# mandt-lab/vbq

Measured on AMD Instinct MI355X. Metric: quantized latents/sec (32-lambda sweep; one count per (element, lambda) pair and entropy-model build), higher is better.
Workload: dtype f32; 1 GPU; kodak24_c256 [36864 x 256] f32, 32-lambda sweep, N=10; step = two-pass entropy-model build (quantizer.py:82-150); elements_per_gpu=9437184, lambdas=32, parallelism=element-sharded x1, launch=one HIP graph replay per step

## Files before the change

### include/vbq.h

```cpp
#ifndef VBQ_H_
#define VBQ_H_

#include <stddef.h>
#include <stdint.h>

#ifdef __cplusplus
extern "C" {
#endif

#define VBQ_ABI_VERSION 5

enum {
    VBQ_OK = 0,
    VBQ_ERR_INVALID_ARGUMENT = -1,
    VBQ_ERR_UNSUPPORTED = -2,
    VBQ_ERR_LAUNCH = -3,
    VBQ_ERR_WORKSPACE = -4
};

enum {
    VBQ_LAYOUT_BC = 0,
    VBQ_LAYOUT_CB = 1,
    VBQ_LAYOUT_BC_TO_CB = 2
};

enum {
    VBQ_MODE_F32 = 0,
    VBQ_MODE_F64_SCORE = 1
};

int vbq_abi_version(void);
const char *vbq_last_error(void);


enum { VBQ_GRID_K1 = 0, VBQ_GRID_K1T = 1 };
int vbq_solve_grid(int32_t kernel, int64_t n_rows, int32_t n_ch, int32_t workgroups_per_cu, int32_t reserved_workgroups,
                   int64_t *h_grid);

int vbq_device_count(void);
int vbq_device_name(int dev, char *buf, size_t buflen);

size_t vbq_quantize_workspace_bytes(int32_t n_ch, int32_t n_lambda, int32_t N);

int vbq_check_inputs_f32(const float *d_mu, const float *d_sigma, int64_t n, uint32_t *d_bad, void *stream);

int vbq_quantize_f32(const float *d_mu, const float *d_sigma, int64_t n_rows, int32_t n_ch,
                     int32_t layout, const float *d_table_lm, const float *d_level_len,
                     const double *h_lambdas, int32_t n_lambda, int32_t N, int32_t mode,
                     uint16_t *d_out_idx, float *d_out_zhat, float *d_out_bits,
                     void *d_workspace, size_t workspace_bytes, void *stream);

int vbq_n_bit_intervals_f32(const float *d_z_cb, int64_t n_rows, int32_t n_ch, const float *d_table_lm, int32_t N,
                            float *d_left, float *d_right, void *stream);

int vbq_quantize_rows_f32(const float *d_mu, const float *d_sigma, int64_t n_rows, int32_t n_ch,
                          int32_t layout, const float *d_table_lm, const float *d_level_len,
                          const double *h_lambdas, int32_t n_lambda, int32_t N, int32_t mode,
                          uint16_t *d_out_idx, float *d_out_zhat, float *d_out_bits,
                          void *d_workspace, size_t workspace_bytes, int64_t row_begin, int64_t row_end,
                          int32_t workgroups_per_cu, int32_t reserved_workgroups, void *stream);

int vbq_level_counts_f32(const float *d_mu, const float *d_sigma, int64_t n_rows, int32_t n_ch,
                         int32_t layout, const float *d_table_lm, const float *d_level_len,
                         const double *h_lambdas, int32_t n_lambda, int32_t N, int64_t *d_level_counts,
                         void *d_workspace, size_t workspace_bytes, int32_t reserved_workgroups, void *stream);

int vbq_code_lengths_from_counts(const void *d_counts, int32_t counts_are_i32, int64_t n,
                                 const float *d_lut, int64_t lut_n, int32_t level_period,
                                 float *d_out_len, float *d_out_model, void *stream);

typedef void (*vbq_f32_loop)(char **args, const intptr_t *dimensions, const intptr_t *steps, void *data);
typedef struct vbq_host_stage {
    const void *h_counts;
    int32_t counts_are_i32;
    int32_t add_level;
    int64_t n_rows;
    int64_t K;
    float add_n_smoothing;
    int32_t status;
    vbq_f32_loop log2_loop;
    void *log2_data;
    float *h_out_model;
    float *h_out_len;
    int64_t runs;
} vbq_host_stage;
int vbq_host_neg_log2_freq_f32(const void *h_counts, int32_t counts_are_i32, int64_t n_rows, int64_t K, float add_n_smoothing,
                               int32_t add_level, vbq_f32_loop log2_loop, void *log2_data, float *h_out_model,
                               float *h_out_len);
void vbq_host_stage_run(void *stage);

int vbq_argmax_candidates_f32(const float *d_P, const float *d_len, int32_t len_per_lambda,
                              const float *d_mu, const float *d_sigma, int64_t n_elems,
                              const double *h_lambdas, int32_t n_lambda, int32_t M, int32_t mode,
                              int32_t *d_out_j, float *d_out_zhat, float *d_out_bits, void *stream);

int vbq_xi_intervals_f64(const double *d_xi, int64_t K, int32_t N, double *d_left, double *d_right, void *stream);
int vbq_xi_select_f64(const double *d_F, const double *d_endpoints, const double *d_unsquashed, int64_t K, int32_t N,
                      double lamb, double *d_z_hat, int64_t *d_num_bits, double *d_xi_hat, double *d_f_z_hat, void *stream);

int vbq_quantize_notebook_f64(const float *d_means, const float *d_stds, int64_t n,
                              const double *d_codebook_lm, const double *h_betas, int32_t n_beta,
                              int32_t N, uint16_t *d_out_idx, float *d_out_val, void *stream);

int vbq_histogram_u16(const uint16_t *d_idx, int64_t n_rows, int32_t n_ch, int32_t layout,
                      int32_t n_lambda, int32_t N, int64_t *d_counts, void *stream);

int vbq_histogram_u16_i32(const uint16_t *d_idx, int64_t n_rows, int32_t n_ch, int32_t layout,
                          int32_t n_lambda, int32_t N, int32_t *d_counts, void *stream);

int vbq_histogram_rows_u16(const uint16_t *d_idx, int64_t n_rows, int32_t n_ch, int32_t layout,
                           int32_t n_lambda, int32_t N, void *d_counts, int32_t counts_are_i32,
                           int64_t row_begin, int64_t row_end, void *stream);

int vbq_histogram_models_u16(const uint16_t *d_idx, int64_t n_rows, int32_t n_ch, int32_t n_lambda, int32_t N,
                             void *d_counts, int32_t counts_are_i32, const float *d_lut, int64_t lut_n,
                             float *d_models, void *stream);

int vbq_index_max_u16(const uint16_t *d_idx, int64_t n, uint32_t *d_max, void *stream);

int vbq_moments_f32(const float *d_x, int64_t n_rows, int32_t n_ch, int32_t layout,
                    double *d_out , void *stream);

size_t vbq_numpy_sum_sq_workspace_bytes(int64_t n);
int vbq_numpy_sum_sq_f32(const float *d_x, int64_t n, float *d_out, void *d_workspace, size_t workspace_bytes,
                         void *stream);

size_t vbq_numpy_row_sums_workspace_bytes(int64_t n_rows, int64_t n);
int vbq_numpy_row_sums_f32(const float *d_x, int64_t n_rows, int64_t n, float *d_out, void *d_workspace,
                           size_t workspace_bytes, void *stream);

int vbq_gather_f32(const uint16_t *d_idx, int64_t n_rows, int32_t n_ch, int32_t layout,
                   int32_t n_lambda, int32_t N, const float *d_tab, int32_t tab_per_lambda,
                   float *d_out, int32_t out_layout, void *stream);

int vbq_rd_sums_u16(const float *d_mu, const float *d_sigma, const uint16_t *d_idx, int64_t n_rows, int32_t n_ch,
                    int32_t layout, int32_t n_lambda, int32_t N, const float *d_tab_sorted, const float *d_rate,
                    int32_t rate_per_lambda, double *d_out, void *stream);

int vbq_transpose_f32(const float *d_in, int64_t n_rows, int64_t n_cols, float *d_out, void *stream);

int vbq_transpose_planes(const void *d_in, int64_t n_batch, int64_t n_rows, int64_t n_cols, int32_t elem_bytes,
                         void *d_out, void *stream);

enum { VBQ_SPREAD_SIGMA = 0, VBQ_SPREAD_VARIANCE = 1, VBQ_SPREAD_LOGVAR = 2 };
int vbq_prep_planes_f32(const float *d_means_bc, const float *d_spread_bc, int32_t spread_kind, int64_t n_rows,
                        int32_t n_ch, float *d_mu_cb, float *d_sigma_cb, void *stream);
int vbq_gather_latents_u16(const uint16_t *d_idx_planes, int64_t n_rows, int32_t n_ch, int32_t n_lambda, int32_t N,
                           const float *d_table_sorted, const float *d_level_len, const float *d_models,
                           float *d_out_zhat, void *d_out_raw_bits, float *d_out_num_bits, uint16_t *d_out_idx,
                           void *stream);
size_t vbq_compress_latents_workspace_bytes(int64_t n_rows, int32_t n_ch, int32_t n_lambda, int32_t N);
int vbq_compress_latents_f32(const float *d_means_bc, const float *d_spread_bc, int32_t spread_kind,
                             int64_t n_rows, int32_t n_ch, const float *d_table_lm, const float *d_table_sorted,
                             const float *d_level_len, const float *d_models, const double *h_lambdas,
                             int32_t n_lambda, int32_t N, float *d_out_zhat, void *d_out_raw_bits,
                             float *d_out_num_bits, void *d_workspace, size_t workspace_bytes, void *stream);

size_t vbq_build_entropy_models_workspace_bytes(int64_t n_rows, int32_t n_ch, int32_t n_lambda, int32_t N);
int vbq_build_entropy_models_f32(const float *d_means_bc, const float *d_spread_bc, int32_t spread_kind, int64_t n_rows,
                                 int32_t n_ch, const float *d_table_lm, const double *h_lambdas, int32_t n_lambda,
                                 int32_t N, const float *d_lut_levels, int64_t n_lut_levels, const float *d_lut_ranks,
                                 int64_t n_lut_ranks, int64_t *d_level_counts, float *d_level_len, float *d_raw_models,
                                 void *d_counts, int32_t counts_are_i32, float *d_models, void *d_workspace,
                                 size_t workspace_bytes, int32_t reserved_workgroups, void *stream);

#define VBQ_BMSHJ_PARAMS_PER_CHANNEL 43

int vbq_bmshj_cdf_pdf_f32(const float *d_params, const float *d_x, int64_t n_rows, int32_t n_ch,
                          float *d_cdf, float *d_pdf, float *d_logpdf, void *stream);

int vbq_bmshj_icdf_step_f32(const float *d_params, const float *d_xi, int64_t n_rows, int32_t n_ch,
                            float *d_left, float *d_right, float *d_mid, uint32_t *d_flags,
                            void *stream);

int vbq_bmshj_icdf_chain_f32(const float *d_params, const float *d_xi, int64_t n_rows, int32_t n_ch,
                             float *d_left, float *d_right, float *d_mid, uint32_t *d_flags, int32_t n_steps,
                             float tol, int32_t first, void *stream);

int vbq_bmshj_nll_grad_f32(const float *d_params, const float *d_x_cb, int64_t n_rows, int32_t n_ch,
                           double *d_out , void *stream);

int vbq_rans_encode_u16(const uint16_t *d_idx, int64_t n_streams, int64_t n, int32_t N, int32_t seg,
                        const uint16_t *d_freq, uint16_t *d_words, uint32_t *d_sizes, void *stream);
int vbq_rans_sizes_u16(const uint16_t *d_idx, int64_t n_streams, int64_t n, int32_t N, int32_t seg, const uint16_t *d_freq,
                       uint32_t *d_sizes, void *stream);
int vbq_rans_decode_u16(const uint16_t *d_words, const uint32_t *d_sizes, int64_t n_streams, int64_t n,
                        int32_t N, int32_t seg, const uint16_t *d_freq, uint16_t *d_idx, uint32_t *d_status,
                        void *stream);
int vbq_rans_pack_u16(const uint16_t *d_words, const uint32_t *d_sizes, int64_t n_streams, int64_t n, int32_t seg,
                      uint16_t *d_payload, int64_t *d_offsets, uint64_t *d_total, void *stream);
int vbq_rans_unpack_u16(const uint16_t *d_payload, int64_t n_words, const uint16_t *d_sizes_in, int64_t n_streams,
                        int64_t n, int32_t seg, uint16_t *d_words, uint32_t *d_sizes, int64_t *d_offsets,
                        uint32_t *d_status, void *stream);
int vbq_rans_segment_offsets_u16(const uint16_t *d_sizes, int64_t M, int32_t seg, int64_t n_words, int64_t *d_offsets,
                                 uint32_t *d_status, void *stream);
int vbq_rans_decode_values_f32(const uint16_t *d_payload, int64_t n_words, const uint16_t *d_sizes, const int64_t *d_offsets,
                               int64_t n, int32_t seg, int32_t N, const uint16_t *d_freq, const float *d_values,
                               const int64_t *d_segments, int64_t n_sel, float *d_out, uint32_t *d_status, void *stream);

int vbq_rans_il_sizes_u16(const uint16_t *d_idx, int64_t n_streams, int64_t n, int32_t N, int32_t part,
                          const uint16_t *d_freq, uint32_t *d_sizes, void *stream);
int vbq_rans_il_encode_u16(const uint16_t *d_idx, int64_t n_streams, int64_t n, int32_t N, int32_t part,
                           const uint16_t *d_freq, const uint32_t *d_sizes, const int64_t *d_offsets, uint16_t *d_payload,
                           int64_t n_words, void *stream);
int vbq_rans_il_decode_u16(const uint16_t *d_payload, int64_t n_words, const uint32_t *d_sizes, const int64_t *d_offsets,
                           int64_t n_streams, int64_t n, int32_t N, int32_t part, const uint16_t *d_freq, uint16_t *d_idx,
                           uint32_t *d_status, void *stream);

int vbq_rans_map_encode_u16(const uint16_t *d_idx, int32_t n_planes, const uint8_t *d_cls, int32_t n_classes, int64_t n_streams,
                            int64_t n, int32_t N, int32_t seg, const uint16_t *d_freq, uint16_t *d_words, uint32_t *d_sizes,
                            void *stream);
int vbq_rans_map_sizes_u16(const uint16_t *d_idx, int32_t n_planes, const uint8_t *d_cls, int32_t n_classes, int64_t n_streams,
                           int64_t n, int32_t N, int32_t seg, const uint16_t *d_freq, uint32_t *d_sizes, void *stream);
int vbq_rans_map_decode_u16(const uint16_t *d_words, const uint32_t *d_sizes, const uint8_t *d_cls, int32_t n_classes,
                            int64_t n_streams, int64_t n, int32_t N, int32_t seg, const uint16_t *d_freq, uint16_t *d_idx,
                            uint32_t *d_status, void *stream);

int vbq_pack_counts_3x21(const int32_t *d_counts, int64_t n, int64_t *d_words, int32_t n_ranks,
                         uint32_t *d_overflow, void *stream);
int vbq_unpack_counts_3x21(const int64_t *d_words, int64_t n, int32_t *d_counts, void *stream);

#define VBQ_COMM_ID_BYTES 128
// ... 75 lines not shown
```

### vbq_amd/_lib.py

```python
from __future__ import annotations

import ctypes as C
import os


_LIB = None

c_f32p = C.c_void_p
c_u16p = C.c_void_p

OK = 0
ABI_VERSION = 5
LAYOUT_BC, LAYOUT_CB, LAYOUT_BC_TO_CB = 0, 1, 2
MODE_F32, MODE_F64_SCORE = 0, 1
BMSHJ_PARAMS_PER_CHANNEL = 43
COMM_ID_BYTES = 128

SIGNATURES = {
    "vbq_abi_version": (C.c_int, []),
    "vbq_last_error": (C.c_char_p, []),
    "vbq_solve_grid": (C.c_int, [C.c_int32, C.c_int64, C.c_int32, C.c_int32, C.c_int32, C.POINTER(C.c_int64)]),
    "vbq_device_count": (C.c_int, []),
    "vbq_device_name": (C.c_int, [C.c_int, C.c_char_p, C.c_size_t]),
    "vbq_quantize_workspace_bytes": (C.c_size_t, [C.c_int32, C.c_int32, C.c_int32]),
    "vbq_check_inputs_f32": (C.c_int, [C.c_void_p, C.c_void_p, C.c_int64, C.c_void_p, C.c_void_p]),
    "vbq_quantize_f32": (C.c_int, [C.c_void_p, C.c_void_p, C.c_int64, C.c_int32, C.c_int32, C.c_void_p, C.c_void_p,
                                   C.POINTER(C.c_double), C.c_int32, C.c_int32, C.c_int32, C.c_void_p, C.c_void_p,
                                   C.c_void_p, C.c_void_p, C.c_size_t, C.c_void_p]),
    "vbq_n_bit_intervals_f32": (C.c_int, [C.c_void_p, C.c_int64, C.c_int32, C.c_void_p, C.c_int32, C.c_void_p, C.c_void_p,
                                          C.c_void_p]),
    "vbq_quantize_rows_f32": (C.c_int, [C.c_void_p, C.c_void_p, C.c_int64, C.c_int32, C.c_int32, C.c_void_p, C.c_void_p,
                                        C.POINTER(C.c_double), C.c_int32, C.c_int32, C.c_int32, C.c_void_p, C.c_void_p,
                                        C.c_void_p, C.c_void_p, C.c_size_t, C.c_int64, C.c_int64, C.c_int32, C.c_int32, C.c_void_p]),
    "vbq_level_counts_f32": (C.c_int, [C.c_void_p, C.c_void_p, C.c_int64, C.c_int32, C.c_int32, C.c_void_p, C.c_void_p,
                                       C.POINTER(C.c_double), C.c_int32, C.c_int32, C.c_void_p, C.c_void_p, C.c_size_t,
                                       C.c_int32, C.c_void_p]),
    "vbq_code_lengths_from_counts": (C.c_int, [C.c_void_p, C.c_int32, C.c_int64, C.c_void_p, C.c_int64, C.c_int32,
                                               C.c_void_p, C.c_void_p, C.c_void_p]),
    "vbq_host_neg_log2_freq_f32": (C.c_int, [C.c_void_p, C.c_int32, C.c_int64, C.c_int64, C.c_float, C.c_int32, C.c_void_p, C.c_void_p,
                                             C.c_void_p, C.c_void_p]),
    "vbq_host_stage_run": (None, [C.c_void_p]),
    "vbq_histogram_rows_u16": (C.c_int, [C.c_void_p, C.c_int64, C.c_int32, C.c_int32, C.c_int32, C.c_int32, C.c_void_p,
                                         C.c_int32, C.c_int64, C.c_int64, C.c_void_p]),
    "vbq_xi_intervals_f64": (C.c_int, [C.c_void_p, C.c_int64, C.c_int32, C.c_void_p, C.c_void_p, C.c_void_p]),
    "vbq_xi_select_f64": (C.c_int, [C.c_void_p, C.c_void_p, C.c_void_p, C.c_int64, C.c_int32, C.c_double, C.c_void_p,
                                    C.c_void_p, C.c_void_p, C.c_void_p, C.c_void_p]),
    "vbq_quantize_notebook_f64": (C.c_int, [C.c_void_p, C.c_void_p, C.c_int64, C.c_void_p, C.POINTER(C.c_double),
                                            C.c_int32, C.c_int32, C.c_void_p, C.c_void_p, C.c_void_p]),
    "vbq_histogram_u16": (C.c_int, [C.c_void_p, C.c_int64, C.c_int32, C.c_int32, C.c_int32, C.c_int32, C.c_void_p,
                                    C.c_void_p]),
    "vbq_histogram_u16_i32": (C.c_int, [C.c_void_p, C.c_int64, C.c_int32, C.c_int32, C.c_int32, C.c_int32,
                                        C.c_void_p, C.c_void_p]),
    "vbq_histogram_models_u16": (C.c_int, [C.c_void_p, C.c_int64, C.c_int32, C.c_int32, C.c_int32, C.c_void_p, C.c_int32,
                                           C.c_void_p, C.c_int64, C.c_void_p, C.c_void_p]),
    "vbq_index_max_u16": (C.c_int, [C.c_void_p, C.c_int64, C.c_void_p, C.c_void_p]),
    "vbq_moments_f32": (C.c_int, [C.c_void_p, C.c_int64, C.c_int32, C.c_int32, C.c_void_p, C.c_void_p]),
    "vbq_numpy_sum_sq_workspace_bytes": (C.c_size_t, [C.c_int64]),
    "vbq_numpy_sum_sq_f32": (C.c_int, [C.c_void_p, C.c_int64, C.c_void_p, C.c_void_p, C.c_size_t, C.c_void_p]),
    "vbq_numpy_row_sums_workspace_bytes": (C.c_size_t, [C.c_int64, C.c_int64]),
    "vbq_numpy_row_sums_f32": (C.c_int, [C.c_void_p, C.c_int64, C.c_int64, C.c_void_p, C.c_void_p, C.c_size_t, C.c_void_p]),
    "vbq_gather_f32": (C.c_int, [C.c_void_p, C.c_int64, C.c_int32, C.c_int32, C.c_int32, C.c_int32, C.c_void_p,
                                 C.c_int32, C.c_void_p, C.c_int32, C.c_void_p]),
    "vbq_rd_sums_u16": (C.c_int, [C.c_void_p, C.c_void_p, C.c_void_p, C.c_int64, C.c_int32, C.c_int32, C.c_int32, C.c_int32,
                                  C.c_void_p, C.c_void_p, C.c_int32, C.c_void_p, C.c_void_p]),
    "vbq_transpose_f32": (C.c_int, [C.c_void_p, C.c_int64, C.c_int64, C.c_void_p, C.c_void_p]),
    "vbq_transpose_planes": (C.c_int, [C.c_void_p, C.c_int64, C.c_int64, C.c_int64, C.c_int32, C.c_void_p, C.c_void_p]),
    "vbq_prep_planes_f32": (C.c_int, [C.c_void_p, C.c_void_p, C.c_int32, C.c_int64, C.c_int32, C.c_void_p, C.c_void_p, C.c_void_p]),
    "vbq_gather_latents_u16": (C.c_int, [C.c_void_p, C.c_int64, C.c_int32, C.c_int32, C.c_int32, C.c_void_p, C.c_void_p,
                                         C.c_void_p, C.c_void_p, C.c_void_p, C.c_void_p, C.c_void_p, C.c_void_p]),
    "vbq_compress_latents_workspace_bytes": (C.c_size_t, [C.c_int64, C.c_int32, C.c_int32, C.c_int32]),
    "vbq_compress_latents_f32": (C.c_int, [C.c_void_p, C.c_void_p, C.c_int32, C.c_int64, C.c_int32, C.c_void_p, C.c_void_p,
                                           C.c_void_p, C.c_void_p, C.POINTER(C.c_double), C.c_int32, C.c_int32, C.c_void_p,
                                           C.c_void_p, C.c_void_p, C.c_void_p, C.c_size_t, C.c_void_p]),
    "vbq_build_entropy_models_workspace_bytes": (C.c_size_t, [C.c_int64, C.c_int32, C.c_int32, C.c_int32]),
    "vbq_build_entropy_models_f32": (C.c_int, [C.c_void_p, C.c_void_p, C.c_int32, C.c_int64, C.c_int32, C.c_void_p,
                                               C.POINTER(C.c_double), C.c_int32, C.c_int32, C.c_void_p, C.c_int64, C.c_void_p,
                                               C.c_int64, C.c_void_p, C.c_void_p, C.c_void_p, C.c_void_p, C.c_int32, C.c_void_p,
                                               C.c_void_p, C.c_size_t, C.c_int32, C.c_void_p]),
    "vbq_argmax_candidates_f32": (C.c_int, [C.c_void_p, C.c_void_p, C.c_int32, C.c_void_p, C.c_void_p, C.c_int64,
                                            C.POINTER(C.c_double), C.c_int32, C.c_int32, C.c_int32, C.c_void_p,
                                            C.c_void_p, C.c_void_p, C.c_void_p]),
    "vbq_bmshj_cdf_pdf_f32": (C.c_int, [C.c_void_p, C.c_void_p, C.c_int64, C.c_int32, C.c_void_p, C.c_void_p,
                                        C.c_void_p, C.c_void_p]),
    "vbq_bmshj_icdf_step_f32": (C.c_int, [C.c_void_p, C.c_void_p, C.c_int64, C.c_int32, C.c_void_p, C.c_void_p,
                                          C.c_void_p, C.c_void_p, C.c_void_p]),
    "vbq_bmshj_icdf_chain_f32": (C.c_int, [C.c_void_p, C.c_void_p, C.c_int64, C.c_int32, C.c_void_p, C.c_void_p,
                                           C.c_void_p, C.c_void_p, C.c_int32, C.c_float, C.c_int32, C.c_void_p]),
    "vbq_uniform_quantize_f32": (C.c_int, [C.c_void_p, C.c_int64, C.c_float, C.c_float, C.c_float, C.c_int32, C.c_void_p,
                                           C.c_void_p, C.c_void_p, C.c_void_p]),
    "vbq_nearest_code_f64": (C.c_int, [C.c_void_p, C.c_int64, C.c_void_p, C.c_int32, C.c_void_p, C.c_void_p, C.c_void_p,
                                       C.c_void_p]),
    "vbq_analogy_ranks_workspace_bytes": (C.c_size_t, [C.c_int64, C.c_int32, C.c_int64]),
    "vbq_analogy_ranks_f32": (C.c_int, [C.c_void_p, C.c_int64, C.c_int32, C.c_void_p, C.c_int64, C.c_void_p, C.c_void_p,
                                        C.c_size_t, C.c_void_p]),
    "vbq_image_sqerr_u8": (C.c_int, [C.c_void_p, C.c_void_p, C.c_int64, C.c_int64, C.c_void_p, C.c_void_p]),
    "vbq_u8_to_f64": (C.c_int, [C.c_void_p, C.c_int64, C.c_void_p, C.c_void_p]),
    "vbq_unit_to_u8_f32": (C.c_int, [C.c_void_p, C.c_int64, C.c_void_p, C.c_void_p]),
    "vbq_ssim_scale_workspace_bytes": (C.c_size_t, [C.c_int32, C.c_int32, C.c_int32, C.c_int32, C.c_int32]),
    "vbq_ssim_scale_f64": (C.c_int, [C.c_void_p, C.c_void_p, C.c_int32, C.c_int32, C.c_int32, C.c_int32, C.c_void_p, C.c_int32,
                                     C.c_double, C.c_double, C.c_void_p, C.c_void_p, C.c_void_p, C.c_size_t, C.c_void_p]),
    "vbq_downsample2_f64": (C.c_int, [C.c_void_p, C.c_int32, C.c_int32, C.c_int32, C.c_int32, C.c_void_p, C.c_void_p]),
    "vbq_pack_counts_3x21": (C.c_int, [C.c_void_p, C.c_int64, C.c_void_p, C.c_int32, C.c_void_p, C.c_void_p]),
    "vbq_unpack_counts_3x21": (C.c_int, [C.c_void_p, C.c_int64, C.c_void_p, C.c_void_p]),
    "vbq_comm_unique_id": (C.c_int, [C.c_void_p]),
    "vbq_comm_init": (C.c_int, [C.POINTER(C.c_void_p), C.c_int32, C.c_void_p, C.c_int32]),
    "vbq_allreduce_hist": (C.c_int, [C.c_void_p, C.c_void_p, C.c_int64, C.c_int32, C.c_void_p]),
    "vbq_comm_destroy": (C.c_int, [C.c_void_p]),
    "vbq_rans_encode_u16": (C.c_int, [C.c_void_p, C.c_int64, C.c_int64, C.c_int32, C.c_int32, C.c_void_p, C.c_void_p,
                                      C.c_void_p, C.c_void_p]),
    "vbq_rans_sizes_u16": (C.c_int, [C.c_void_p, C.c_int64, C.c_int64, C.c_int32, C.c_int32, C.c_void_p, C.c_void_p,
                                     C.c_void_p]),
    "vbq_rans_decode_u16": (C.c_int, [C.c_void_p, C.c_void_p, C.c_int64, C.c_int64, C.c_int32, C.c_int32, C.c_void_p,
                                      C.c_void_p, C.c_void_p, C.c_void_p]),
    "vbq_rans_pack_u16": (C.c_int, [C.c_void_p, C.c_void_p, C.c_int64, C.c_int64, C.c_int32, C.c_void_p, C.c_void_p,
                                    C.c_void_p, C.c_void_p]),
    "vbq_rans_unpack_u16": (C.c_int, [C.c_void_p, C.c_int64, C.c_void_p, C.c_int64, C.c_int64, C.c_int32, C.c_void_p,
                                      C.c_void_p, C.c_void_p, C.c_void_p, C.c_void_p]),
    "vbq_rans_segment_offsets_u16": (C.c_int, [C.c_void_p, C.c_int64, C.c_int32, C.c_int64, C.c_void_p, C.c_void_p,
                                               C.c_void_p]),
    "vbq_rans_decode_values_f32": (C.c_int, [C.c_void_p, C.c_int64, C.c_void_p, C.c_void_p, C.c_int64, C.c_int32, C.c_int32,
                                             C.c_void_p, C.c_void_p, C.c_void_p, C.c_int64, C.c_void_p, C.c_void_p,
                                             C.c_void_p]),
    "vbq_rans_il_sizes_u16": (C.c_int, [C.c_void_p, C.c_int64, C.c_int64, C.c_int32, C.c_int32, C.c_void_p, C.c_void_p,
                                        C.c_void_p]),
    "vbq_rans_il_encode_u16": (C.c_int, [C.c_void_p, C.c_int64, C.c_int64, C.c_int32, C.c_int32, C.c_void_p, C.c_void_p,
                                         C.c_void_p, C.c_void_p, C.c_int64, C.c_void_p]),
    "vbq_rans_il_decode_u16": (C.c_int, [C.c_void_p, C.c_int64, C.c_void_p, C.c_void_p, C.c_int64, C.c_int64, C.c_int32,
                                         C.c_int32, C.c_void_p, C.c_void_p, C.c_void_p, C.c_void_p]),
    "vbq_rans_map_encode_u16": (C.c_int, [C.c_void_p, C.c_int32, C.c_void_p, C.c_int32, C.c_int64, C.c_int64, C.c_int32,
                                          C.c_int32, C.c_void_p, C.c_void_p, C.c_void_p, C.c_void_p]),
    "vbq_rans_map_sizes_u16": (C.c_int, [C.c_void_p, C.c_int32, C.c_void_p, C.c_int32, C.c_int64, C.c_int64, C.c_int32,
                                         C.c_int32, C.c_void_p, C.c_void_p, C.c_void_p]),
    "vbq_rans_map_decode_u16": (C.c_int, [C.c_void_p, C.c_void_p, C.c_void_p, C.c_int32, C.c_int64, C.c_int64, C.c_int32,
                                          C.c_int32, C.c_void_p, C.c_void_p, C.c_void_p, C.c_void_p]),
    "vbq_bmshj_nll_grad_f32":(C.c_int, [C.c_void_p, C.c_void_p, C.c_int64, C.c_int32, C.c_void_p, C.c_void_p]),
    "vbq_budget_dp_workspace_bytes": (C.c_size_t, [C.c_int64, C.c_int32, C.c_int32, C.c_int32]),
    "vbq_budget_dp_f64": (C.c_int, [C.c_void_p, C.c_int64, C.c_int32, C.c_int32, C.c_int32, C.c_void_p, C.c_void_p, C.c_void_p,
                                    C.c_void_p, C.c_size_t, C.c_void_p]),
    "vbq_budget_patience_f64": (C.c_int, [C.c_void_p, C.c_int64, C.c_int32, C.c_double, C.c_int32, C.c_void_p, C.c_void_p,
                                          C.c_void_p]),
    "vbq_records_words": (C.c_size_t, [C.c_int32, C.c_int32, C.c_int32]),
    "vbq_records_pack_u16": (C.c_int, [C.c_void_p, C.c_int64, C.c_int32, C.c_int32, C.c_int32, C.c_void_p, C.c_void_p,
                                       C.c_void_p]),
    "vbq_records_unpack_f32": (C.c_int, [C.c_void_p, C.c_int64, C.c_int32, C.c_int32, C.c_int32, C.c_void_p, C.c_int32,
                                         C.c_void_p, C.c_int64, C.c_void_p, C.c_void_p, C.c_void_p, C.c_void_p]),
    "vbq_topk_workspace_bytes": (C.c_size_t, [C.c_int64, C.c_int32, C.c_int64, C.c_int32, C.c_int32]),
    "vbq_records_topk_f32": (C.c_int, [C.c_void_p, C.c_int64, C.c_int32, C.c_int32, C.c_int32, C.c_void_p, C.c_int32,
                                       C.c_void_p, C.c_int64, C.c_int32, C.c_int32, C.c_void_p, C.c_int32, C.c_void_p,
                                       C.c_void_p, C.c_void_p, C.c_int32, C.c_void_p, C.c_size_t, C.c_void_p]),
    "vbq_topk_f32": (C.c_int, [C.c_void_p, C.c_int64, C.c_int32, C.c_void_p, C.c_int64, C.c_int32, C.c_int32, C.c_void_p,
                               C.c_int32, C.c_void_p, C.c_void_p, C.c_int32, C.c_void_p, C.c_size_t, C.c_void_p]),
    "vbq_records_bag_f32": (C.c_int, [C.c_void_p, C.c_int64, C.c_int32, C.c_int32, C.c_int32, C.c_void_p, C.c_int32,
                                      C.c_void_p, C.c_int64, C.c_void_p, C.c_int64, C.c_void_p, C.c_int32, C.c_void_p,
                                      C.c_void_p, C.c_void_p]),
    "vbq_bag_f32": (C.c_int, [C.c_void_p, C.c_int64, C.c_int32, C.c_void_p, C.c_int64, C.c_void_p, C.c_int64, C.c_void_p,
                              C.c_int32, C.c_void_p, C.c_void_p, C.c_void_p]),
    "vbq_rans_decode_window_f32": (C.c_int, [C.c_void_p, C.c_int64, C.c_void_p, C.c_void_p, C.c_int64, C.c_void_p, C.c_int32,
                                             C.c_void_p, C.c_int32, C.c_void_p, C.c_int32, C.c_int32, C.c_int32, C.c_int32,
                                             C.c_void_p, C.c_int32, C.c_void_p, C.c_int64, C.c_int64, C.c_int64, C.c_void_p,
                                             C.c_void_p, C.c_void_p]),
    "vbq_rans_encode_files_u16": (C.c_int, [C.c_void_p, C.c_int64, C.c_void_p, C.c_int32, C.c_void_p, C.c_int64, C.c_int32,
                                            C.c_int32, C.c_int32, C.c_void_p, C.c_int32, C.c_void_p, C.c_void_p, C.c_void_p,
                                            C.c_int64, C.c_void_p, C.c_void_p]),
    "vbq_rans_sizes_files_u16": (C.c_int, [C.c_void_p, C.c_int64, C.c_int64, C.c_void_p, C.c_int32, C.c_void_p, C.c_int64,
                                           C.c_int32, C.c_int32, C.c_int32, C.c_void_p, C.c_int32, C.c_void_p, C.c_void_p,
                                           C.c_void_p, C.c_void_p]),
}


class HostStageDesc(C.Structure):
    _fields_ = [("h_counts", C.c_void_p), ("counts_are_i32", C.c_int32), ("add_level", C.c_int32), ("n_rows", C.c_int64),
                ("K", C.c_int64), ("add_n_smoothing", C.c_float), ("status", C.c_int32), ("log2_loop", C.c_void_p),
                ("log2_data", C.c_void_p), ("h_out_model", C.c_void_p), ("h_out_len", C.c_void_p), ("runs", C.c_int64)]


class VBQError(RuntimeError):
    pass


def library_path() -> str:
    from . import build as _build
    return os.environ.get("VBQ_HIP_LIBRARY", _build.LIB)


def lib():
    global _LIB
    if _LIB is not None:
        return _LIB
    path = library_path()
    if not os.path.exists(path):
        raise VBQError(f"HIP extension not built: {path} is missing. Run `python -m vbq_amd.build` "
# ... 23 lines not shown
```

### vbq_amd/csrc/vbq_common.h

```cpp
#pragma once

#include <hip/hip_runtime.h>
#include <stdint.h>

#include "vbq.h"

namespace vbq {

void set_error(const char *fmt, ...);

int num_cus();
int fast_debug();
int64_t resident_slots(int per_cu, int reserved);

#define VBQ_REQUIRE(cond, code, ...)            \
    do {                                        \
        if (!(cond)) {                          \
            ::vbq::set_error(__VA_ARGS__);      \
            return (code);                      \
        }                                       \
    } while (0)

#define VBQ_CHECK_LAUNCH(what)                                                        \
    do {                                                                              \
        hipError_t e__ = hipGetLastError();                                           \
        if (e__ != hipSuccess) {                                                      \
            ::vbq::set_error("%s: %s", (what), hipGetErrorString(e__));               \
            return VBQ_ERR_LAUNCH;                                                    \
        }                                                                             \
    } while (0)

__device__ __forceinline__ void set_issue_priority(unsigned int p) {
    p = __builtin_amdgcn_readfirstlane(p) & 3u;
    if (p == 0) __builtin_amdgcn_s_setprio(0);
    else if (p == 1) __builtin_amdgcn_s_setprio(1);
    else if (p == 2) __builtin_amdgcn_s_setprio(2);
    else __builtin_amdgcn_s_setprio(3);
}
__device__ __forceinline__ unsigned int wave_slot() { return __builtin_amdgcn_s_getreg((3 << 11) | 4); }
__device__ __forceinline__ void rotate_issue_priority(unsigned int &rot) {
#ifndef VBQ_NO_ISSUE_ROTATION
    set_issue_priority(rot);
    rot += 3u;
#endif
}

constexpr int kWave = 64;
constexpr int kTileChannels = 16;
constexpr int kMaxLambdaChunk = 32;

__host__ __device__ constexpr int table_size(int N) { return (2 << N) - 1; }

__device__ __forceinline__ float neg_half_sq_err(float P, float mu, float sigma) {
    float d = __fsub_rn(P, mu);
    float t = __fdiv_rn(d, sigma);
    float q = __fmul_rn(t, t);
    return __fmul_rn(-0.5f, q);
}

#ifdef VBQ_ONLY_N10
#define VBQ_FOR_EACH_N(X) X(10)
#else
#define VBQ_FOR_EACH_N(X) X(12) X(11) X(10) X(9) X(8) X(7) X(6) X(5) X(4)
#endif

struct Lambdas32 {
    float lam[kMaxLambdaChunk];
};

template <int N>
int launch_quant_fast(const float *mu, const float *sg, int64_t n_per_ch, int64_t ch_stride, int32_t n_ch, const float *table,
                      const Lambdas32 &lam, const float *len, int32_t L, uint16_t *out_idx, float *out_zhat,
                      float *out_bits, int64_t E, int vec_ok,
                      unsigned long long *level_counts, int wg_per_cu, int reserved, hipStream_t st);

template <int N>
int launch_quant_pruned(const float *mu, const float *sg, int64_t n_per_ch, int64_t ch_stride, int32_t n_ch, const float *table,
                        const Lambdas32 &lam, const float *len, int32_t L, uint16_t *out_idx, int64_t E, int vec_ok, hipStream_t st);

int launch_level_counts_hull10(const float *mu, const float *sg, int64_t n_per_ch, int64_t ch_stride, int32_t n_ch,
                               const float *table, const double *lam, int32_t L, int vec_ok,
                               unsigned long long *level_counts, int reserved, hipStream_t st);

int launch_quant_hull_idx10(const float *mu, const float *sg, int64_t n_per_ch, int64_t ch_stride, int32_t n_ch,
                            const float *table, const double *lam, int32_t L, int vec_ok, uint16_t *out_idx, int64_t E,
                            hipStream_t st);

}
```

### vbq_amd/csrc/vbq_latents.hip

```cpp
#include <atomic>

#include <type_traits>

#include "vbq_common.h"

namespace vbq {
namespace {

constexpr int kGlRows = 32, kGlCh = 64;
template <int N>
__global__ void __launch_bounds__(256)
k_gather_latents(const uint16_t *__restrict__ idx, long B, int C, const float *__restrict__ tab_sorted,
                 const float *__restrict__ level_len, const float *__restrict__ models, float *__restrict__ out_z,
                 float *__restrict__ out_raw, int raw_as_int, float *__restrict__ out_nb, uint16_t *__restrict__ out_idx) {
    constexpr int T = table_size(N), N1 = N + 1;
    __shared__ float tz[kGlCh][kGlRows + 1], tr[kGlCh][kGlRows + 1], tn[kGlCh][kGlRows + 1];
    __shared__ uint16_t tq[kGlCh][kGlRows + 2];
    const int l = blockIdx.y;
    const long ctiles = (C + kGlCh - 1) / kGlCh;
    const long r0 = ((long)blockIdx.x / ctiles) * kGlRows;
    const int c0 = (int)((long)blockIdx.x % ctiles) * kGlCh;
    const long E = B * (long)C;
    {
        const int tx = threadIdx.x & 31, ty = threadIdx.x >> 5;
// ... 318 lines not shown
}

namespace vbq {
namespace {
__global__ void __launch_bounds__(256)
k_gather(const uint16_t *__restrict__ idx, long n_rows, int C, int layout, long E, int T,
         const float *__restrict__ tab, int per_lambda, float *__restrict__ out) {
    const int l = blockIdx.y;
    const uint16_t *src = idx + (long)l * E;
    float *dst = out + (long)l * E;
    const float *tl = tab + (per_lambda ? (long)l * C * T : 0);
    for (long e = (long)blockIdx.x * blockDim.x + threadIdx.x; e < E; e += (long)gridDim.x * blockDim.x) {
        const int c = (C == 1) ? 0 : (layout == VBQ_LAYOUT_BC ? (int)(e % C) : (int)(e / n_rows));
        dst[e] = tl[(long)c * T + min((int)src[e], T - 1)];
    }
}

__global__ void __launch_bounds__(256)
k_gather_transpose(const uint16_t *__restrict__ idx, long in_rows, long in_cols, int in_layout, long E, int C, int T,
                   const float *__restrict__ tab, int per_lambda, float *__restrict__ out) {
    __shared__ float tile[32][33];
    const int l = blockIdx.z;
    const uint16_t *src = idx + (long)l * E;
    float *dst = out + (long)l * E;
    const float *tl = tab + (per_lambda ? (long)l * C * T : 0);
    const long ctiles = (in_cols + 31) / 32;
    const long r0 = ((long)blockIdx.x / ctiles) * 32, c0 = ((long)blockIdx.x % ctiles) * 32;
    const int tx = threadIdx.x & 31, ty = threadIdx.x >> 5;
#pragma unroll
    for (int k = 0; k < 4; ++k) {
        const long r = r0 + ty + 8 * k, c = c0 + tx;
        if (r < in_rows && c < in_cols) {
            const int ch = in_layout == VBQ_LAYOUT_CB ? (int)r : (int)c;
            tile[ty + 8 * k][tx] = tl[(long)ch * T + min((int)src[r * in_cols + c], T - 1)];
        }
    }
    __syncthreads();
#pragma unroll
    for (int k = 0; k < 4; ++k) {
        const long c = c0 + ty + 8 * k, r = r0 + tx;
        if (r < in_rows && c < in_cols) dst[c * in_rows + r] = tile[tx][ty + 8 * k];
    }
}
}
}

extern "C" int vbq_gather_f32(const uint16_t *d_idx, int64_t n_rows, int32_t n_ch, int32_t layout,
                              int32_t n_lambda, int32_t N, const float *d_tab, int32_t tab_per_lambda,
                              float *d_out, int32_t out_layout, void *stream) {
    using namespace vbq;
    VBQ_REQUIRE(n_rows == 0 || (d_idx && d_tab && d_out), VBQ_ERR_INVALID_ARGUMENT, "vbq_gather_f32: null pointer argument");
    VBQ_REQUIRE(n_rows >= 0 && n_ch >= 1 && n_lambda >= 1 && n_lambda <= 65535 && N >= 0 && N <= 15,
                VBQ_ERR_INVALID_ARGUMENT, "vbq_gather_f32: bad sizes");
    VBQ_REQUIRE((layout == VBQ_LAYOUT_BC || layout == VBQ_LAYOUT_CB) &&
                    (out_layout == VBQ_LAYOUT_BC || out_layout == VBQ_LAYOUT_CB),
                VBQ_ERR_INVALID_ARGUMENT, "vbq_gather_f32: unknown layout %d -> %d", layout, out_layout);
    if (n_rows == 0) return VBQ_OK;
    const int64_t E = n_rows * (int64_t)n_ch;
    if (n_ch > 1 && layout != out_layout) {
        const int64_t in_rows = layout == VBQ_LAYOUT_CB ? n_ch : n_rows;
        const int64_t in_cols = layout == VBQ_LAYOUT_CB ? n_rows : n_ch;
        const int64_t tiles = ((in_cols + 31) / 32) * ((in_rows + 31) / 32);
        VBQ_REQUIRE(n_lambda <= 65535 && tiles <= 0x7fffffffll, VBQ_ERR_UNSUPPORTED,
                    "vbq_gather_f32: grid too large for the transposing form");
        hipLaunchKernelGGL(k_gather_transpose, dim3((unsigned)tiles, 1, (unsigned)n_lambda),
                           dim3(256), 0, reinterpret_cast<hipStream_t>(stream), d_idx, (long)in_rows, (long)in_cols,
                           (int)layout, (long)E, (int)n_ch, table_size(N), d_tab, (int)tab_per_lambda, d_out);
        VBQ_CHECK_LAUNCH("gather_transpose");
        return VBQ_OK;
    }
    int64_t gx = (E + 255) / 256;
    const int64_t cap = 4096 / n_lambda + 1;
    if (gx > cap) gx = cap;
    hipLaunchKernelGGL(k_gather, dim3((unsigned)gx, (unsigned)n_lambda), dim3(256), 0,
                       reinterpret_cast<hipStream_t>(stream), d_idx, (long)n_rows, (int)n_ch, (int)layout, (long)E,
                       table_size(N), d_tab, (int)tab_per_lambda, d_out);
    VBQ_CHECK_LAUNCH("gather");
    return VBQ_OK;
}

extern "C" size_t vbq_compress_latents_workspace_bytes(int64_t n_rows, int32_t n_ch, int32_t n_lambda, int32_t N) {
    if (n_rows < 0 || n_ch <= 0 || n_lambda <= 0 || N < 0) return 0;
    const size_t E = (size_t)n_rows * (size_t)n_ch;
    return 2 * vbq::align256(E * sizeof(float)) + vbq::align256((size_t)n_lambda * E * sizeof(uint16_t)) +
           vbq::align256(vbq_quantize_workspace_bytes(n_ch, n_lambda, N));
}

extern "C" int vbq_compress_latents_f32(const float *d_means_bc, const float *d_spread_bc, int32_t spread_kind,
                                        int64_t n_rows, int32_t n_ch, const float *d_table_lm, const float *d_table_sorted,
                                        const float *d_level_len, const float *d_models, const double *h_lambdas,
                                        int32_t n_lambda, int32_t N, float *d_out_zhat, void *d_out_raw_bits,
                                        float *d_out_num_bits, void *d_workspace, size_t workspace_bytes, void *stream) {
    using namespace vbq;
    VBQ_REQUIRE(n_rows >= 0 && n_ch >= 1 && n_lambda >= 1, VBQ_ERR_INVALID_ARGUMENT, "vbq_compress_latents_f32: bad sizes");
    if (n_rows == 0) return VBQ_OK;
    const size_t need = vbq_compress_latents_workspace_bytes(n_rows, n_ch, n_lambda, N);
    VBQ_REQUIRE(d_workspace && workspace_bytes >= need, VBQ_ERR_WORKSPACE, "vbq_compress_latents_f32: workspace of %zu bytes given, %zu needed",
                workspace_bytes, need);
    VBQ_REQUIRE((reinterpret_cast<uintptr_t>(d_workspace) & 255) == 0, VBQ_ERR_INVALID_ARGUMENT,
                "vbq_compress_latents_f32: workspace must be 256-byte aligned");
    const size_t E = (size_t)n_rows * (size_t)n_ch;
    char *w = static_cast<char *>(d_workspace);
    float *mu_cb = reinterpret_cast<float *>(w);
    w += align256(E * sizeof(float));
    float *sg_cb = reinterpret_cast<float *>(w);
    w += align256(E * sizeof(float));
    uint16_t *idx = reinterpret_cast<uint16_t *>(w);
    w += align256((size_t)n_lambda * E * sizeof(uint16_t));
    const size_t qws = vbq_quantize_workspace_bytes(n_ch, n_lambda, N);
    int rc = vbq_prep_planes_f32(d_means_bc, d_spread_bc, spread_kind, n_rows, n_ch, mu_cb, sg_cb, stream);
    if (rc != VBQ_OK) return rc;
    rc = vbq_quantize_f32(mu_cb, sg_cb, n_rows, n_ch, VBQ_LAYOUT_CB, d_table_lm, d_level_len, h_lambdas, n_lambda, N, VBQ_MODE_F32,
                          idx, nullptr, nullptr, w, qws, stream);
    if (rc != VBQ_OK) return rc;
    return vbq_gather_latents_u16(idx, n_rows, n_ch, n_lambda, N, d_table_sorted, d_level_len, d_models, d_out_zhat, d_out_raw_bits,
                                  d_out_num_bits, nullptr, stream);
}

extern "C" size_t vbq_build_entropy_models_workspace_bytes(int64_t n_rows, int32_t n_ch, int32_t n_lambda, int32_t N) {
    return vbq_compress_latents_workspace_bytes(n_rows, n_ch, n_lambda, N);
}

extern "C" int vbq_build_entropy_models_f32(const float *d_means_bc, const float *d_spread_bc, int32_t spread_kind, int64_t n_rows,
                                            int32_t n_ch, const float *d_table_lm, const double *h_lambdas, int32_t n_lambda,
                                            int32_t N, const float *d_lut_levels, int64_t n_lut_levels, const float *d_lut_ranks,
                                            int64_t n_lut_ranks, int64_t *d_level_counts, float *d_level_len, float *d_raw_models,
                                            void *d_counts, int32_t counts_are_i32, float *d_models, void *d_workspace,
                                            size_t workspace_bytes, int32_t reserved_workgroups, void *stream) {
    using namespace vbq;
    VBQ_REQUIRE(n_rows >= 1 && n_ch >= 1 && n_lambda >= 1 && N >= 0 && N <= 15, VBQ_ERR_INVALID_ARGUMENT,
                "vbq_build_entropy_models_f32: bad sizes");
    VBQ_REQUIRE(d_lut_levels && n_lut_levels > n_rows && d_level_counts && d_level_len && d_raw_models && d_counts,
                VBQ_ERR_INVALID_ARGUMENT, "vbq_build_entropy_models_f32: null pointer argument, or a code-length table shorter than n_rows + 1");
    VBQ_REQUIRE((d_models == nullptr) == (d_lut_ranks == nullptr) && (!d_lut_ranks || n_lut_ranks > n_rows), VBQ_ERR_INVALID_ARGUMENT,
                "vbq_build_entropy_models_f32: d_models and d_lut_ranks go together (n_rows + 1 entries)");
    const size_t need = vbq_build_entropy_models_workspace_bytes(n_rows, n_ch, n_lambda, N);
    VBQ_REQUIRE(d_workspace && workspace_bytes >= need, VBQ_ERR_WORKSPACE,
                "vbq_build_entropy_models_f32: workspace of %zu bytes given, %zu needed", workspace_bytes, need);
    VBQ_REQUIRE((reinterpret_cast<uintptr_t>(d_workspace) & 255) == 0, VBQ_ERR_INVALID_ARGUMENT,
                "vbq_build_entropy_models_f32: workspace must be 256-byte aligned");
    const size_t E = (size_t)n_rows * (size_t)n_ch;
    const int64_t N1 = N + 1;
    char *w = static_cast<char *>(d_workspace);
    float *mu_cb = reinterpret_cast<float *>(w);
    w += align256(E * sizeof(float));
    float *sg_cb = reinterpret_cast<float *>(w);
    w += align256(E * sizeof(float));
    uint16_t *idx = reinterpret_cast<uint16_t *>(w);
    w += align256((size_t)n_lambda * E * sizeof(uint16_t));
    const size_t qws = vbq_quantize_workspace_bytes(n_ch, n_lambda, N);
    hipStream_t st = reinterpret_cast<hipStream_t>(stream);
    int rc = vbq_prep_planes_f32(d_means_bc, d_spread_bc, spread_kind, n_rows, n_ch, mu_cb, sg_cb, stream);
    if (rc != VBQ_OK) return rc;
    hipError_t e = hipMemsetAsync(d_level_counts, 0, sizeof(int64_t) * (size_t)n_lambda * (size_t)n_ch * (size_t)N1, st);
    if (e != hipSuccess) {
        set_error("vbq_build_entropy_models_f32: hipMemsetAsync: %s", hipGetErrorString(e));
        return VBQ_ERR_LAUNCH;
    }
    rc = vbq_level_counts_f32(mu_cb, sg_cb, n_rows, n_ch, VBQ_LAYOUT_CB, d_table_lm, nullptr, h_lambdas, n_lambda, N, d_level_counts, w, qws,
                              reserved_workgroups, stream);
    if (rc != VBQ_OK) return rc;
    rc = vbq_code_lengths_from_counts(d_level_counts, 0, (int64_t)n_lambda * n_ch * N1, d_lut_levels, n_lut_levels, (int32_t)N1, d_level_len,
                                      d_raw_models, stream);
    if (rc != VBQ_OK) return rc;
    rc = vbq_quantize_rows_f32(mu_cb, sg_cb, n_rows, n_ch, VBQ_LAYOUT_CB, d_table_lm, d_level_len, h_lambdas, n_lambda, N, VBQ_MODE_F32, idx,
                               nullptr, nullptr, w, qws, 0, n_rows, 0, reserved_workgroups, stream);
    if (rc != VBQ_OK) return rc;
    return vbq_histogram_models_u16(idx, n_rows, n_ch, n_lambda, N, d_counts, counts_are_i32, d_lut_ranks, n_lut_ranks, d_models, stream);
}
```

### vbq_amd/csrc/vbq_quantize.hip

```cpp
#include "vbq_common.h"

namespace vbq {
namespace {

template <int N>
struct Elem {
    float a[N + 1];
    float b[N + 1];
    uint32_t G;
};

template <int N>
__device__ __forceinline__ void search_and_score(const float *tb, float z, float sg, Elem<N> &e) {
    uint32_t g = 0;
#pragma unroll
    for (int n = 0; n <= N; ++n) {
        const int off = (1 << n) - 1;
        const int m = 1 << n;
        const uint32_t j = g;
        const float pj = tb[off + j];
        const bool below = pj < z;
        if (n == 0) {
            const float s0 = neg_half_sq_err(pj, z, sg);
            e.a[0] = s0;
// ... 192 lines not shown

    const int c0 = blockIdx.y * kTileChannels;
    const int ncg = min(kTileChannels, C - c0);
    for (int i = threadIdx.x; i < ncg * T; i += blockDim.x) {
        const int ch = i / T, s = i - ch * T;
        tb[ch * TS + s] = table[(long)(c0 + ch) * T + s];
    }
    if constexpr (kPenInLds) {
        for (int i = threadIdx.x; i < L * ncg * N1; i += blockDim.x) {
            const int n = i % N1;
            const int ch = (i / N1) % ncg;
            const int l = i / (N1 * ncg);
            pl[(l * kTileChannels + ch) * PS + n] = pen[((long)l * C + c0 + ch) * N1 + n];
        }
    }
    __syncthreads();

    const int cl = threadIdx.x & (kTileChannels - 1);
    const int slot = threadIdx.x >> 4;
    if (cl >= ncg) return;
    const float *mytb = tb + cl * TS;
    const int c = c0 + cl;

    for (long rb = (long)blockIdx.x * kRowsPerIter; rb < n_rows; rb += (long)gridDim.x * kRowsPerIter) {
        Elem<N> el[kTiledNE];
        long row[kTiledNE];
#pragma unroll
        for (int k = 0; k < kTiledNE; ++k) {
            row[k] = rb + k * 64 + slot;
            const bool ok = row[k] < n_rows;
            const float m = ok ? mu[row[k] * C + c] : 0.0f;
            const float s = ok ? sg[row[k] * C + c] : 1.0f;
            search_and_score<N>(mytb, m, s, el[k]);
        }
        for (int l = 0; l < L; ++l) {
            PenT p[N1];
            const PenT *pp = kPenInLds ? pl + (l * kTileChannels + cl) * PS : pen + ((long)l * C + c) * N1;
#pragma unroll
            for (int n = 0; n < N1; ++n) p[n] = pp[n];
#pragma unroll
            for (int k = 0; k < kTiledNE; ++k) {
                int bj;
                if constexpr (sizeof(PenT) == 4) bj = argmax_scan<N>(el[k], p);
                else bj = argmax_scan_f64<N>(el[k], p);
                int lvl; uint32_t pos;
                winner_slot<N>(el[k].G, bj, lvl, pos);
                if (row[k] < n_rows) {
                    const long o = (long)l * E + row[k] * C + c;
                    out_idx[o] = (uint16_t)(((2 * pos + 1) << (N - lvl)) - 1);
                    if (out_zhat) out_zhat[o] = mytb[(1 << lvl) - 1 + pos];
                    if (out_bits) out_bits[o] = len ? len[((long)l * C + c) * N1 + lvl] : (float)lvl;
                }
            }
        }
    }
}

template <int N>
__global__ void __launch_bounds__(256)
k_intervals(const float *__restrict__ z_cb, long n_rows, const float *__restrict__ table, float *__restrict__ left,
            float *__restrict__ right) {
    constexpr int T = table_size(N);
    __shared__ float tb[T + 1];
    const int c = blockIdx.y;
    for (int i = threadIdx.x; i < T; i += blockDim.x) tb[i] = table[(long)c * T + i];
    __syncthreads();
    for (long b = (long)blockIdx.x * blockDim.x + threadIdx.x; b < n_rows; b += (long)gridDim.x * blockDim.x) {
        const float z = z_cb[(long)c * n_rows + b];
        uint32_t g = 0;
#pragma unroll
        for (int n = 0; n <= N; ++n) {
            const int off = (1 << n) - 1;
            const int m = 1 << n;
            const uint32_t j = g;
            const float pj = tb[off + j];
            const bool below = pj < z;
            float l = pj, r = pj;
            if (n > 0) {
                int jo = below ? (int)j + 1 : (int)j - 1;
                jo = jo < 0 ? 0 : (jo > m - 1 ? m - 1 : jo);
                bool swap = false;
                if (n == N && below && j == (uint32_t)(m - 1)) { jo = m - 2; swap = true; }
                const float po = tb[off + jo];
                const bool j_is_left = below && !swap;
                l = j_is_left ? pj : po;
                r = j_is_left ? po : pj;
            }
            const long o = ((long)c * (N + 1) + n) * n_rows + b;
            left[o] = l;
            right[o] = r;
            g = 2 * g + (below ? 1u : 0u);
        }
    }
}

template <int N, typename PenT>
int launch_quantize(const float *mu, const float *sg, int64_t n_rows, int32_t n_ch, int32_t layout,
                    const float *table, const float *level_len, const double *h_lambdas, int32_t L,
                    uint16_t *out_idx, float *out_zhat, float *out_bits, void *ws, int64_t row_begin, int64_t row_end,
                    unsigned long long *level_counts, int wg_per_cu, int reserved, hipStream_t st) {
    constexpr int N1 = N + 1;
    const int64_t E = n_rows * (int64_t)n_ch;
    const int64_t n_sub = row_end - row_begin;
    PenT *pen = reinterpret_cast<PenT *>(ws);
    const bool bc_to_cb = layout == VBQ_LAYOUT_BC_TO_CB && n_ch > 1;
    const bool flat = (n_ch == 1) || (layout == VBQ_LAYOUT_CB) || bc_to_cb;

    for (int l0 = 0; l0 < L; l0 += kMaxLambdaChunk) {
        const int Lc = (L - l0 < kMaxLambdaChunk) ? (L - l0) : kMaxLambdaChunk;
        LambdaChunk lc;
        for (int i = 0; i < kMaxLambdaChunk; ++i) lc.lam[i] = i < Lc ? h_lambdas[l0 + i] : 0.0;
        const int total = Lc * n_ch * N1;
        const float *len_c = level_len ? level_len + (int64_t)l0 * n_ch * N1 : nullptr;
        bool pen_ready = false;
        auto prepare = [&]() -> int {
            if (pen_ready) return VBQ_OK;
            hipLaunchKernelGGL((k_prepare_penalties<PenT>), dim3((total + 255) / 256), dim3(256), 0, st, lc, Lc,
                               (int)n_ch, N1, len_c, pen);
            VBQ_CHECK_LAUNCH("prepare_penalties");
            pen_ready = true;
            return VBQ_OK;
        };
        Lambdas32 l32;
        for (int i = 0; i < kMaxLambdaChunk; ++i) l32.lam[i] = i < Lc ? (float)lc.lam[i] : 0.0f;

        const int64_t off = (flat && !bc_to_cb) ? row_begin : row_begin * n_ch;
        const int64_t off_out = flat ? row_begin : row_begin * n_ch;
        const float *mu_r = mu + off, *sg_r = sg + off;
        uint16_t *oi = out_idx ? out_idx + (int64_t)l0 * E + off_out : nullptr;
        float *oz = out_zhat ? out_zhat + (int64_t)l0 * E + off_out : nullptr;
        float *ob = out_bits ? out_bits + (int64_t)l0 * E + off_out : nullptr;
        unsigned long long *lc_out = level_counts ? level_counts + (int64_t)l0 * n_ch * N1 : nullptr;
        if (flat) {
            const int64_t n_per_ch = n_sub;
            const int64_t ch_stride = n_rows;
            const int vec_ok = ((n_rows % 4 == 0) || n_ch == 1) &&
                               ((reinterpret_cast<uintptr_t>(mu_r) | reinterpret_cast<uintptr_t>(sg_r)) % 16 == 0) &&
                               (reinterpret_cast<uintptr_t>(oi) % 8 == 0) && (E % 4 == 0 || L == 1) &&
                               (!oz || reinterpret_cast<uintptr_t>(oz) % 16 == 0) &&
                               (!ob || reinterpret_cast<uintptr_t>(ob) % 16 == 0);
            const int vec2_ok = ((reinterpret_cast<uintptr_t>(mu_r) | reinterpret_cast<uintptr_t>(sg_r)) % 4 == 0) &&
                                (reinterpret_cast<uintptr_t>(oi) % 2 == 0) && (!oz || reinterpret_cast<uintptr_t>(oz) % 4 == 0) &&
                                (!ob || reinterpret_cast<uintptr_t>(ob) % 4 == 0);
            const int64_t nquads = (n_per_ch + 3) / 4;
            int64_t gx = (nquads + 255) / 256;
            const int64_t cap = (int64_t)num_cus() * 8 / (n_ch < 8 ? n_ch : 8) + 1;
            if (gx > cap) gx = cap;
            if (gx < 1) gx = 1;
            bool fast_ok = sizeof(PenT) == 4;
            for (int i = 0; i < Lc; ++i) fast_ok = fast_ok && (lc.lam[i] >= 1.9e-12 && lc.lam[i] <= 1.8e19);
            if constexpr (sizeof(PenT) == 4 && N == 10) {
                if (fast_ok && lc_out && !len_c) {
                    const int r = launch_level_counts_hull10(mu_r, sg_r, n_per_ch, ch_stride, n_ch, table, lc.lam, Lc,
                                                             vec2_ok | (bc_to_cb ? 2 : 0), lc_out, reserved, st);
                    if (r == VBQ_OK) continue;
                    if (r < 0) return r;
                }
            }
            if constexpr (sizeof(PenT) == 4 && N == 10) {
                if (fast_ok && !lc_out && !len_c && oi && !oz && !ob) {
                    const int r = launch_quant_hull_idx10(mu_r, sg_r, n_per_ch, ch_stride, n_ch, table, lc.lam, Lc,
                                                          vec2_ok | (bc_to_cb ? 2 : 0), oi, E, st);
                    if (r == VBQ_OK) continue;
                    if (r < 0) return r;
                }
            }
            if constexpr (sizeof(PenT) == 4) {
                if (!lc_out && oi && !oz && !ob && wg_per_cu == 0) {
                    const int r = launch_quant_pruned<N>(mu_r, sg_r, n_per_ch, ch_stride, n_ch, table, l32, len_c, Lc, oi, E,
                                                         vec2_ok | (bc_to_cb ? 2 : 0), st);
                    if (r == VBQ_OK) continue;
                    if (r < 0) return r;
                }
            }
            if constexpr (sizeof(PenT) == 4) {
                if (fast_ok) {
                    const int r = launch_quant_fast<N>(mu_r, sg_r, n_per_ch, ch_stride, n_ch, table, l32, len_c, Lc, oi, oz, ob,
                                                       E, vec2_ok | (bc_to_cb ? 2 : 0), lc_out, wg_per_cu, reserved, st);
                    if (r != VBQ_OK) return r;
                    continue;
                }
            }
            if (level_counts) {
                set_error("vbq_level_counts_f32 is served by the fast f32 kernel only (every lambda in [1.9e-12, 1.8e19]); "
                          "use vbq_quantize_f32 + vbq_histogram_u16 instead");
                return VBQ_ERR_UNSUPPORTED;
            }
            if (bc_to_cb) {
                set_error("vbq_quantize_f32: VBQ_LAYOUT_BC_TO_CB is served by the fast f32 kernel only (VBQ_MODE_F32, every "
                          "lambda in [1.9e-12, 1.8e19]); transpose with vbq_transpose_f32 and use VBQ_LAYOUT_CB instead");
                return VBQ_ERR_UNSUPPORTED;
            }
            if (const int r = prepare(); r != VBQ_OK) return r;
            hipLaunchKernelGGL((k_quant_flat<N, PenT>), dim3((unsigned)gx, (unsigned)n_ch), dim3(256), 0, st, mu_r, sg_r,
                               (long)n_per_ch, (long)ch_stride, (int)n_ch, table, pen, len_c, Lc, oi, oz, ob, (long)E, vec_ok);
            VBQ_CHECK_LAUNCH("quant_flat");
        } else if constexpr (N > 10) {
            set_error("vbq_quantize_f32: N=%d is built for channel-major planes only (VBQ_LAYOUT_CB, or n_ch = 1): "
                      "16 tables of %d points do not fit the LDS; transpose with vbq_transpose_f32 first", N, table_size(N));
            return VBQ_ERR_UNSUPPORTED;
        } else {
            constexpr int T = table_size(N);
            constexpr int PS = (N1 + 3) & ~3;
            const size_t lds = sizeof(float) * kTileChannels * (T + 2) + 16 +
                               (sizeof(PenT) == 4 ? sizeof(PenT) * (size_t)kMaxLambdaChunk * kTileChannels * PS : 0);
            {
                hipError_t e = hipFuncSetAttribute(reinterpret_cast<const void *>(&k_quant_tiled<N, PenT>),
                                                   hipFuncAttributeMaxDynamicSharedMemorySize, (int)lds);
                if (e != hipSuccess) {
                    set_error("hipFuncSetAttribute(%zu B LDS): %s", lds, hipGetErrorString(e));
                    return VBQ_ERR_LAUNCH;
                }
            }
            const int groups = (n_ch + kTileChannels - 1) / kTileChannels;
            int64_t iters = (n_sub + kRowsPerIter - 1) / kRowsPerIter;
            int64_t gx = (256 + groups - 1) / groups;
            if (gx > iters) gx = iters;
            if (gx < 1) gx = 1;
            if (const int r = prepare(); r != VBQ_OK) return r;
            hipLaunchKernelGGL((k_quant_tiled<N, PenT>), dim3((unsigned)gx, (unsigned)groups), dim3(kTiledThreads),
                               lds, st, mu_r, sg_r, (long)n_sub, (int)n_ch, table, pen, len_c, Lc, oi, oz, ob, (long)E);
            VBQ_CHECK_LAUNCH("quant_tiled");
        }
    }
    return VBQ_OK;
}

}
}

extern "C" size_t vbq_quantize_workspace_bytes(int32_t n_ch, int32_t n_lambda, int32_t N) {
    if (n_ch <= 0 || n_lambda <= 0 || N < 0) return 0;
    const int Lc = n_lambda < vbq::kMaxLambdaChunk ? n_lambda : vbq::kMaxLambdaChunk;
    return (size_t)Lc * (size_t)n_ch * (size_t)(N + 1) * sizeof(double) + 256;
}

namespace vbq {
namespace {
int quantize_entry(const char *who, const float *d_mu, const float *d_sigma, int64_t n_rows, int32_t n_ch, int32_t layout,
                   const float *d_table_lm, const float *d_level_len, const double *h_lambdas, int32_t n_lambda,
                   int32_t N, int32_t mode, uint16_t *d_out_idx, float *d_out_zhat, float *d_out_bits,
                   void *d_workspace, size_t workspace_bytes, int64_t row_begin, int64_t row_end,
                   unsigned long long *level_counts, int32_t wg_per_cu, int32_t reserved_wgs, void *stream) {
    const bool counting = level_counts != nullptr;
    VBQ_REQUIRE(n_rows >= 0 && n_ch >= 1 && n_lambda >= 1, VBQ_ERR_INVALID_ARGUMENT,
                "%s: bad sizes n_rows=%lld n_ch=%d n_lambda=%d", who, (long long)n_rows, n_ch, n_lambda);
    VBQ_REQUIRE(0 <= row_begin && row_begin <= row_end && row_end <= n_rows, VBQ_ERR_INVALID_ARGUMENT,
                "%s: row range [%lld, %lld) outside [0, %lld)", who, (long long)row_begin, (long long)row_end, (long long)n_rows);
    VBQ_REQUIRE(row_begin == row_end || (d_mu && d_sigma && d_table_lm && h_lambdas && (d_out_idx || counting)),
                VBQ_ERR_INVALID_ARGUMENT, "%s: null pointer argument", who);
    VBQ_REQUIRE(layout == VBQ_LAYOUT_BC || layout == VBQ_LAYOUT_CB || layout == VBQ_LAYOUT_BC_TO_CB, VBQ_ERR_INVALID_ARGUMENT,
                "%s: unknown layout %d", who, layout);
    VBQ_REQUIRE(mode == VBQ_MODE_F32 || mode == VBQ_MODE_F64_SCORE, VBQ_ERR_INVALID_ARGUMENT, "%s: unknown mode %d", who, mode);
    VBQ_REQUIRE(!(mode == VBQ_MODE_F64_SCORE && d_level_len), VBQ_ERR_UNSUPPORTED,
                "%s: VBQ_MODE_F64_SCORE supports raw integer lengths only", who);
    VBQ_REQUIRE(n_ch <= 65535, VBQ_ERR_UNSUPPORTED, "%s: n_ch=%d exceeds 65535", who, n_ch);
    VBQ_REQUIRE(wg_per_cu >= 0 && wg_per_cu <= 5, VBQ_ERR_INVALID_ARGUMENT, "%s: workgroups_per_cu=%d not in 0..5", who, wg_per_cu);
    VBQ_REQUIRE(!counting || n_ch == 1 || layout != VBQ_LAYOUT_BC, VBQ_ERR_UNSUPPORTED,
                "%s: channel-last input with n_ch > 1 is not served (use VBQ_LAYOUT_CB planes or VBQ_LAYOUT_BC_TO_CB)", who);
    const size_t need = vbq_quantize_workspace_bytes(n_ch, n_lambda, N);
    VBQ_REQUIRE(d_workspace && workspace_bytes >= need, VBQ_ERR_WORKSPACE, "%s: workspace of %zu bytes given, %zu needed", who,
                workspace_bytes, need);
    if (row_begin == row_end) return VBQ_OK;
    hipStream_t st = reinterpret_cast<hipStream_t>(stream);
    const int reserved = reserved_wgs < 0 ? 0 : reserved_wgs;
#define VBQ_DISPATCH_N(NN)                                                                                         \
    case NN:                                                                                                       \
        return mode == VBQ_MODE_F32                                                                                \
                   ? launch_quantize<NN, float>(d_mu, d_sigma, n_rows, n_ch, layout, d_table_lm, d_level_len,      \
                                                h_lambdas, n_lambda, d_out_idx, d_out_zhat, d_out_bits,            \
                                                d_workspace, row_begin, row_end, level_counts, wg_per_cu, reserved, st) \
                   : launch_quantize<NN, double>(d_mu, d_sigma, n_rows, n_ch, layout, d_table_lm, d_level_len,     \
                                                 h_lambdas, n_lambda, d_out_idx, d_out_zhat, d_out_bits,           \
                                                 d_workspace, row_begin, row_end, level_counts, wg_per_cu, reserved, st);
    switch (N) {
        VBQ_FOR_EACH_N(VBQ_DISPATCH_N)
        default:
            set_error("%s: max_bits_per_coord N=%d not built (have 4 ... 12; only 10 with VBQ_ONLY_N10)", who, N);
            return VBQ_ERR_UNSUPPORTED;
    }
#undef VBQ_DISPATCH_N
}
}
}

extern "C" int vbq_quantize_f32(const float *d_mu, const float *d_sigma, int64_t n_rows, int32_t n_ch,
                                int32_t layout, const float *d_table_lm, const float *d_level_len,
                                const double *h_lambdas, int32_t n_lambda, int32_t N, int32_t mode,
                                uint16_t *d_out_idx, float *d_out_zhat, float *d_out_bits, void *d_workspace,
                                size_t workspace_bytes, void *stream) {
    return vbq::quantize_entry("vbq_quantize_f32", d_mu, d_sigma, n_rows, n_ch, layout, d_table_lm, d_level_len, h_lambdas,
                               n_lambda, N, mode, d_out_idx, d_out_zhat, d_out_bits, d_workspace, workspace_bytes, 0,
                               n_rows, nullptr, 0, -1, stream);
}

extern "C" int vbq_quantize_rows_f32(const float *d_mu, const float *d_sigma, int64_t n_rows, int32_t n_ch,
                                     int32_t layout, const float *d_table_lm, const float *d_level_len,
                                     const double *h_lambdas, int32_t n_lambda, int32_t N, int32_t mode,
                                     uint16_t *d_out_idx, float *d_out_zhat, float *d_out_bits, void *d_workspace,
                                     size_t workspace_bytes, int64_t row_begin, int64_t row_end,
                                     int32_t workgroups_per_cu, int32_t reserved_workgroups, void *stream) {
    return vbq::quantize_entry("vbq_quantize_rows_f32", d_mu, d_sigma, n_rows, n_ch, layout, d_table_lm, d_level_len,
                               h_lambdas, n_lambda, N, mode, d_out_idx, d_out_zhat, d_out_bits, d_workspace, workspace_bytes,
                               row_begin, row_end, nullptr, workgroups_per_cu, reserved_workgroups, stream);
}

extern "C" int vbq_level_counts_f32(const float *d_mu, const float *d_sigma, int64_t n_rows, int32_t n_ch,
                                    int32_t layout, const float *d_table_lm, const float *d_level_len,
                                    const double *h_lambdas, int32_t n_lambda, int32_t N, int64_t *d_level_counts,
                                    void *d_workspace, size_t workspace_bytes, int32_t reserved_workgroups, void *stream) {
    using namespace vbq;
    VBQ_REQUIRE(n_rows == 0 || d_level_counts, VBQ_ERR_INVALID_ARGUMENT, "vbq_level_counts_f32: null pointer argument");
    return quantize_entry("vbq_level_counts_f32", d_mu, d_sigma, n_rows, n_ch, layout, d_table_lm, d_level_len, h_lambdas,
                          n_lambda, N, VBQ_MODE_F32, nullptr, nullptr, nullptr, d_workspace, workspace_bytes, 0, n_rows,
                          reinterpret_cast<unsigned long long *>(d_level_counts), 0, reserved_workgroups, stream);
}

extern "C" int vbq_n_bit_intervals_f32(const float *d_z_cb, int64_t n_rows, int32_t n_ch, const float *d_table_lm, int32_t N,
                                       float *d_left, float *d_right, void *stream) {
    using namespace vbq;
    VBQ_REQUIRE(n_rows >= 0 && n_ch >= 1 && n_ch <= 65535, VBQ_ERR_INVALID_ARGUMENT, "vbq_n_bit_intervals_f32: bad sizes");
    if (n_rows == 0) return VBQ_OK;
    VBQ_REQUIRE(d_z_cb && d_table_lm && d_left && d_right, VBQ_ERR_INVALID_ARGUMENT, "vbq_n_bit_intervals_f32: null pointer argument");
    hipStream_t st = reinterpret_cast<hipStream_t>(stream);
    int64_t gx = (n_rows + 255) / 256;
    const int64_t cap = 2048 / n_ch + 1;
    if (gx > cap) gx = cap;
#define VBQ_DISPATCH_N(NN)                                                                                              \
    case NN:                                                                                                            \
        hipLaunchKernelGGL((k_intervals<NN>), dim3((unsigned)gx, (unsigned)n_ch), dim3(256), 0, st, d_z_cb, (long)n_rows, \
                           d_table_lm, d_left, d_right);                                                                \
        break;
    switch (N) {
        VBQ_FOR_EACH_N(VBQ_DISPATCH_N)
        default:
            set_error("vbq_n_bit_intervals_f32: max_bits_per_coord N=%d not built", N);
            return VBQ_ERR_UNSUPPORTED;
    }
#undef VBQ_DISPATCH_N
    VBQ_CHECK_LAUNCH("n_bit_intervals");
    return VBQ_OK;
}
```

### vbq_amd/csrc/vbq_quantize_fast.hip

```cpp
#include <stddef.h>

#include "vbq_common.h"
#include "vbq_sweep.h"

namespace vbq {
namespace {

constexpr int kFastThreads = 256;
#ifndef VBQ_FAST_NE
#define VBQ_FAST_NE 2
#endif
#ifndef VBQ_FAST_WAVES
#define VBQ_FAST_WAVES 4
#endif
#ifndef VBQ_SLOW_INLINE
#define VBQ_SLOW_INLINE __noinline__
#endif
constexpr int kFastNE = VBQ_FAST_NE;

__device__ __forceinline__ float dist_cost(float P, float mu, double rinv) {
    const float d = __fsub_rn(P, mu);
    const float t = (float)__dmul_rn((double)d, rinv);
    const float q = __fmul_rn(t, t);
    return __fmul_rn(0.5f, q);
}

__device__ __forceinline__ float min3f(float a, float b, float c) { return fminf(fminf(a, b), c); }

template <bool NT>
__device__ __forceinline__ void store_idx2(uint32_t *p, uint32_t v) {
    if constexpr (NT) __builtin_nontemporal_store(v, p);
    else *p = v;
}

template <int M>
__device__ __forceinline__ float min_of(const float (&v)[M]) {
    float t[M];
#pragma unroll
    for (int i = 0; i < M; ++i) t[i] = v[i];
    int m = M;
#pragma unroll
    for (int pass = 0; pass < 8; ++pass) {
        if (m <= 1) break;
        int o = 0;
        int i = 0;
#pragma unroll
        for (; i + 2 < m; i += 3) t[o++] = min3f(t[i], t[i + 1], t[i + 2]);
        if (o == 0) { t[o++] = fminf(t[0], t[1]); i = 2; }
        for (; i < m; ++i) t[o++] = t[i];
        m = o;
    }
    return t[0];
}

template <int N>
struct LevelInfo {
    float dL, dR;
    uint32_t posL, posR;
};

template <int N>
__device__ __forceinline__ LevelInfo<N> descend(const float *tb, int n, float z, double sg, uint32_t &g) {
    const int off = (1 << n) - 1;
    const int m = 1 << n;
    const uint32_t j = g;
    const float pj = tb[off + j];
    const bool below = pj < z;
    LevelInfo<N> r;
    if (n == 0) {
        r.dL = r.dR = dist_cost(pj, z, sg);
        r.posL = r.posR = 0;
    } else {
        int jo = below ? (int)j + 1 : (int)j - 1;
        jo = jo < 0 ? 0 : (jo > m - 1 ? m - 1 : jo);
        bool swap = false;
        if (n == N && below && j == (uint32_t)(m - 1)) { jo = m - 2; swap = true; }
        const float po = tb[off + jo];
        const float dj = dist_cost(pj, z, sg);
        const float dn = dist_cost(po, z, sg);
        const bool j_is_left = below && !swap;
        r.dL = j_is_left ? dj : dn;
        r.dR = j_is_left ? dn : dj;
        r.posL = j_is_left ? j : (uint32_t)jo;
        r.posR = j_is_left ? (uint32_t)jo : j;
    }
    g = 2 * g + (below ? 1u : 0u);
    return r;
}

template <int N>
__device__ VBQ_SLOW_INLINE uint32_t exact_rank_scan(const float *tb, float z, float sigma, const float *pen) {
    const double sg = __ddiv_rn(1.0, (double)sigma);
    uint32_t g = 0;
    float bestL = 0.f, bestR = 0.f;
    uint32_t rkL = 0, rkR = 0;
    for (int n = 0; n <= N; ++n) {
        const LevelInfo<N> li = descend<N>(tb, n, z, sg, g);
        const float p = pen[n];
        const float cL = __fadd_rn(li.dL, p);
        if (n == 0 || cL < bestL) { bestL = cL; rkL = ((2 * li.posL + 1) << (N - n)) - 1; }
        if (n >= 1) {
            const float cR = __fadd_rn(li.dR, p);
            if (n == 1 || cR < bestR) { bestR = cR; rkR = ((2 * li.posR + 1) << (N - n)) - 1; }
        }
    }
    if (N == 0) return rkL;
    return (bestL <= bestR) ? rkL : rkR;
}

template <int N, int MODE>
__global__ void __launch_bounds__(kFastThreads, VBQ_FAST_WAVES)
k_quant_fast(const float *__restrict__ mu, const float *__restrict__ sg, long n_per_ch, long ch_stride, int C,
             const float *__restrict__ table, Lambdas32 lam, const float *__restrict__ len,
             int L, uint16_t *__restrict__ out_idx, float *__restrict__ out_zhat,
             float *__restrict__ out_bits, long E, int vec_ok, int dbg,
             unsigned long long *__restrict__ level_counts) {
    constexpr int T = table_size(N);
    constexpr int N1 = N + 1;
    constexpr int NE = kFastNE;
    constexpr bool EXTRA = MODE == 1;
    constexpr bool COUNT = MODE == 2;
    const bool never_flag = dbg == 2;
    constexpr int PS = (N1 + 3) & ~3;
    __shared__ float tb[T + 1];
    __shared__ uint32_t scratch[N1 * NE * kFastThreads];
    __shared__ __align__(16) float penl[kMaxLambdaChunk * PS];
    const int c = blockIdx.y;
    if (COUNT) {
        for (int i = threadIdx.x; i < N1 * NE * kFastThreads; i += blockDim.x) scratch[i] = 0;
    }
    for (int i = threadIdx.x; i < T; i += blockDim.x) tb[i] = table[(long)c * T + i];
    int odd = 0;
    for (int i = threadIdx.x; i < L * PS; i += blockDim.x) {
        const int l = i / PS, n = i - l * PS;
        const float p = n < N1 ? __fmul_rn(lam.lam[l], len ? len[((long)l * C + c) * N1 + n] : (float)n) : 0.0f;
        penl[i] = p;
        odd |= (len != nullptr && !(p == 0.0f || (p >= 1.8189894e-12f && p <= 1.1805916e21f))) ? 1 : 0;
    }
    const bool force_slow = dbg == 1 || __syncthreads_or(odd) != 0;

    const long base = (long)c * ch_stride;
    const long nquads = (n_per_ch + NE - 1) / NE;

    auto load_group = [&](long q, float (&m)[NE], float (&sv)[NE]) {
        const long i0 = q * NE;
        if (!(vec_ok & 2) && (vec_ok & 1) && (i0 + NE <= n_per_ch)) {
            if constexpr (NE == 4) {
                const float4 mv = *reinterpret_cast<const float4 *>(mu + base + i0);
                const float4 s4v = *reinterpret_cast<const float4 *>(sg + base + i0);
                m[0] = mv.x; m[1] = mv.y; m[2] = mv.z; m[3] = mv.w;
                sv[0] = s4v.x; sv[1] = s4v.y; sv[2] = s4v.z; sv[3] = s4v.w;
            } else {
                const float2 mv = *reinterpret_cast<const float2 *>(mu + base + i0);
                const float2 s2v = *reinterpret_cast<const float2 *>(sg + base + i0);
                m[0] = mv.x; m[1] = mv.y;
                sv[0] = s2v.x; sv[1] = s2v.y;
            }
        } else {
#pragma unroll
            for (int k = 0; k < NE; ++k) {
                const bool ok = i0 + k < n_per_ch;
                const long at = (vec_ok & 2) ? (i0 + k) * C + c : base + i0 + k;
                m[k] = ok ? mu[at] : 0.0f;
                sv[k] = ok ? sg[at] : 1.0f;
            }
        }
    };
    const long q0 = (long)blockIdx.x * blockDim.x + threadIdx.x, qstep = (long)gridDim.x * blockDim.x;
    float mn[NE], sn[NE];
#pragma unroll
    for (int k = 0; k < NE; ++k) { mn[k] = 0.0f; sn[k] = 1.0f; }
    if (q0 < nquads) load_group(q0, mn, sn);
    const bool resident = (vec_ok & 4) != 0;
    unsigned int rot = wave_slot();
    for (long q = q0; q < nquads; q += qstep) {
        if (resident) __builtin_amdgcn_s_setprio(3);
        const long i0 = q * NE;
        const bool full = (vec_ok & 1) && (i0 + NE <= n_per_ch);
        float m4[NE], s4[NE];
#pragma unroll
        for (int k = 0; k < NE; ++k) { m4[k] = mn[k]; s4[k] = sn[k]; }
        {
            const long qn = q + qstep < nquads ? q + qstep : q;
            load_group(qn, mn, sn);
        }

        float du[NE][N1];
        uint32_t g[NE];
        double rinv[NE];
#pragma unroll
        for (int k = 0; k < NE; ++k) {
            g[k] = 0;
            rinv[k] = __ddiv_rn(1.0, (double)s4[k]);
        }
        const char *tbb = reinterpret_cast<const char *>(tb);
#pragma unroll
        for (int n = 0; n <= N; ++n) {
            constexpr int kWordMask = 0xffe00000u;
            const int off4 = 4 * ((1 << n) - 1);
            const int top4 = 4 * ((1 << n) - 1);
#pragma unroll
            for (int k = 0; k < NE; ++k) {
                const float pj = *reinterpret_cast<const float *>(tbb + off4 + g[k]);
                const bool below = pj < m4[k];
                float dL, dR;
                uint32_t lo4, hi4;
                if (n == 0) {
                    dL = dR = dist_cost(pj, m4[k], rinv[k]);
                    lo4 = hi4 = 0;
                } else {
                    const uint32_t G4 = g[k] + (below ? 4u : 0u);
                    int lo = (int)G4 - 4;
                    lo = lo < 0 ? 0 : lo;
                    if (n == N) lo = lo > top4 - 4 ? top4 - 4 : lo;
                    lo4 = (uint32_t)lo;
                    hi4 = G4 > (uint32_t)top4 ? (uint32_t)top4 : G4;
                    dL = dist_cost(*reinterpret_cast<const float *>(tbb + off4 + lo4), m4[k], rinv[k]);
                    dR = dist_cost(*reinterpret_cast<const float *>(tbb + off4 + hi4), m4[k], rinv[k]);
                }
                du[k][n] = vmin(dL, dR);
                g[k] = 2 * g[k] + (below ? 4u : 0u);
                if (COUNT) continue;
                const bool r_better = dR < dL;
                const uint32_t b4 = r_better ? hi4 : lo4;
                const uint32_t better = n < N ? (b4 << (N - n - 1)) + ((1u << (N - n)) - 1u) : (b4 >> 1);
                const uint32_t gap = __float_as_uint(__fsub_rn(dR, dL)) ^ 0x80000000u;
                scratch[(n * NE + k) * kFastThreads + threadIdx.x] = (gap & kWordMask) | better;
            }
        }

        if (resident) {
            set_issue_priority(rot);
            rot += 3u;
        }
        for (int l = 0; l < L; ++l) {
            const float *pp = penl + l * PS;
            float p[N1];
#pragma unroll
            for (int n = 0; n < N1; ++n) p[n] = pp[n];
            uint32_t rank[NE];
            float cst[NE][N1];
            float S[NE];
            uint32_t ne[NE];
#pragma unroll
            for (int n = 0; n < N1; ++n)
#pragma unroll
                for (int k = 0; k < NE; ++k) cst[k][n] = __fadd_rn(du[k][n], p[n]);
#pragma unroll
            for (int k = 0; k < NE; ++k) S[k] = min_of<N1>(cst[k]);
            {
#pragma unroll
                for (int k = 0; k < NE; ++k) ne[k] = 0;
#pragma unroll
                for (int n = N; n >= 0; --n)
#pragma unroll
                    for (int k = 0; k < NE; ++k)
                        ne[k] = __builtin_amdgcn_alignbit(ne[k], __float_as_uint(__fsub_rn(S[k], cst[k][n])), 31);
            }
            uint64_t fmk[NE];
            if constexpr (COUNT) {
                uint64_t any_multi = 0;
                uint32_t lvl[NE];
#pragma unroll
                for (int k = 0; k < NE; ++k) {
                    lvl[k] = (uint32_t)__builtin_ctz(~ne[k]);
                    const uint64_t multi = __builtin_amdgcn_uicmp((uint32_t)__popc(ne[k]), (uint32_t)N, 33);
                    fmk[k] = never_flag ? 0ull : (force_slow ? ~0ull : multi);
                    any_multi |= fmk[k];
                }
                if (any_multi != 0) {
                    const uint32_t lane = __lane_id();
#pragma unroll
                    for (int k = 0; k < NE; ++k)
                        if ((fmk[k] >> lane) & 1ull)
                            lvl[k] = (uint32_t)N - (uint32_t)__builtin_ctz(exact_rank_scan<N>(tb, m4[k], s4[k], pp) + 1u);
                }
                const uint32_t lane = threadIdx.x & 63u;
                const uint32_t inc = (lane & 16u) ? 0x10000u : 1u;
#pragma unroll
                for (int k = 0; k < NE; ++k)
                    if (i0 + k < n_per_ch) atomicAdd(&scratch[((uint32_t)(l * N1) + lvl[k]) * 16u + (lane & 15u)], inc);
                continue;
            }
            uint32_t pk[NE];
#pragma unroll
            for (int k = 0; k < NE; ++k) {
                const int n1 = __builtin_ctz(~ne[k]);
                pk[k] = scratch[(n1 * NE + k) * kFastThreads + threadIdx.x];
            }
            uint64_t fm[NE];
// ... 41 lines not shown
                    store_idx2<false>(reinterpret_cast<uint32_t *>(out_idx + o), rank[0] | (rank[1] << 16));
                    if (EXTRA) {
                        if (out_zhat) *reinterpret_cast<float2 *>(out_zhat + o) = make_float2(zh[0], zh[1]);
                        if (out_bits) *reinterpret_cast<float2 *>(out_bits + o) = make_float2(bt[0], bt[1]);
                    }
                }
            } else {
#pragma unroll
                for (int k = 0; k < NE; ++k) {
                    if (i0 + k < n_per_ch) {
                        out_idx[o + k] = (uint16_t)rank[k];
                        if (EXTRA) {
                            if (out_zhat) out_zhat[o + k] = zh[k];
                            if (out_bits) out_bits[o + k] = bt[k];
                        }
                    }
                }
            }
        }
    }
    if constexpr (COUNT) {
        __syncthreads();
        for (int i = threadIdx.x; i < L * N1; i += blockDim.x) {
            unsigned int v = 0;
#pragma unroll
            for (int j = 0; j < 16; ++j) {
                const unsigned int w = scratch[i * 16 + j];
                v += (w & 0xffffu) + (w >> 16);
            }
            const int l = i / N1, n = i - l * N1;
            if (v) atomicAdd(&level_counts[((long)l * C + c) * N1 + n], (unsigned long long)v);
        }
    }
}


#ifndef VBQ_HULL_WAVES
#define VBQ_HULL_WAVES 4
#endif
#ifndef VBQ_HULL_NE
#define VBQ_HULL_NE 2
#endif
#ifndef VBQ_HULL_THREADS
#define VBQ_HULL_THREADS 256
#endif
constexpr int kHullThreads = VBQ_HULL_THREADS;
#ifndef VBQ_HULL_COPIES
#define VBQ_HULL_COPIES 16
#endif
constexpr int kHullKeys = 2048;
constexpr int kFixQueue = 192;
struct HullSweep : SweepTable<32, kHullKeys> {};
static_assert(sizeof(HullSweep) == 2220 && offsetof(HullSweep, val) == 0 && offsetof(HullSweep, perm) == 128 && offsetof(HullSweep, L) == 160 &&
              offsetof(HullSweep, key0) == 164 && offsetof(HullSweep, nkeys) == 168 && offsetof(HullSweep, lut) == 172,
              "HullSweep travels in the kernel arguments: its layout is fixed");

template <int N>
__device__ __forceinline__ void hull_du_nearest(const char *tbb, float z, float sigma, float (&du)[N + 1]) {
    uint32_t g = 0;
    const double rinv = __ddiv_rn(1.0, (double)sigma);
#pragma unroll
    for (int n = 0; n <= N; ++n) {
        const int off4 = 4 * ((1 << n) - 1);
        const int top4 = off4;
        const float pj = *reinterpret_cast<const float *>(tbb + off4 + g);
        const bool below = pj < z;
        float dmin;
        if (n == 0) {
            dmin = __fsub_rn(pj, z);
        } else {
            int o4 = (int)g + (below ? 4 : -4);
            o4 = o4 < 0 ? 0 : (o4 > top4 ? top4 : o4);
            const float po = *reinterpret_cast<const float *>(tbb + off4 + o4);
            dmin = fminf(fabsf(__fsub_rn(pj, z)), fabsf(__fsub_rn(po, z)));
        }
        const float t = (float)__dmul_rn((double)dmin, rinv);
        du[n] = __fmul_rn(0.5f, __fmul_rn(t, t));
        g = 2 * g + (below ? 4u : 0u);
    }
}

template <int N>
__device__ __forceinline__ uint32_t level_of_min(const float (&du)[N + 1], const float *pen, bool &multi) {
    constexpr int N1 = N + 1;
    float cst[N1];
#pragma unroll
    for (int n = 0; n < N1; ++n) cst[n] = __fadd_rn(du[n], pen[n]);
    const float S = min_of<N1>(cst);
    uint32_t ne = 0;
#pragma unroll
    for (int n = N; n >= 0; --n) ne = __builtin_amdgcn_alignbit(ne, __float_as_uint(__fsub_rn(S, cst[n])), 31);
    multi = (uint32_t)__popc(ne) != (uint32_t)N;
    return (uint32_t)__builtin_ctz(~ne);
}

template <int N>
__device__ __forceinline__ void hull_counts_fix(uint64_t lanes, const float (&du_hot)[N + 1], const float *tb, float z, float sigma,
                                                int L, int key0, int nkeys, const unsigned char *perm, const unsigned char *lut,
                                                const float4 *rec, const float *penl, int *corr, bool all_points) {
    constexpr int N1 = N + 1;
    constexpr int PS = (N1 + 3) & ~3;
    const bool mine = (lanes >> (threadIdx.x & 63u)) & 1ull;
    float du[N1];
#pragma unroll
    for (int n = 0; n < N1; ++n) {
        float d = du_hot[n];
        asm volatile("" : "+v"(d));
        du[n] = d;
    }
    float Tn[N];
    uint32_t apos[N];
    sweep_thresholds<N>(du, Tn);
    uint32_t fl = (!(sweep_max_du<N>(du) < kSweepBig) || all_points) ? 0xffffffffu : 0u;
    float G[N];
    uint32_t near = 0;
#pragma unroll
    for (int n = 0; n < N; ++n) {
        float4 nb;
        apos[n] = sweep_position<16>(Tn[n], key0, nkeys, lut, rec, nb);
        G[n] = sweep_band(Tn[n], n, du[n]);
        const float dist = sweep_distance(Tn[n], nb);
        near |= (mine && dist <= G[n]) ? (1u << n) : 0u;
    }
#pragma unroll
    for (int n = 0; n < N; ++n) {
        if ((near >> n) & 1u) {
            for (int l = (int)apos[n] - 1; l >= 0 && fabsf(__fsub_rn(rec[l + 1].x, Tn[n])) <= G[n]; --l) fl |= 1u << l;
            for (int l = (int)apos[n]; l < L && fabsf(__fsub_rn(rec[l + 1].x, Tn[n])) <= G[n]; ++l) fl |= 1u << l;
        }
    }
    fl &= L >= 32 ? 0xffffffffu : ((1u << L) - 1u);
    if (!mine) fl = 0u;
    while (fl != 0u) {
        const int l = __builtin_ctz(fl);
        fl &= fl - 1u;
        const int lo_ = perm[l];
        bool multi;
        int n_ex = (int)level_of_min<N>(du, penl + lo_ * PS, multi);
        if (multi) n_ex = N - __builtin_ctz(exact_rank_scan<N>(tb, z, sigma, penl + lo_ * PS) + 1u);
        int n_pred = 0;
#pragma unroll
        for (int n = 0; n < N; ++n) n_pred += apos[n] > (uint32_t)l ? 1 : 0;
        if (n_ex != n_pred) {
            atomicAdd(&corr[l * N1 + n_ex], 1);
            atomicSub(&corr[l * N1 + n_pred], 1);
        }
    }
}

template <int N>
__global__ void __launch_bounds__(kHullThreads, (VBQ_HULL_WAVES * 256) / kHullThreads)
k_level_counts_hull(const float *__restrict__ mu, const float *__restrict__ sg, long n_per_ch, long ch_stride, int C,
                    const float *__restrict__ table, Lambdas32 lam, HullSweep sw, int vec_ok,
                    unsigned long long *__restrict__ level_counts, int dbg) {
    constexpr int T = table_size(N);
    constexpr int N1 = N + 1;
    constexpr int NE = VBQ_HULL_NE;
    constexpr int KC = VBQ_HULL_COPIES;
    constexpr int PS = (N1 + 3) & ~3;
    constexpr int LB = 33;
    __shared__ float tb[T + 1];
    __shared__ __align__(16) float penl[kMaxLambdaChunk * PS];
    __shared__ __align__(4) unsigned char lut[kHullKeys];
    __shared__ float4 rec[34];
    __shared__ unsigned int H[N * LB * KC];
    __shared__ int corr[kMaxLambdaChunk * N1];
    __shared__ unsigned int n_valid;
    __shared__ unsigned char perm_s[32];
    __shared__ unsigned int fixq[kFixQueue], fixn;
    const int c = blockIdx.y;
    const int L = sw.L;
    for (int i = threadIdx.x; i < T; i += blockDim.x) tb[i] = table[(long)c * T + i];
    for (int i = threadIdx.x; i < L * PS; i += blockDim.x) {
        const int l = i / PS, n = i - l * PS;
        penl[i] = n < N1 ? __fmul_rn(lam.lam[l], (float)n) : 0.0f;
    }
    if (threadIdx.x < 32) perm_s[threadIdx.x] = sw.perm[threadIdx.x];
    for (int i = threadIdx.x; i < N * LB * KC; i += blockDim.x) H[i] = 0;
    for (int i = threadIdx.x; i < L * N1; i += blockDim.x) corr[i] = 0;
    for (int b = threadIdx.x; b < kHullKeys / 4; b += blockDim.x)
        reinterpret_cast<uint32_t *>(lut)[b] = reinterpret_cast<const uint32_t *>(sw.lut)[b];
    if (threadIdx.x < 34) {
        const int i = (int)threadIdx.x;
        rec[i] = sweep_rec(sw.val, L, i);
    }
    if (threadIdx.x == 0) { n_valid = 0; fixn = 0; }
    __syncthreads();

    const bool force_slow = dbg == 1, never_flag = dbg == 2;
    const long base = (long)c * ch_stride;
    const long nquads = (n_per_ch + NE - 1) / NE;
    const char *tbb = reinterpret_cast<const char *>(tb);
    const unsigned int lane = threadIdx.x & 63u;
    const unsigned int inc = (lane & (unsigned)KC) ? 0x10000u : 1u;
    const unsigned int copy = lane & (unsigned)(KC - 1);
    const int key0 = sw.key0, nkeys = sw.nkeys;
    unsigned int my_valid = 0;

    const long q0 = (long)blockIdx.x * blockDim.x + threadIdx.x, qstep = (long)gridDim.x * blockDim.x;
    int it = 0;
    unsigned int rot = wave_slot();
    for (long q = q0; q < nquads; q += qstep, ++it) {
        rotate_issue_priority(rot);
        const long i0 = q * NE;
        const bool full = (vec_ok & 1) && (i0 + NE <= n_per_ch);
        float m4[NE], s4[NE];
        if (vec_ok & 2) {
#pragma unroll
            for (int k = 0; k < NE; ++k) {
                const bool ok = i0 + k < n_per_ch;
                m4[k] = ok ? mu[(i0 + k) * C + c] : 0.0f;
                s4[k] = ok ? sg[(i0 + k) * C + c] : 1.0f;
            }
        } else if (full && NE == 2) {
            const float2 mv = *reinterpret_cast<const float2 *>(mu + base + i0);
            const float2 sv = *reinterpret_cast<const float2 *>(sg + base + i0);
            m4[0] = mv.x; m4[NE - 1] = mv.y;
            s4[0] = sv.x; s4[NE - 1] = sv.y;
        } else {
#pragma unroll
            for (int k = 0; k < NE; ++k) {
                const bool ok = i0 + k < n_per_ch;
                m4[k] = ok ? mu[base + i0 + k] : 0.0f;
                s4[k] = ok ? sg[base + i0 + k] : 1.0f;
            }
        }
        float du[NE][N1];
#pragma unroll
        for (int k = 0; k < NE; ++k) hull_du_nearest<N>(tbb, m4[k], s4[k], du[k]);
        uint64_t fix[NE];
#pragma unroll
        for (int k = 0; k < NE; ++k) {
            const bool valid = i0 + k < n_per_ch;
            my_valid += valid ? 1u : 0u;
            const unsigned int vinc = valid ? inc : 0u;
            float Tn[N];
            sweep_thresholds<N>(du[k], Tn);
            fix[k] = __builtin_amdgcn_ballot_w64(!(sweep_max_du<N>(du[k]) < kSweepBig)) | (force_slow ? ~0ull : 0ull);
#pragma unroll
            for (int n = 0; n < N; ++n) {
                float4 nb;
                const uint32_t a = sweep_position<16>(Tn[n], key0, nkeys, lut, rec, nb);
                const float G = sweep_band(Tn[n], n, du[k][n]);
                const float dist = sweep_distance(Tn[n], nb);
                fix[k] |= __builtin_amdgcn_ballot_w64(dist <= G);
                atomicAdd(&H[((uint32_t)n * LB + a) * (unsigned)KC + copy], vinc);
            }
            fix[k] &= __builtin_amdgcn_ballot_w64(valid);
        }
        uint64_t any_fix = 0;
#pragma unroll
        for (int k = 0; k < NE; ++k) any_fix |= fix[k];
        if (any_fix != 0 && !never_flag) {
#pragma unroll
            for (int k = 0; k < NE; ++k) {
                const bool mine = (fix[k] >> lane) & 1ull;
                unsigned int slot = kFixQueue;
                if (mine) slot = atomicAdd(&fixn, 1u);
                if (mine && slot < (unsigned)kFixQueue) fixq[slot] = ((unsigned int)it << 9) | (threadIdx.x << 1) | (unsigned)k;
                const uint64_t now = __builtin_amdgcn_ballot_w64(mine && slot >= (unsigned)kFixQueue);
                if (now != 0ull)
                    hull_counts_fix<N>(now, du[k], tb, m4[k], s4[k], L, key0, nkeys, perm_s, lut, rec, penl, corr, force_slow);
            }
        }
    }
    __syncthreads();
    {
        const unsigned int nq = fixn < (unsigned)kFixQueue ? fixn : (unsigned)kFixQueue;
        for (unsigned int i = threadIdx.x; i < ((nq + 63u) & ~63u); i += blockDim.x) {
            const bool on = i < nq;
            const unsigned int e = on ? fixq[i] : 0u;
            const long qq = q0 + (long)(e >> 9) * qstep + (long)((e >> 1) & 255u) - (long)threadIdx.x;
            const long el = qq * NE + (long)(e & 1u);
            const long at = (vec_ok & 2) ? el * C + c : base + el;
            const float z = on ? mu[at] : 0.0f, sgm = on ? sg[at] : 1.0f;
            float du[N1];
            hull_du_nearest<N>(tbb, z, sgm, du);
            const uint64_t lanes = __builtin_amdgcn_ballot_w64(on);
            hull_counts_fix<N>(lanes, du, tb, z, sgm, L, key0, nkeys, perm_s, lut, rec, penl, corr, force_slow);
        }
    }
    atomicAdd(&n_valid, my_valid);
    __syncthreads();
    unsigned int *hs = reinterpret_cast<unsigned int *>(penl);
    static_assert(N * LB <= kMaxLambdaChunk * PS, "hs must fit the penalty staging area");
    for (int i = threadIdx.x; i < N * LB; i += blockDim.x) {
        unsigned int v = 0;
#pragma unroll
        for (int j = 0; j < KC; ++j) {
            const unsigned int w = H[i * KC + j];
            v += (w & 0xffffu) + (w >> 16);
        }
        hs[i] = v;
    }
    __syncthreads();
    if (threadIdx.x < N) {
        unsigned int run = 0;
        for (int a = LB - 1; a >= 0; --a) { run += hs[threadIdx.x * LB + a]; hs[threadIdx.x * LB + a] = run; }
    }
    __syncthreads();
    for (int i = threadIdx.x; i < L * N1; i += blockDim.x) {
        const int l = i / N1, n = i - l * N1;
        const long hi_cnt = n == 0 ? (long)n_valid : (long)hs[(n - 1) * LB + l + 1];
        const long lo_cnt = n == N ? 0 : (long)hs[n * LB + l + 1];
        const long v = hi_cnt - lo_cnt + corr[i];
        if (v) atomicAdd(&level_counts[((long)sw.perm[l] * C + c) * N1 + n], (unsigned long long)v);
    }
}


#ifndef VBQ_K1E_STAGE
#define VBQ_K1E_STAGE 5
#endif
#ifndef VBQ_K1E_WAVES
#define VBQ_K1E_WAVES 4
#endif
template <int N, int LFIX, bool BUF>
__global__ void __launch_bounds__(256, VBQ_K1E_WAVES)
k_quant_hull_idx(const float *__restrict__ mu, const float *__restrict__ sg, long n_per_ch, long ch_stride, int C,
                 const float *__restrict__ table, Lambdas32 lam, HullSweep sw, int vec_ok,
                 uint16_t *__restrict__ out_idx, long E, int dbg) {
    constexpr int T = table_size(N);
    constexpr int N1 = N + 1;
    constexpr int NE = 2;
    constexpr int PS = (N1 + 3) & ~3;
    constexpr int CW = 5;
    struct Lds {
        unsigned short rk[N1 * NE * 256];
        float tb[T + 1];
        float penl[kMaxLambdaChunk * PS];
        unsigned char lut[kHullKeys];
        float4 rec[34];
        unsigned char perm_s[32];
        unsigned int cnt[CW * NE * 256];
    };
    __shared__ __align__(16) Lds lds;
    unsigned short *rk = lds.rk;
    float *tb = lds.tb, *penl = lds.penl;
    unsigned char *lut = lds.lut, *perm_s = lds.perm_s;
    float4 *rec = lds.rec;
    unsigned int *cnt = lds.cnt;
    const int c = blockIdx.y;
    const int L = LFIX ? LFIX : sw.L;
    const unsigned int tid = threadIdx.x;
    for (int i = tid; i < T; i += blockDim.x) tb[i] = table[(long)c * T + i];
    for (int i = tid; i < L * PS; i += blockDim.x) {
        const int l = i / PS, n = i - l * PS;
        penl[i] = n < N1 ? __fmul_rn(lam.lam[l], (float)n) : 0.0f;
    }
    stage_sweep_lut(lut, sw.lut);
    if (tid < 34) {
        const int i = (int)tid;
        auto at = [&](int l) { return l < 0 ? -kSweepBig : (l < L ? sw.val[l < 32 ? l : 31] : kSweepBig); };
        rec[i] = make_float4(at(i - 1), at(i), at(i + 1), 0.0f);
    }
    if (tid < 32) perm_s[tid] = sw.perm[tid];
    for (int i = tid; i < CW * NE * 256; i += blockDim.x) cnt[i] = 0;
    __syncthreads();

    const bool force_slow = dbg == 1, never_flag = dbg == 2;
    const uint32_t all_l = L >= 32 ? 0xffffffffu : ((1u << L) - 1u);
    const long base = (long)c * ch_stride;
    const long npairs = (n_per_ch + NE - 1) / NE;
    const char *tbb = reinterpret_cast<const char *>(tb);
    const unsigned int lane = tid & 63u;

    const __amdgpu_buffer_rsrc_t orsrc = __builtin_amdgcn_make_buffer_rsrc(out_idx, 0, -1 , 0x00020000);
    const uint32_t plane_bytes = (uint32_t)(2 * E);
    unsigned int rot = wave_slot();
    for (long q = (long)blockIdx.x * blockDim.x + tid; q < npairs; q += (long)gridDim.x * blockDim.x) {
        rotate_issue_priority(rot);
        const long i0 = q * NE;
        const bool full = (vec_ok & 1) && (i0 + NE <= n_per_ch);
        float m4[NE], s4[NE];
        if (vec_ok & 2) {
#pragma unroll
            for (int k = 0; k < NE; ++k) {
                const bool ok = i0 + k < n_per_ch;
                m4[k] = ok ? mu[(i0 + k) * C + c] : 0.0f;
                s4[k] = ok ? sg[(i0 + k) * C + c] : 1.0f;
            }
        } else if (full) {
            const float2 mv = *reinterpret_cast<const float2 *>(mu + base + i0);
            const float2 sv = *reinterpret_cast<const float2 *>(sg + base + i0);
            m4[0] = mv.x; m4[1] = mv.y;
            s4[0] = sv.x; s4[1] = sv.y;
        } else {
#pragma unroll
            for (int k = 0; k < NE; ++k) {
                const bool ok = i0 + k < n_per_ch;
                m4[k] = ok ? mu[base + i0 + k] : 0.0f;
                s4[k] = ok ? sg[base + i0 + k] : 1.0f;
            }
        }
        float du[NE][N1];
        uint32_t tiny[NE] = {0, 0};
        {
            uint32_t g[NE] = {0, 0};
            double rinv[NE];
#pragma unroll
            for (int k = 0; k < NE; ++k) rinv[k] = __ddiv_rn(1.0, (double)s4[k]);
#pragma unroll
            for (int n = 0; n <= N; ++n) {
                const int off4 = 4 * ((1 << n) - 1);
                const int top4 = off4;
#pragma unroll
                for (int k = 0; k < NE; ++k) {
                    const float pj = *reinterpret_cast<const float *>(tbb + off4 + g[k]);
                    const bool below = pj < m4[k];
                    float dL, dR;
                    uint32_t lo4, hi4;
                    if (n == 0) {
                        dL = dR = dist_cost(pj, m4[k], rinv[k]);
                        lo4 = hi4 = 0;
                    } else {
                        const uint32_t G4 = g[k] + (below ? 4u : 0u);
                        int lo = (int)G4 - 4;
                        lo = lo < 0 ? 0 : lo;
                        if (n == N) lo = lo > top4 - 4 ? top4 - 4 : lo;
                        lo4 = (uint32_t)lo;
                        hi4 = G4 > (uint32_t)top4 ? (uint32_t)top4 : G4;
                        dL = dist_cost(*reinterpret_cast<const float *>(tbb + off4 + lo4), m4[k], rinv[k]);
                        dR = dist_cost(*reinterpret_cast<const float *>(tbb + off4 + hi4), m4[k], rinv[k]);
                    }
                    const bool r_better = dR < dL;
                    du[k][n] = r_better ? dR : dL;
                    g[k] = 2 * g[k] + (below ? 4u : 0u);
                    const uint32_t b4 = r_better ? hi4 : lo4;
                    const uint32_t better = n < N ? (b4 << (N - n - 1)) + ((1u << (N - n)) - 1u) : (b4 >> 1);
                    rk[(((N - n) * 256 + tid) * NE) + k] = (unsigned short)better;
                    if (n >= 1) {
                        const float bound = __fmul_rn(fmaf((float)n, du[k][n - 1], du[k][n]), 1.9073486328125e-06f);
                        tiny[k] |= (r_better && !(__fsub_rn(dL, dR) > bound)) ? (1u << n) : 0u;
                    }
                }
            }
        }
        uint32_t flags[NE];
#pragma unroll
        for (int k = 0; k < NE; ++k) {
            const bool valid = i0 + k < n_per_ch;
            float Pm[N1], Tn[N];
            uint64_t near[N];
            float big = du[k][0];
#pragma unroll
            for (int j = 1; j + 1 < N1; j += 2) big = vmax3(big, du[k][j], du[k][j + 1]);
            if ((N1 & 1) == 0) big = vmax(big, du[k][N1 - 1]);
            uint32_t fl = (!(big < kSweepBig) || force_slow) ? 0xffffffffu : 0u;
            uint64_t any_near = 0;
#pragma unroll
            for (int n = 0; n < N; ++n) {
#pragma unroll
                for (int j = n + 1; j < N1; ++j) {
                    const float r = __fmul_rn(__fsub_rn(du[k][n], du[k][j]), 1.0f / (float)(j - n));
                    Pm[j] = n == 0 ? r : vmin(Pm[j], r);
                }
                float t = Pm[n + 1];
                {
                    int j = n + 2;
// ... 238 lines not shown
        double rinv[NE];
        float S[NE][LL];
        uint32_t win[NE][LL];
        uint64_t multi[NE][LL];
#pragma unroll
        for (int k = 0; k < NE; ++k) {
            g[k] = 0;
            rinv[k] = __ddiv_rn(1.0, (double)s4[k]);
#pragma unroll
            for (int l = 0; l < LL; ++l) { S[k][l] = 0.0f; win[k][l] = 0; multi[k][l] = 0; }
        }
        uint32_t opq = 0;
        asm volatile("" : "+v"(opq));
        const float *psv = reinterpret_cast<const float *>(&ps[0][0]) + opq;
#pragma unroll
        for (int n = 0; n <= N; ++n) {
            const int off4 = 4 * ((1 << n) - 1);
            const int top4 = off4;
            uint64_t active = 0;
            float pen[LL], stop[LL];
#pragma unroll
            for (int l = 0; l < LL; ++l) {
                pen[l] = psv[2 * (l * (N1 + 1) + n)];
                stop[l] = psv[2 * (l * (N1 + 1) + n + 1) + 1];
            }
#pragma unroll
            for (int k = 0; k < NE; ++k) {
                const float pj = *reinterpret_cast<const float *>(tbb + off4 + g[k]);
                const bool below = pj < m4[k];
                float dmin;
                if (n == 0) {
                    dmin = __fsub_rn(pj, m4[k]);
                } else {
                    int o4 = (int)g[k] + (below ? 4 : -4);
                    o4 = o4 < 0 ? 0 : (o4 > top4 ? top4 : o4);
                    const float po = *reinterpret_cast<const float *>(tbb + off4 + o4);
                    dmin = fminf(fabsf(__fsub_rn(pj, m4[k])), fabsf(__fsub_rn(po, m4[k])));
                }
                const float t = (float)__dmul_rn((double)dmin, rinv[k]);
                const float du = __fmul_rn(0.5f, __fmul_rn(t, t));
                const uint32_t here = g[k] | ((uint32_t)n << 16);
#pragma unroll
                for (int l = 0; l < LL; ++l) {
                    const float cst = __fadd_rn(du, pen[l]);
                    if (n == 0) {
                        S[k][l] = cst;
                        win[k][l] = here;
                    } else {
                        const bool lt = cst < S[k][l];
                        const uint64_t eq = __builtin_amdgcn_ballot_w64(cst == S[k][l]);
                        multi[k][l] = (multi[k][l] & ~__builtin_amdgcn_ballot_w64(lt)) | eq;
                        S[k][l] = lt ? cst : S[k][l];
                        win[k][l] = lt ? here : win[k][l];
                    }
                    if (n < N) active |= __builtin_amdgcn_ballot_w64(!(S[k][l] < stop[l]));
                }
                g[k] = 2 * g[k] + (below ? 4u : 0u);
            }
            if (n < N && active == 0 && n >= 1) break;
        }
        uint32_t rank[LL][NE];
#pragma unroll
        for (int k = 0; k < NE; ++k)
#pragma unroll
            for (int l = 0; l < LL; ++l) {
                const uint32_t n = win[k][l] >> 16;
                const uint32_t gj = win[k][l] & 0xffffu;
                const uint32_t off4 = 4u * ((1u << n) - 1u), top4 = off4;
                const float pj = *reinterpret_cast<const float *>(tbb + off4 + gj);
                const bool below = pj < m4[k];
                const uint32_t G4 = gj + (below ? 4u : 0u);
                uint32_t lo4 = G4 >= 4u ? G4 - 4u : 0u;
                if (n == (uint32_t)N) lo4 = lo4 > top4 - 4u ? top4 - 4u : lo4;
                const uint32_t hi4 = G4 > top4 ? top4 : G4;
                const float pen = psv[2 * (l * (N1 + 1) + n)];
                const float cL = __fadd_rn(dist_cost(*reinterpret_cast<const float *>(tbb + off4 + lo4), m4[k], rinv[k]), pen);
                const float cR = __fadd_rn(dist_cost(*reinterpret_cast<const float *>(tbb + off4 + hi4), m4[k], rinv[k]), pen);
                const uint32_t b4 = (n >= 1u && cR < cL) ? hi4 : lo4;
                rank[l][k] = (((b4 >> 1) + 1u) << ((uint32_t)N - n)) - 1u;
            }
        uint64_t any_multi = force_slow ? ~0ull : 0ull;
#pragma unroll
        for (int k = 0; k < NE; ++k)
#pragma unroll
            for (int l = 0; l < LL; ++l) any_multi |= multi[k][l];
        if (any_multi != 0) {
#pragma unroll
            for (int k = 0; k < NE; ++k)
#pragma unroll
                for (int l = 0; l < LL; ++l)
                    if (((multi[k][l] >> lane) & 1ull) || force_slow) rank[l][k] = exact_rank_scan<N>(tb, m4[k], s4[k], prow[l]);
        }
#pragma unroll
        for (int l = 0; l < LL; ++l) {
            uint16_t *o = out_idx + (long)l * E + base + i0;
            if (full) {
                *reinterpret_cast<uint32_t *>(o) = rank[l][0] | (rank[l][1] << 16);
            } else {
#pragma unroll
                for (int k = 0; k < NE; ++k)
                    if (i0 + k < n_per_ch) o[k] = (uint16_t)rank[l][k];
            }
        }
    }
}

}

void quant_fast_grid(int64_t n_per_ch, int32_t n_ch, int wg_per_cu, int reserved, bool counting, int64_t *out_gx, bool *out_resident) {
    const int64_t nquads = (n_per_ch + kFastNE - 1) / kFastNE;
    int64_t gx = (nquads + kFastThreads - 1) / kFastThreads;
    const bool explicit_wgs = wg_per_cu >= 1 && wg_per_cu <= 5;
    const int fit = kFastNE == 4 ? 3 : 4;
    const bool dynamic_grid = !explicit_wgs && reserved > 0 &&
                              (resident_slots(fit, reserved) / n_ch) * n_ch * 10 < (int64_t)num_cus() * fit * 9;
    const int per_cu = explicit_wgs ? (wg_per_cu < fit ? wg_per_cu : fit) : (dynamic_grid ? 5 : fit);
    int64_t cap = (dynamic_grid ? (int64_t)num_cus() * per_cu * 4 : resident_slots(per_cu, reserved)) / n_ch;
    const bool resident = !dynamic_grid && (int64_t)n_ch <= (int64_t)num_cus() * per_cu;
    if (cap < 1) cap = 1;
    if (gx > cap) {
        const int64_t iters = gx;
        if (resident) {
            const int64_t rounds_needed = (iters + cap - 1) / cap;
            gx = (iters + rounds_needed - 1) / rounds_needed;
        } else {
            int64_t best = cap, best_pad = ((iters + cap - 1) / cap) * cap - iters;
            for (int64_t g = cap - 1; g >= (cap + 1) / 2 && best_pad > 0; --g) {
                const int64_t pad = ((iters + g - 1) / g) * g - iters;
                if (pad * best < best_pad * g) { best = g; best_pad = pad; }
            }
            gx = best;
        }
        constexpr int64_t max_iters = 65000 / ((64 / 32) * (kFastThreads / 64) * kFastNE);
        if (counting && (iters + gx - 1) / gx > max_iters) gx = (iters + max_iters - 1) / max_iters;
    }
    if (gx < 1) gx = 1;
    *out_gx = gx;
    *out_resident = resident;
}

template <int N>
int launch_quant_fast(const float *mu, const float *sg, int64_t n_per_ch, int64_t ch_stride, int32_t n_ch, const float *table,
                      const Lambdas32 &lam, const float *len, int32_t L, uint16_t *out_idx, float *out_zhat,
                      float *out_bits, int64_t E, int vec_ok,
                      unsigned long long *level_counts, int wg_per_cu, int reserved, hipStream_t st) {
    int64_t gx = 1;
    bool resident = false;
    quant_fast_grid(n_per_ch, n_ch, wg_per_cu, reserved, level_counts != nullptr, &gx, &resident);
    if (resident) vec_ok |= 4;
    const dim3 grid((unsigned)gx, (unsigned)n_ch), block(kFastThreads);
    const int dbg = fast_debug();
    if (level_counts)
        hipLaunchKernelGGL((k_quant_fast<N, 2>), grid, block, 0, st, mu, sg, (long)n_per_ch, (long)ch_stride, (int)n_ch, table,
                           lam, len, (int)L, out_idx, out_zhat, out_bits, (long)E, vec_ok, dbg, level_counts);
    else if (out_zhat || out_bits)
        hipLaunchKernelGGL((k_quant_fast<N, 1>), grid, block, 0, st, mu, sg, (long)n_per_ch, (long)ch_stride, (int)n_ch, table,
                           lam, len, (int)L, out_idx, out_zhat, out_bits, (long)E, vec_ok, dbg, level_counts);
    else
        hipLaunchKernelGGL((k_quant_fast<N, 0>), grid, block, 0, st, mu, sg, (long)n_per_ch, (long)ch_stride, (int)n_ch, table,
                           lam, len, (int)L, out_idx, out_zhat, out_bits, (long)E, vec_ok, dbg, level_counts);
    VBQ_CHECK_LAUNCH("quant_fast");
    return VBQ_OK;
}

template <int N>
int launch_quant_pruned(const float *mu, const float *sg, int64_t n_per_ch, int64_t ch_stride, int32_t n_ch, const float *table,
                        const Lambdas32 &lam, const float *len, int32_t L, uint16_t *out_idx, int64_t E, int vec_ok, hipStream_t st) {
    if (L < 1 || L > kPrunedMaxL) return 1;
    const int64_t npairs = (n_per_ch + 1) / 2;
    int64_t gx = (npairs + 255) / 256;
    int64_t cap = (int64_t)num_cus() * 4 / n_ch;
    if (cap < 1) cap = 1;
    if (gx > cap) gx = cap;
    const int dbg = fast_debug();
    const dim3 grid((unsigned)gx, (unsigned)n_ch), block(256);
#define VBQ_PRUNED_CASE(LLv)                                                                                          \
    case LLv:                                                                                                          \
        hipLaunchKernelGGL((k_quant_pruned<N, LLv>), grid, block, 0, st, mu, sg, (long)n_per_ch, (long)ch_stride, (int)n_ch, \
                           table, lam, len, out_idx, (long)E, vec_ok, dbg);                                            \
        break;
    switch (L) {
        VBQ_PRUNED_CASE(1) VBQ_PRUNED_CASE(2) VBQ_PRUNED_CASE(3) VBQ_PRUNED_CASE(4)
        default: return 1;
    }
#undef VBQ_PRUNED_CASE
    VBQ_CHECK_LAUNCH("quant_pruned");
    return VBQ_OK;
}


static bool build_lambda_sweep(const double *lam, int L, HullSweep &sw) {
    float v[32];
    for (int i = 0; i < L && i < 32; ++i) v[i] = (float)lam[i];
    return build_sweep_table<16>(v, L, 1.9e-12f, 1.8e19f, sw);
}

int64_t level_counts_hull_grid(int64_t n_per_ch, int32_t n_ch, int reserved) {
    const int64_t nquads = (n_per_ch + VBQ_HULL_NE - 1) / VBQ_HULL_NE;
    int64_t gx = (nquads + kHullThreads - 1) / kHullThreads;
    constexpr int per_cu = VBQ_HULL_WAVES * 256 / kHullThreads;
    constexpr int rounds = 1;
    int64_t slots = resident_slots(per_cu, reserved);
    if (reserved > 0 && (slots / n_ch) * n_ch * 10 < (int64_t)num_cus() * per_cu * 9)
        slots = (int64_t)num_cus() * (per_cu > 1 ? per_cu - 1 : 1);
    int64_t cap = slots * rounds / n_ch;
    if (cap < 1) cap = 1;
    if (gx > cap) {
        const int64_t iters = gx;
        const int64_t rounds_needed = (iters + cap - 1) / cap;
        gx = (iters + rounds_needed - 1) / rounds_needed;
        const int64_t max_iters = 65000 / ((32 / VBQ_HULL_COPIES) * (kHullThreads / 64) * VBQ_HULL_NE);
        if ((iters + gx - 1) / gx > max_iters) gx = (iters + max_iters - 1) / max_iters;
    }
    return gx < 1 ? 1 : gx;
}

int launch_level_counts_hull10(const float *mu, const float *sg, int64_t n_per_ch, int64_t ch_stride, int32_t n_ch,
                               const float *table, const double *lam, int32_t L, int vec_ok,
                               unsigned long long *level_counts, int reserved, hipStream_t st) {
    if (L < 1 || L > 32) return 1;
    HullSweep sw;
    if (!build_lambda_sweep(lam, L, sw)) return 1;
    const int64_t gx = level_counts_hull_grid(n_per_ch, n_ch, reserved);
    const int dbg = fast_debug();
    Lambdas32 l32;
    for (int i = 0; i < kMaxLambdaChunk; ++i) l32.lam[i] = i < L ? (float)lam[i] : 0.0f;
    hipLaunchKernelGGL((k_level_counts_hull<10>), dim3((unsigned)gx, (unsigned)n_ch), dim3(kHullThreads), 0, st, mu, sg,
                       (long)n_per_ch, (long)ch_stride, (int)n_ch, table, l32, sw, vec_ok, level_counts, dbg);
    VBQ_CHECK_LAUNCH("level_counts_hull");
    return VBQ_OK;
}

int launch_quant_hull_idx10(const float *mu, const float *sg, int64_t n_per_ch, int64_t ch_stride, int32_t n_ch,
                            const float *table, const double *lam, int32_t L, int vec_ok, uint16_t *out_idx, int64_t E,
                            hipStream_t st) {
    if (L < 16) return 1;
    if (2 * (uint64_t)E > 0xffffffffull) return 1;
    HullSweep sw;
    if (!build_lambda_sweep(lam, L, sw)) return 1;
    const int64_t npairs = (n_per_ch + 1) / 2;
    int64_t gx = (npairs + 255) / 256;
    constexpr int rounds = 2;
    int64_t cap = (int64_t)num_cus() * VBQ_K1E_WAVES * rounds / n_ch;
    if (cap < 1) cap = 1;
    if (gx > cap) gx = cap;
    const int dbg = fast_debug();
    Lambdas32 l32;
    for (int i = 0; i < kMaxLambdaChunk; ++i) l32.lam[i] = i < L ? (float)lam[i] : 0.0f;
    const bool buf = (uint64_t)L * 2ull * (uint64_t)E <= 0xffffffffull;
#define VBQ_K1E_LAUNCH(LF, BF)                                                                                                \
    hipLaunchKernelGGL((k_quant_hull_idx<10, LF, BF>), dim3((unsigned)gx, (unsigned)n_ch), dim3(256), 0, st, mu, sg,          \
                       (long)n_per_ch, (long)ch_stride, (int)n_ch, table, l32, sw, vec_ok, out_idx, (long)E, dbg)
    if (L == 32) { if (buf) VBQ_K1E_LAUNCH(32, true); else VBQ_K1E_LAUNCH(32, false); }
    else if (L == 16) { if (buf) VBQ_K1E_LAUNCH(16, true); else VBQ_K1E_LAUNCH(16, false); }
    else VBQ_K1E_LAUNCH(0, false);
#undef VBQ_K1E_LAUNCH
    VBQ_CHECK_LAUNCH("quant_hull_idx");
    return VBQ_OK;
}

#define VBQ_INST_FAST(NN)                                                                                              \
    template int launch_quant_fast<NN>(const float *, const float *, int64_t, int64_t, int32_t, const float *,        \
                                       const Lambdas32 &, const float *, int32_t, uint16_t *, float *, float *, int64_t, \
                                       int, unsigned long long *, int, int, hipStream_t);
VBQ_FOR_EACH_N(VBQ_INST_FAST)
#undef VBQ_INST_FAST
#define VBQ_INST_PRUNED(NN)                                                                                           \
    template int launch_quant_pruned<NN>(const float *, const float *, int64_t, int64_t, int32_t, const float *,     \
                                         const Lambdas32 &, const float *, int32_t, uint16_t *, int64_t, int, hipStream_t);
VBQ_FOR_EACH_N(VBQ_INST_PRUNED)
#undef VBQ_INST_PRUNED

}

extern "C" int vbq_solve_grid(int32_t kernel, int64_t n_rows, int32_t n_ch, int32_t workgroups_per_cu, int32_t reserved_workgroups,
                              int64_t *h_grid) {
    using namespace vbq;
    VBQ_REQUIRE(h_grid && n_rows >= 1 && n_ch >= 1 && n_ch <= 65535, VBQ_ERR_INVALID_ARGUMENT, "vbq_solve_grid: bad sizes or null pointer");
    VBQ_REQUIRE(kernel == VBQ_GRID_K1 || kernel == VBQ_GRID_K1T, VBQ_ERR_INVALID_ARGUMENT, "vbq_solve_grid: unknown kernel %d", kernel);
    VBQ_REQUIRE(workgroups_per_cu >= 0 && workgroups_per_cu <= 5, VBQ_ERR_INVALID_ARGUMENT, "vbq_solve_grid: workgroups_per_cu=%d not in 0..5",
                workgroups_per_cu);
    const int reserved = reserved_workgroups < 0 ? 0 : reserved_workgroups;
    if (kernel == VBQ_GRID_K1) {
        int64_t gx = 1;
        bool resident = false;
        quant_fast_grid(n_rows, n_ch, workgroups_per_cu, reserved, false, &gx, &resident);
        h_grid[0] = gx;
        h_grid[2] = resident ? 1 : 0;
    } else {
        h_grid[0] = level_counts_hull_grid(n_rows, n_ch, reserved);
        h_grid[2] = 1;
    }
    h_grid[1] = n_ch;
    return VBQ_OK;
}
```

### vbq_amd/ops.py

```python
from __future__ import annotations

import ctypes as C
from typing import Optional, Sequence

import numpy as np
import torch

from . import _lib
from ._lib import LAYOUT_BC, LAYOUT_BC_TO_CB, LAYOUT_CB, MODE_F32, MODE_F64_SCORE, VBQError, check
from .tables import table_size

_LAYOUTS = {"bc": LAYOUT_BC, "cb": LAYOUT_CB, LAYOUT_BC: LAYOUT_BC, LAYOUT_CB: LAYOUT_CB}
_MODES = {"f32": MODE_F32, "f64": MODE_F64_SCORE, MODE_F32: MODE_F32, MODE_F64_SCORE: MODE_F64_SCORE}


_raw_stream = getattr(torch._C, "_cuda_getCurrentRawStream", None)


def raw_stream(device: torch.device) -> int:
    if _raw_stream is not None:
        return _raw_stream(device.index if device.index is not None else torch.cuda.current_device())
    return torch.cuda.current_stream(device).cuda_stream


# ... 20 lines not shown
                       "(there is no CPU implementation in this package)")
    if t.dtype != dtype:
        raise ValueError(f"{name}: expected dtype {dtype}, got {t.dtype}")
    return t.contiguous()


def _ptr(t: Optional[torch.Tensor]):
    return C.c_void_p(t.data_ptr()) if t is not None else None


def _doubles(vals: Sequence[float]):
    arr = (C.c_double * len(vals))(*[float(v) for v in vals])
    return arr


def _rows_channels(shape, layout):
    if len(shape) == 1:
        return shape[0], 1
    if len(shape) != 2:
        raise ValueError(f"expected a 1-D or 2-D tensor, got shape {tuple(shape)}")
    return (shape[0], shape[1]) if layout == LAYOUT_BC else (shape[1], shape[0])


def _pair(mu, sigma):
    mu = _dev(mu, torch.float32, "mu")
    sigma = _dev(sigma, torch.float32, "sigma")
    if mu.shape != sigma.shape:
        raise ValueError(f"mu {tuple(mu.shape)} and sigma {tuple(sigma.shape)} differ in shape")
    return mu, sigma


def _pair_bc(means_bc, spread_bc):
    means_bc = _dev(means_bc, torch.float32, "means")
    spread_bc = _dev(spread_bc, torch.float32, "spread")
    if means_bc.dim() != 2 or means_bc.shape != spread_bc.shape:
        raise ValueError(f"expected two [rows, C] tensors, got {tuple(means_bc.shape)} / {tuple(spread_bc.shape)}")
    return means_bc, spread_bc


def _table(t, Cc, T, name):
    t = _dev(t, torch.float32, name)
    if t.numel() != Cc * T:
        raise ValueError(f"{name} has {t.numel()} entries, expected C*T = {Cc}*{T}")
    return t


def _per_lambda(t, shape, name):
    t = _dev(t, torch.float32, name)
    if tuple(t.shape) != shape:
        raise ValueError(f"{name} shape {tuple(t.shape)} != {shape}")
    return t


def _workspace(given, nbytes, device, floor=0):
    ws = given if given is not None else torch.empty(max(nbytes, floor), dtype=torch.uint8, device=device)
    if ws.numel() * ws.element_size() < nbytes or not ws.is_cuda:
        raise ValueError(f"workspace must be a device tensor of at least {nbytes} bytes")
    return ws


def _out(given, shape, dtype, device, name, want=True):
    if given is not None:
        if tuple(given.shape) != shape or given.dtype != dtype or not given.is_cuda or not given.is_contiguous():
            raise ValueError(f"{name}: expected a contiguous {dtype} device tensor of shape {shape}")
        return given
    return torch.empty(shape, dtype=dtype, device=device) if want else None


def _solve_inputs(mu, sigma, table_lm, lambdas, N, level_len, layout):
    mu, sigma = _pair(mu, sigma)
    rows, Cc = _rows_channels(mu.shape, layout)
    table_lm = _table(table_lm, Cc, table_size(N), "table_lm")
    L = len(lambdas)
    if L < 1:
        raise ValueError("need at least one lambda")
    if level_len is not None:
        level_len = _per_lambda(level_len, (L, Cc, N + 1), "level_len")
    return mu, sigma, rows, Cc, table_lm, L, level_len


def quantize(mu: torch.Tensor, sigma: torch.Tensor, table_lm: torch.Tensor, lambdas: Sequence[float], *,
             N: int = 10, level_len: Optional[torch.Tensor] = None, layout="bc", mode="f32",
             want_zhat: bool = False, want_bits: bool = False, out_idx: Optional[torch.Tensor] = None,
             out_zhat: Optional[torch.Tensor] = None, out_bits: Optional[torch.Tensor] = None,
             workspace: Optional[torch.Tensor] = None, rows: Optional[Sequence[int]] = None,
             workgroups_per_cu: int = 0, reserved_workgroups: Optional[int] = None):
    to_planes = layout in ("bc->cb", LAYOUT_BC_TO_CB)
    layout = LAYOUT_BC if to_planes else _LAYOUTS[layout]
    mode = _MODES[mode]
    rows_range = rows
    mu, sigma, rows, Cc, table_lm, L, level_len = _solve_inputs(mu, sigma, table_lm, lambdas, N, level_len, layout)
    h = _lib.lib()
    if to_planes and mu.dim() == 2 and Cc > 1:
        layout, oshape = LAYOUT_BC_TO_CB, (L, Cc, rows)
    else:
        oshape = (L,) + tuple(mu.shape)
    idx = _out(out_idx, oshape, torch.uint16, mu.device, "out_idx")
    zhat = _out(out_zhat, oshape, torch.float32, mu.device, "out_zhat", want_zhat)
    bits = _out(out_bits, oshape, torch.float32, mu.device, "out_bits", want_bits)
    want_zhat, want_bits = zhat is not None, bits is not None
    wsb = h.vbq_quantize_workspace_bytes(Cc, L, N)
    ws = _workspace(workspace, wsb, mu.device)
    if mu.numel() == 0:
        out = (idx,) + ((zhat,) if want_zhat else ()) + ((bits,) if want_bits else ())
        return out if len(out) > 1 else idx
    if rows_range is None and not workgroups_per_cu and reserved_workgroups is None:
        check(h.vbq_quantize_f32(_ptr(mu), _ptr(sigma), rows, Cc, layout, _ptr(table_lm), _ptr(level_len),
                                 _doubles(lambdas), L, N, mode, _ptr(idx), _ptr(zhat), _ptr(bits), _ptr(ws), wsb,
                                 _stream(mu)), "vbq_quantize_f32")
    else:
        r0, r1 = (0, rows) if rows_range is None else (int(rows_range[0]), int(rows_range[1]))
        check(h.vbq_quantize_rows_f32(_ptr(mu), _ptr(sigma), rows, Cc, layout, _ptr(table_lm), _ptr(level_len),
                                      _doubles(lambdas), L, N, mode, _ptr(idx), _ptr(zhat), _ptr(bits), _ptr(ws), wsb,
                                      r0, r1, int(workgroups_per_cu), -1 if reserved_workgroups is None else int(reserved_workgroups),
                                      _stream(mu)), "vbq_quantize_rows_f32")
    out = (idx,)
    if want_zhat:
        out += (zhat,)
    if want_bits:
        out += (bits,)
    return out if len(out) > 1 else idx


def check_inputs(mu: torch.Tensor, sigma: torch.Tensor):
    mu, sigma = _pair(mu, sigma)
    bad = torch.zeros(2, dtype=torch.uint32, device=mu.device)
    check(_lib.lib().vbq_check_inputs_f32(_ptr(mu), _ptr(sigma), mu.numel(), _ptr(bad), _stream(mu)), "vbq_check_inputs_f32")
    b = bad.cpu().numpy()
    if b[0] or b[1]:
        raise ValueError(f"invalid latents: {int(b[0])} non-finite means, {int(b[1])} standard deviations that are not finite and positive")


def level_counts(mu: torch.Tensor, sigma: torch.Tensor, table_lm: torch.Tensor, lambdas: Sequence[float], *,
                 N: int = 10, level_len: Optional[torch.Tensor] = None, layout="bc", out: Optional[torch.Tensor] = None,
                 workspace: Optional[torch.Tensor] = None, reserved_workgroups: Optional[int] = None):
    to_planes = layout in ("bc->cb", LAYOUT_BC_TO_CB)
    layout = LAYOUT_BC if to_planes else _LAYOUTS[layout]
    mu, sigma, rows, Cc, table_lm, L, level_len = _solve_inputs(mu, sigma, table_lm, lambdas, N, level_len, layout)
    if to_planes and mu.dim() == 2 and Cc > 1:
        layout = LAYOUT_BC_TO_CB
    if out is None:
        out = torch.zeros((L, Cc, N + 1), dtype=torch.int64, device=mu.device)
    else:
        _out(out, (L, Cc, N + 1), torch.int64, mu.device, "out")
    h = _lib.lib()
    wsb = h.vbq_quantize_workspace_bytes(Cc, L, N)
    ws = _workspace(workspace, wsb, mu.device)
    if mu.numel():
        check(h.vbq_level_counts_f32(_ptr(mu), _ptr(sigma), rows, Cc, layout, _ptr(table_lm), _ptr(level_len),
                                     _doubles(lambdas), L, N, _ptr(out), _ptr(ws), wsb,
                                     -1 if reserved_workgroups is None else int(reserved_workgroups), _stream(mu)),
              "vbq_level_counts_f32")
    return out


def code_lengths_from_counts(counts: torch.Tensor, lut: torch.Tensor, *, level_period: int = 0, want_len: bool = True,
                             want_model: bool = False, out_len: Optional[torch.Tensor] = None,
                             out_model: Optional[torch.Tensor] = None):
    if counts.dtype not in (torch.int64, torch.int32):
        raise ValueError("counts must be int64 or int32")
    counts = _dev(counts, counts.dtype, "counts")
    lut = _dev(lut, torch.float32, "lut")
    out_len = _out(out_len, tuple(counts.shape), torch.float32, counts.device, "out_len", want_len)
    out_model = _out(out_model, tuple(counts.shape), torch.float32, counts.device, "out_model", want_model)
    check(_lib.lib().vbq_code_lengths_from_counts(_ptr(counts), int(counts.dtype == torch.int32), counts.numel(), _ptr(lut),
                                                  lut.numel(), int(level_period), _ptr(out_len), _ptr(out_model),
                                                  _stream(counts)), "vbq_code_lengths_from_counts")
    if out_len is not None and out_model is not None:
        return out_len, out_model
    return out_len if out_len is not None else out_model


def quantize_notebook(means: torch.Tensor, stds: torch.Tensor, codebook_lm: torch.Tensor, betas: Sequence[float], *,
                      N: int = 10, want_values: bool = True, out_idx: Optional[torch.Tensor] = None):
    means = _dev(means, torch.float32, "means")
    stds = _dev(stds, torch.float32, "stds")
    if means.shape != stds.shape:
        raise ValueError("means and stds differ in shape")
    codebook_lm = _dev(codebook_lm, torch.float64, "codebook_lm")
    if codebook_lm.numel() != table_size(N):
        raise ValueError(f"codebook has {codebook_lm.numel()} entries, expected {table_size(N)}")
    nb = len(betas)
    n = means.numel()
    idx = _out(out_idx, (nb,) + tuple(means.shape), torch.uint16, means.device, "out_idx")
    val = torch.empty((nb,) + tuple(means.shape), dtype=torch.float32, device=means.device) if want_values else None
    check(_lib.lib().vbq_quantize_notebook_f64(_ptr(means), _ptr(stds), n, _ptr(codebook_lm), _doubles(betas), nb, N,
                                               _ptr(idx), _ptr(val), _stream(means)), "vbq_quantize_notebook_f64")
    return idx, val


def histogram(idx: torch.Tensor, n_ch: int, *, N: int = 10, layout="bc", out: Optional[torch.Tensor] = None,
              dtype=torch.int64, rows: Optional[Sequence[int]] = None):
    layout = _LAYOUTS[layout]
    rows_range = rows
    idx = _dev(idx, torch.uint16, "idx")
    L = idx.shape[0]
    E = idx[0].numel()
    if E % n_ch:
        raise ValueError(f"{E} indices per lambda is not a multiple of n_ch={n_ch}")
    rows = E // n_ch
    T = table_size(N)
    if out is None:
        out = torch.zeros((L, n_ch, T), dtype=dtype, device=idx.device)
    else:
        if out.dtype not in (torch.int64, torch.int32):
            raise ValueError("out must be int64 or int32")
        if not out.is_contiguous():
            raise ValueError("out must be contiguous (counts are accumulated in place)")
        out = _out(_dev(out, out.dtype, "out"), (L, n_ch, T), out.dtype, idx.device, "out")
    h = _lib.lib()
    if rows_range is not None:
        check(h.vbq_histogram_rows_u16(_ptr(idx), rows, n_ch, layout, L, N, _ptr(out), int(out.dtype == torch.int32),
                                       int(rows_range[0]), int(rows_range[1]), _stream(idx)), "vbq_histogram_rows_u16")
        return out
    fn, name = (h.vbq_histogram_u16, "vbq_histogram_u16") if out.dtype == torch.int64 else \
               (h.vbq_histogram_u16_i32, "vbq_histogram_u16_i32")
    check(fn(_ptr(idx), rows, n_ch, layout, L, N, _ptr(out), _stream(idx)), name)
    return out


def histogram_models(idx: torch.Tensor, n_ch: int, counts: torch.Tensor, *, N: int = 10, lut: Optional[torch.Tensor] = None,
                     models: Optional[torch.Tensor] = None):
    idx = _dev(idx, torch.uint16, "idx")
    if idx.dim() != 3 or idx.shape[1] != n_ch:
        raise ValueError(f"idx must be planes [L, {n_ch}, rows], got {tuple(idx.shape)}")
    L, _, rows = idx.shape
    T = table_size(N)
    if counts.dtype not in (torch.int64, torch.int32):
        raise ValueError(f"counts: expected a contiguous int32 / int64 device tensor of shape {(L, n_ch, T)}")
    _out(counts, (L, n_ch, T), counts.dtype, idx.device, "counts")
    if (lut is None) != (models is None):
        raise ValueError("lut and models go together")
    if models is not None:
        lut = _dev(lut, torch.float32, "lut")
        _out(models, (L, n_ch, T), torch.float32, idx.device, "models")
    check(_lib.lib().vbq_histogram_models_u16(_ptr(idx), rows, n_ch, L, N, _ptr(counts), int(counts.dtype == torch.int32), _ptr(lut),
                                              lut.numel() if lut is not None else 0, _ptr(models), _stream(idx)),
          "vbq_histogram_models_u16")
    return counts, models


def index_max(idx: torch.Tensor) -> int:
    idx = _dev(idx, torch.uint16, "idx")
    m = torch.zeros(1, dtype=torch.uint32, device=idx.device)
    check(_lib.lib().vbq_index_max_u16(_ptr(idx), idx.numel(), _ptr(m), _stream(idx)), "vbq_index_max_u16")
    return int(m.cpu().item())


def moments(x: torch.Tensor, *, layout="bc", out: Optional[torch.Tensor] = None):
    layout = _LAYOUTS[layout]
    x = _dev(x, torch.float32, "x")
    rows, Cc = _rows_channels(x.shape, layout)
    if out is None:
        out = torch.zeros((Cc, 2), dtype=torch.float64, device=x.device)
    check(_lib.lib().vbq_moments_f32(_ptr(x), rows, Cc, layout, _ptr(out), _stream(x)), "vbq_moments_f32")
    return out


def numpy_sum_sq(x: torch.Tensor) -> torch.Tensor:
    x = _dev(x, torch.float32, "x").reshape(-1)
    if x.data_ptr() % 16:
        x = x.clone()
    out = torch.zeros(1, dtype=torch.float32, device=x.device)
    h = _lib.lib()
    wsb = h.vbq_numpy_sum_sq_workspace_bytes(x.numel())
    ws = torch.empty(max(wsb, 4), dtype=torch.uint8, device=x.device)
    check(h.vbq_numpy_sum_sq_f32(_ptr(x), x.numel(), _ptr(out), _ptr(ws), wsb, _stream(x)), "vbq_numpy_sum_sq_f32")
    return out


def unit_to_u8(x: torch.Tensor) -> torch.Tensor:
    x = _dev(x, torch.float32, "x")
    out = torch.empty(x.shape, dtype=torch.uint8, device=x.device)
    check(_lib.lib().vbq_unit_to_u8_f32(_ptr(x), x.numel(), _ptr(out), _stream(x)), "vbq_unit_to_u8_f32")
    return out


def numpy_row_sums(x: torch.Tensor, workspace: Optional[torch.Tensor] = None) -> torch.Tensor:
    x = _dev(x, torch.float32, "x")
    rows = x.shape[0]
    n = x[0].numel() if rows else 0
    out = torch.empty(rows, dtype=torch.float32, device=x.device)
    h = _lib.lib()
    wsb = h.vbq_numpy_row_sums_workspace_bytes(rows, n)
    ws = workspace if workspace is not None and workspace.numel() * workspace.element_size() >= wsb else \
        torch.empty(max(wsb, 4), dtype=torch.uint8, device=x.device)
    check(h.vbq_numpy_row_sums_f32(_ptr(x), rows, n, _ptr(out), _ptr(ws), wsb, _stream(x)), "vbq_numpy_row_sums_f32")
    return out


def gather(idx: torch.Tensor, tab: torch.Tensor, n_ch: int, *, N: int = 10, layout="bc", out_layout=None):
    layout = _LAYOUTS[layout]
    out_layout = layout if out_layout is None else _LAYOUTS[out_layout]
    idx = _dev(idx, torch.uint16, "idx")
    tab = _dev(tab, torch.float32, "tab")
    L = idx.shape[0]
    E = idx[0].numel()
    rows = E // n_ch
    T = table_size(N)
    per_lambda = tab.dim() == 3
    if tuple(tab.shape) != ((L, n_ch, T) if per_lambda else (n_ch, T)):
        raise ValueError(f"tab shape {tuple(tab.shape)} does not match (L={L}, C={n_ch}, T={T})")
    oshape = tuple(idx.shape)
    if out_layout != layout and idx.dim() == 3 and n_ch == 1:
        oshape = (L, idx.shape[2], idx.shape[1])
    if out_layout != layout and n_ch > 1:
# ... 535 lines not shown
```

### vbq_amd/pipeline.py

```python
from __future__ import annotations

from typing import Optional, Sequence

import numpy as np
import torch

import ctypes as _C
import glob as _glob
import os as _os

from . import entropy as _entropy
from . import ops
from ._lib import VBQError

_HIP = None


def _hip_runtime():
    global _HIP
    if _HIP is None:
        cands = _glob.glob(_os.path.join(_os.path.dirname(torch.__file__), "lib", "libamdhip64.so*")) + ["libamdhip64.so"]
        for c in cands:
            try:
                _HIP = _C.CDLL(c)
# ... 78 lines not shown
    global _LOG2_LOOP
    if _LOG2_LOOP is None:
        _LOG2_LOOP = False
        try:
            if not _ufunc_struct_is_readable():
                return None
            u = _PyUFuncObject.from_address(id(np.log2))
            NPY_FLOAT = 11
            if u.nin == 1 and u.nout == 1 and u.nargs == 2 and 0 < u.ntypes < 64 and u.functions and u.types and u.name == b"log2":
                for i in range(u.ntypes):
                    if ord(u.types[2 * i]) == NPY_FLOAT and ord(u.types[2 * i + 1]) == NPY_FLOAT and u.functions[i]:
                        cand = (int(u.functions[i]), int((u.data[i] if u.data else 0) or 0))
                        rng = np.random.default_rng(7)
                        ok = True
                        for K, dt, sm in ((11, np.int64, 1), (2047, np.int32, 1), (257, np.int64, 0.5)):
                            cnt = rng.gamma(0.3, 4e7 / K, (5, K)).astype(dt)
                            got = np.empty((5, K), np.float32)
                            rc = ops._lib.lib().vbq_host_neg_log2_freq_f32(cnt.ctypes.data, int(dt == np.int32), 5, K, float(sm), 0,
                                                                          cand[0], cand[1], got.ctypes.data, None)
                            ok = ok and rc == 0 and np.array_equal(got, _entropy.neg_log2_freq(cnt, sm))
                        if ok:
                            _LOG2_LOOP = cand
                        break
        except Exception:
            _LOG2_LOOP = False
    return _LOG2_LOOP or None


class NativeHostStage:

    def __init__(self, counts: torch.Tensor, out_model: torch.Tensor, out_len: Optional[torch.Tensor], add_n_smoothing, loop):
        self.counts, self.out_model, self.out_len = counts, out_model, out_len
        self.h_in = torch.empty(counts.shape, dtype=counts.dtype, pin_memory=True)
        self.h_model = torch.empty(counts.shape, dtype=torch.float32, pin_memory=True)
        self.h_len = torch.empty(counts.shape, dtype=torch.float32, pin_memory=True) if out_len is not None else None
        K = counts.shape[-1]
        d = self.desc = ops._lib.HostStageDesc()
        d.h_counts, d.counts_are_i32, d.add_level = self.h_in.data_ptr(), int(counts.dtype == torch.int32), int(out_len is not None)
        d.n_rows, d.K, d.add_n_smoothing, d.status, d.runs = counts.numel() // K, K, float(add_n_smoothing), 0, 0
        d.log2_loop, d.log2_data = loop
        d.h_out_model, d.h_out_len = self.h_model.data_ptr(), (self.h_len.data_ptr() if self.h_len is not None else None)
        self._fn = _C.cast(ops._lib.lib().vbq_host_stage_run, _C.c_void_p)
        self.error = None

    def enqueue(self):
        st = torch.cuda.current_stream(self.counts.device)
        self.h_in.copy_(self.counts, non_blocking=True)
        rc = _hip_runtime().hipLaunchHostFunc(_C.c_void_p(st.cuda_stream), self._fn, _C.byref(self.desc))
        if rc != 0:
            raise VBQError(f"hipLaunchHostFunc failed ({rc})")
        self.out_model.copy_(self.h_model, non_blocking=True)
        if self.out_len is not None:
            self.out_len.copy_(self.h_len, non_blocking=True)

    def check(self):
        if self.desc.status != 0:
            rc, self.desc.status = self.desc.status, 0
            raise VBQError(f"host stage failed: vbq_host_neg_log2_freq_f32 returned {rc}")


def chunk_bounds(rows: int, n_chunks: int, unit: int = 2048):
    if n_chunks <= 1 or rows < 2 * unit:
        return [(0, rows)]
    units = rows // unit
    n_chunks = min(n_chunks, units)
    base, rem = divmod(units, n_chunks)
    cuts, r = [0], 0
    for j in range(n_chunks):
        r += (base + (1 if j < rem else 0)) * unit
        cuts.append(r)
    cuts[-1] = rows
    return list(zip(cuts[:-1], cuts[1:]))


class EntropyModelBuild:

    def __init__(self, rows: int, n_ch: int, lambdas: Sequence[float], table_lm: torch.Tensor, *, N: int = 10,
                 add_n_smoothing=1, global_rows: Optional[int] = None, distributed: bool = False, group=None,
                 level_group=None, n_chunks: Optional[int] = None, counts_dtype=None, keep_models: bool = True,
                 buffers: Optional[dict] = None, reserved_workgroups: Optional[int] = None, python_host_stage: bool = False):
        self.rows, self.C, self.N = int(rows), int(n_ch), int(N)
        self.lambdas = [float(l) for l in lambdas]
        self.L = len(self.lambdas)
        self.T = ops.table_size(N)
        self.table = table_lm
        self.dev = table_lm.device
        self.smooth = add_n_smoothing
        self.group = group
        self.level_group = level_group if level_group is not None else group
        self.world = torch.distributed.get_world_size(group) if distributed else 1
        if distributed and self.world > 1 and global_rows is None:
            raise ValueError("EntropyModelBuild(distributed=True) needs global_rows = the number of rows summed over all ranks")
        self.global_rows = int(global_rows if global_rows is not None else rows)
        L, C, N1, T = self.L, self.C, N + 1, self.T
        if counts_dtype is None:
            counts_dtype = torch.int32 if self.global_rows < 2 ** 31 else torch.int64
        buf = buffers if buffers is not None else {}

        def kept(key, make):
            t = buf.get(key)
            if t is None:
                if len(buf) > 16:
                    buf.clear()
                t = buf[key] = make()
            return t
        self._kept = kept
        self._idx = None
        self.level_counts = torch.empty((L, C, N1), dtype=torch.int64, device=self.dev)
        self._counts2 = [torch.empty((L, C, T), dtype=counts_dtype, device=self.dev) for _ in range(2 if self.world > 1 else 1)]
        self._slot = 0
        self.counts = self._counts2[0]
        self.ws = kept(("ws", L, C, N, str(self.dev)),
                       lambda: torch.empty(ops._lib.lib().vbq_quantize_workspace_bytes(C, L, N), dtype=torch.uint8, device=self.dev))

        def lut(K, max_entries):
            def make():
                h = _entropy.neg_log2_lut(self.global_rows, K, add_n_smoothing, max_entries=max_entries)
                return (torch.from_numpy(h).to(self.dev) if h is not None else None,)
            return kept(("lut", self.global_rows, K, repr(add_n_smoothing), max_entries, str(self.dev)), make)[0]
        self.lut1 = lut(N1, max(1 << 20, 4 * L * C * N1))
        self.lut2 = lut(T, max(1 << 20, L * C * T)) if keep_models else None
        self.level_len = torch.empty((L, C, N1), dtype=torch.float32, device=self.dev)
        self.raw_models = torch.empty((L, C, N1), dtype=torch.float32, device=self.dev)
        self.models = torch.empty((L, C, T), dtype=torch.float32, device=self.dev) \
            if keep_models and (self.lut2 is not None or L * C * T <= (1 << 22)) else None
        smooth = add_n_smoothing
        lv = np.arange(N1, dtype=np.int32).astype(np.float32)

        def lengths_host(level_counts):
            raw = _entropy.neg_log2_freq(level_counts, smooth)
            return (lv + raw).astype(np.float32), raw

        loop = None
        if type(add_n_smoothing) in (int, float) and T <= 8192 and not python_host_stage:
            loop = numpy_log2_f32_loop()
        self.host_stage_kind = None
        self._len_stage = None
        if self.lut1 is None:
            self._len_stage = NativeHostStage(self.level_counts, self.raw_models, self.level_len, add_n_smoothing, loop) if loop else \
                HostStage([self.level_counts], [self.level_len, self.raw_models], lengths_host)
            self.host_stage_kind = "native" if loop else "python"
        self._model_stages = None
        if self.lut2 is None and self.models is not None:
            self._model_stages = [NativeHostStage(c, self.models, None, add_n_smoothing, loop) if loop else
                                  HostStage([c], [self.models], lambda counts: _entropy.neg_log2_freq(counts, smooth))
                                  for c in self._counts2]
            self.host_stage_kind = "native" if loop else "python"
        if n_chunks is None:
            n_chunks = 1
        self.chunks = chunk_bounds(self.rows, n_chunks)
        self.k1_workgroups_per_cu = 3
        self.side = torch.cuda.Stream(device=self.dev) if len(self.chunks) > 1 else None
        self._events = [torch.cuda.Event() for _ in self.chunks] if self.side is not None else []
        self.reducers = [None, None]
        self.works = [None, None]
        self._models_pending = [False, False]
        self.timers = None
        self.collectives = True
        if self.world > 1 and counts_dtype == torch.int32:
            from .dist import CountsAllReduce
            self.reducers = [CountsAllReduce(L * C * T, self.dev, max_global_count=self.global_rows, group=group) for _ in range(2)]
        if reserved_workgroups is None:
            payload = 0
            if self.world > 1:
                r = self.reducers[0]
                payload = r.payload_bytes(self.counts) if r is not None else self.counts.numel() * self.counts.element_size()
            reserved_workgroups = 64 if payload >= (4 << 20) else 0
        self.reserved_workgroups = int(reserved_workgroups)

    @property
    def idx(self) -> torch.Tensor:
        if self._idx is None:
            L, C = self.L, self.C
            self._idx = self._kept(("idx", L, C, self.rows, str(self.dev)),
                                   lambda: torch.empty((L, C, self.rows), dtype=torch.uint16, device=self.dev))
        return self._idx

    @property
    def one_call_ok(self) -> bool:
        return (self.world == 1 and self.side is None and self.lut1 is not None and
                (self.models is None or self.lut2 is not None) and self.timers is None)

    def run_one_call(self, means_bc: torch.Tensor, spread_bc: torch.Tensor, spread: str = "sigma"):
        if not self.one_call_ok:
            raise VBQError("run_one_call: this build needs the staged form (sharded, chunked, timed, or a -log2 step that is not tabulated)")
        means_bc = ops._dev(means_bc, torch.float32, "means")
        spread_bc = ops._dev(spread_bc, torch.float32, "spread")
        if tuple(means_bc.shape) != (self.rows, self.C) or means_bc.shape != spread_bc.shape:
            raise ValueError(f"expected two [{self.rows}, {self.C}] tensors, got {tuple(means_bc.shape)} / {tuple(spread_bc.shape)}")
        h = ops._lib.lib()
        wsb = h.vbq_build_entropy_models_workspace_bytes(self.rows, self.C, self.L, self.N)
        ws = self._kept(("ws_build", self.L, self.C, self.rows, self.N, str(self.dev)),
                        lambda: torch.empty(max(wsb, 256), dtype=torch.uint8, device=self.dev))
        fused = self.models is not None
        ops._lib.check(h.vbq_build_entropy_models_f32(
            ops._ptr(means_bc), ops._ptr(spread_bc), ops._spread_kind(spread), self.rows, self.C, ops._ptr(self.table),
            ops._doubles(self.lambdas), self.L, self.N, ops._ptr(self.lut1), self.lut1.numel(),
            ops._ptr(self.lut2) if fused else None, self.lut2.numel() if fused else 0, ops._ptr(self.level_counts),
            ops._ptr(self.level_len), ops._ptr(self.raw_models), ops._ptr(self.counts), int(self.counts.dtype == torch.int32),
            ops._ptr(self.models) if fused else None, ops._ptr(ws), ws.numel(), self._reserved(), ops._stream(means_bc)),
            "vbq_build_entropy_models_f32")
        self._models_current = fused
        return self

    def _reserved(self) -> int:
        return self.reserved_workgroups if self.collectives else 0

    def pass1(self, mu_cb, sg_cb, level_len=None):
        self.level_counts.zero_()
        self._t("k1h", 0)
        ops.level_counts(mu_cb, sg_cb, self.table, self.lambdas, N=self.N, level_len=level_len, layout="cb",
                         out=self.level_counts, workspace=self.ws, reserved_workgroups=self._reserved())
        self._t("k1h", 1)
        if self.world > 1 and self.collectives:
            torch.distributed.all_reduce(self.level_counts, group=self.level_group)
        return self.level_counts

    def _t(self, name, phase):
        if self.timers is not None:
            self.timers(name, phase)

    def lengths(self):
        if self.lut1 is not None:
            ops.code_lengths_from_counts(self.level_counts, self.lut1, level_period=self.N + 1, out_len=self.level_len,
                                         out_model=self.raw_models)
        else:
            self._len_stage.enqueue()
        return self.level_len, self.raw_models

    def pass2(self, mu_cb, sg_cb, level_len):
        if self.world > 1:
            self._slot ^= 1
            self.counts = self._counts2[self._slot]
        self.wait(self._slot)
        main = torch.cuda.current_stream(self.dev)
        self._models_current = False
        if self.side is None and self.world == 1:
            fused = self.lut2 is not None and self.models is not None
            self._t("k1", 0)
            ops.quantize(mu_cb, sg_cb, self.table, self.lambdas, N=self.N, level_len=level_len, layout="cb",
                         out_idx=self.idx, workspace=self.ws, reserved_workgroups=self._reserved())
            self._t("k1", 1)
            self._t("k2", 0)
            ops.histogram_models(self.idx, self.C, self.counts, N=self.N, lut=self.lut2 if fused else None,
                                 models=self.models if fused else None)
            self._t("k2", 1)
            self._models_current = fused
            return self.idx, self.counts
        self.counts.zero_()
        if self.side is None:
            self._t("k1", 0)
            ops.quantize(mu_cb, sg_cb, self.table, self.lambdas, N=self.N, level_len=level_len, layout="cb",
                         out_idx=self.idx, workspace=self.ws, reserved_workgroups=self._reserved())
            self._t("k1", 1)
            self._t("k2", 0)
            ops.histogram(self.idx, self.C, N=self.N, layout="cb", out=self.counts)
            self._t("k2", 1)
        else:
            self.side.wait_stream(main)
            for j, (r0, r1) in enumerate(self.chunks):
                self._t("k1", 0)
                ops.quantize(mu_cb, sg_cb, self.table, self.lambdas, N=self.N, level_len=level_len, layout="cb",
                             out_idx=self.idx, workspace=self.ws, rows=(r0, r1), workgroups_per_cu=self.k1_workgroups_per_cu,
                             reserved_workgroups=self._reserved())
                self._t("k1", 1)
                self._events[j].record(main)
                with torch.cuda.stream(self.side):
                    self.side.wait_event(self._events[j])
                    self._t("k2", 0)
                    ops.histogram(self.idx, self.C, N=self.N, layout="cb", out=self.counts, rows=(r0, r1))
                    self._t("k2", 1)
            main.wait_stream(self.side)
        if self.world > 1 and self.collectives:
            if self.reducers[self._slot] is not None:
                self.works[self._slot] = self.reducers[self._slot].start(self.counts)
            else:
                self.works[self._slot] = torch.distributed.all_reduce(self.counts, group=self.group, async_op=True)
        return self.idx, self.counts

    @property
    def reducer(self):
        return self.reducers[self._slot]

    def wait(self, slot=None):
        for s in ((0, 1) if slot is None else (slot,)):
            if self.works[s] is not None:
                self.works[s].wait()
                self.works[s] = None

    def _models_from(self, slot):
        self.wait(slot)
        counts = self._counts2[slot]
        if self.lut2 is None:
            self._model_stages[slot].enqueue()
        else:
            ops.code_lengths_from_counts(counts, self.lut2, want_len=False, out_model=self.models)
        self._models_pending[slot] = False

    def finish_models(self):
        self.wait(self._slot)
        if self.models is None:
            return None
        if getattr(self, "_models_current", False):
            return self.models
        self._models_from(self._slot)
        self._models_current = True
        return self.models

    @property
    def has_host_stages(self) -> bool:
        return self._len_stage is not None or bool(self._model_stages)

    @property
    def graph_safe(self) -> bool:
        return self.world == 1 and self.side is None

    @property
    def length_table_route(self) -> str:
        return "device (tabulated -log2)" if self.lut1 is not None else \
            f"stream-ordered host stage ({self._stage_text()} on [L, C, N+1] counts, hipLaunchHostFunc; no synchronisation)"

    @property
    def models_route(self) -> str:
        if self.models is None:
            return "not in the step (counts stay on the device)"
        return "device (tabulated -log2)" if self.lut2 is not None else \
            f"stream-ordered host stage ({self._stage_text()} on [L, C, T] counts, hipLaunchHostFunc; no synchronisation)"

    def _stage_text(self) -> str:
        return "plain C with NumPy's float32 log2 loop, no interpreter lock" if self.host_stage_kind == "native" else \
            "NumPy float32 -log2 in Python"

    def check(self):
        self.wait()
        for st in [self._len_stage] + list(self._model_stages or []):
            if st is not None:
                torch.cuda.synchronize(self.dev)
                st.check()
        if self.collectives or self.world == 1:
            sums = self.level_counts.sum(dim=-1)
            if not bool(torch.all(sums == self.global_rows)):
                raise VBQError(f"bit-length histogram rows hold {int(sums.min())}..{int(sums.max())} samples, not global_rows = "
                               f"{self.global_rows}: the tabulated code lengths of this build are invalid")
            sums = self.counts.sum(dim=-1, dtype=torch.int64)
            if not bool(torch.all(sums == self.global_rows)):
                raise VBQError(f"rank histogram rows hold {int(sums.min())}..{int(sums.max())} samples, not global_rows = "
                               f"{self.global_rows}: the tabulated models of this build are invalid")
        for r in self.reducers:
            if r is not None:
                r.check()

    def run(self, mu_cb, sg_cb, level_len=None, models: bool = True):
        self.pass1(mu_cb, sg_cb, level_len)
        ll, _ = self.lengths()
        self.pass2(mu_cb, sg_cb, ll)
        if models and self.models is not None:
            if self.world == 1:
                self.finish_models()
            else:
                prev = self._slot ^ 1
                if self._models_pending[prev]:
                    self._models_from(prev)
                self._models_pending[self._slot] = True
        return self
```

Baseline: 506.6 billion latents/s.

## Fuse pass-1 level-count reduction and code-length build into the pass-2 quantize kernel

Pass 1 now writes per-workgroup partial level-count tables into the workspace instead of reducing them globally with atomics. The pass-2 quantize kernel, in a new FROM_PARTIALS variant, sums those partials per channel, derives code lengths and raw models from a LUT, and then solves indices. This removes the separate memset, atomic reduction and code-length kernel launches between the passes. The cost is a larger workspace and redundant partial summation inside every pass-2 workgroup. It applies only on one GPU with N=10 and at most 32 lambdas.

```diff
diff --git a/include/vbq.h b/include/vbq.h
--- a/include/vbq.h
+++ b/include/vbq.h
@@ -68,6 +68,17 @@
 int vbq_code_lengths_from_counts(const void *d_counts, int32_t counts_are_i32, int64_t n,
                                  const float *d_lut, int64_t lut_n, int32_t level_period,
                                  float *d_out_len, float *d_out_model, void *stream);
+
+int vbq_level_partials_f32(const float *d_mu, const float *d_sigma, int64_t n_rows, int32_t n_ch, int32_t layout,
+                           const float *d_table_lm, const double *h_lambdas, int32_t n_lambda, int32_t N,
+                           void *d_workspace, size_t workspace_bytes, int32_t reserved_workgroups,
+                           int32_t *h_n_partials, void *stream);
+int vbq_quantize_from_partials_f32(const float *d_mu, const float *d_sigma, int64_t n_rows, int32_t n_ch, int32_t layout,
+                                   const float *d_table_lm, const double *h_lambdas, int32_t n_lambda, int32_t N,
+                                   int32_t n_partials, const float *d_lut_levels, int64_t n_lut_levels,
+                                   int64_t *d_level_counts, float *d_level_len, float *d_raw_models, uint16_t *d_out_idx,
+                                   void *d_workspace, size_t workspace_bytes, int32_t workgroups_per_cu,
+                                   int32_t reserved_workgroups, void *stream);
 
 typedef void (*vbq_f32_loop)(char **args, const intptr_t *dimensions, const intptr_t *steps, void *data);
 typedef struct vbq_host_stage {
diff --git a/vbq_amd/_lib.py b/vbq_amd/_lib.py
--- a/vbq_amd/_lib.py
+++ b/vbq_amd/_lib.py
@@ -37,6 +37,13 @@
                                        C.c_int32, C.c_void_p]),
     "vbq_code_lengths_from_counts": (C.c_int, [C.c_void_p, C.c_int32, C.c_int64, C.c_void_p, C.c_int64, C.c_int32,
                                                C.c_void_p, C.c_void_p, C.c_void_p]),
+    "vbq_level_partials_f32": (C.c_int, [C.c_void_p, C.c_void_p, C.c_int64, C.c_int32, C.c_int32, C.c_void_p,
+                                         C.POINTER(C.c_double), C.c_int32, C.c_int32, C.c_void_p, C.c_size_t, C.c_int32,
+                                         C.POINTER(C.c_int32), C.c_void_p]),
+    "vbq_quantize_from_partials_f32": (C.c_int, [C.c_void_p, C.c_void_p, C.c_int64, C.c_int32, C.c_int32, C.c_void_p,
+                                                 C.POINTER(C.c_double), C.c_int32, C.c_int32, C.c_int32, C.c_void_p, C.c_int64,
+                                                 C.c_void_p, C.c_void_p, C.c_void_p, C.c_void_p, C.c_void_p, C.c_size_t,
+                                                 C.c_int32, C.c_int32, C.c_void_p]),
     "vbq_host_neg_log2_freq_f32": (C.c_int, [C.c_void_p, C.c_int32, C.c_int64, C.c_int64, C.c_float, C.c_int32, C.c_void_p, C.c_void_p,
                                              C.c_void_p, C.c_void_p]),
     "vbq_host_stage_run": (None, [C.c_void_p]),
diff --git a/vbq_amd/csrc/vbq_common.h b/vbq_amd/csrc/vbq_common.h
--- a/vbq_amd/csrc/vbq_common.h
+++ b/vbq_amd/csrc/vbq_common.h
@@ -80,7 +80,23 @@
 
 int launch_level_counts_hull10(const float *mu, const float *sg, int64_t n_per_ch, int64_t ch_stride, int32_t n_ch,
                                const float *table, const double *lam, int32_t L, int vec_ok,
-                               unsigned long long *level_counts, int reserved, hipStream_t st);
+                               unsigned long long *level_counts, uint32_t *partials, int64_t partials_cap, int32_t *n_partials,
+                               int reserved, hipStream_t st);
+
+int64_t level_counts_hull_resident_grid(int32_t n_ch);
+
+struct Pass1Partials {
+    const uint32_t *partials;
+    int n_partials;
+    const float *lut;
+    long lut_n;
+    long long *level_counts;
+    float *level_len;
+    float *raw_models;
+};
+int launch_quant_fast_p1(const float *mu, const float *sg, int64_t n_per_ch, int64_t ch_stride, int32_t n_ch, const float *table,
+                         const Lambdas32 &lam, int32_t L, uint16_t *out_idx, int64_t E, int vec_ok, const Pass1Partials &p1,
+                         int wg_per_cu, int reserved, hipStream_t st);
 
 int launch_quant_hull_idx10(const float *mu, const float *sg, int64_t n_per_ch, int64_t ch_stride, int32_t n_ch,
                             const float *table, const double *lam, int32_t L, int vec_ok, uint16_t *out_idx, int64_t E,
diff --git a/vbq_amd/csrc/vbq_latents.hip b/vbq_amd/csrc/vbq_latents.hip
--- a/vbq_amd/csrc/vbq_latents.hip
+++ b/vbq_amd/csrc/vbq_latents.hip
@@ -494,6 +494,17 @@
     hipStream_t st = reinterpret_cast<hipStream_t>(stream);
     int rc = vbq_prep_planes_f32(d_means_bc, d_spread_bc, spread_kind, n_rows, n_ch, mu_cb, sg_cb, stream);
     if (rc != VBQ_OK) return rc;
+    int32_t n_partials = 0;
+    rc = vbq_level_partials_f32(mu_cb, sg_cb, n_rows, n_ch, VBQ_LAYOUT_CB, d_table_lm, h_lambdas, n_lambda, N, w, qws, reserved_workgroups,
+                                &n_partials, stream);
+    if (rc != VBQ_OK) return rc;
+    if (n_partials > 0) {
+        rc = vbq_quantize_from_partials_f32(mu_cb, sg_cb, n_rows, n_ch, VBQ_LAYOUT_CB, d_table_lm, h_lambdas, n_lambda, N, n_partials,
+                                            d_lut_levels, n_lut_levels, d_level_counts, d_level_len, d_raw_models, idx, w, qws, 0,
+                                            reserved_workgroups, stream);
+        if (rc != VBQ_OK) return rc;
+        return vbq_histogram_models_u16(idx, n_rows, n_ch, n_lambda, N, d_counts, counts_are_i32, d_lut_ranks, n_lut_ranks, d_models, stream);
+    }
     hipError_t e = hipMemsetAsync(d_level_counts, 0, sizeof(int64_t) * (size_t)n_lambda * (size_t)n_ch * (size_t)N1, st);
     if (e != hipSuccess) {
         set_error("vbq_build_entropy_models_f32: hipMemsetAsync: %s", hipGetErrorString(e));
diff --git a/vbq_amd/csrc/vbq_quantize.hip b/vbq_amd/csrc/vbq_quantize.hip
--- a/vbq_amd/csrc/vbq_quantize.hip
+++ b/vbq_amd/csrc/vbq_quantize.hip
@@ -368,7 +368,7 @@
             if constexpr (sizeof(PenT) == 4 && N == 10) {
                 if (fast_ok && lc_out && !len_c) {
                     const int r = launch_level_counts_hull10(mu_r, sg_r, n_per_ch, ch_stride, n_ch, table, lc.lam, Lc,
-                                                             vec2_ok | (bc_to_cb ? 2 : 0), lc_out, reserved, st);
+                                                             vec2_ok | (bc_to_cb ? 2 : 0), lc_out, nullptr, 0, nullptr, reserved, st);
                     if (r == VBQ_OK) continue;
                     if (r < 0) return r;
                 }
@@ -445,10 +445,23 @@
 }
 }
 
+namespace vbq {
+namespace {
+size_t penalty_table_bytes(int32_t n_ch, int32_t n_lambda, int32_t N) {
+    const int Lc = n_lambda < kMaxLambdaChunk ? n_lambda : kMaxLambdaChunk;
+    return ((size_t)Lc * (size_t)n_ch * (size_t)(N + 1) * sizeof(double) + 256 + 255) & ~(size_t)255;
+}
+size_t partial_table_bytes(int32_t n_ch, int32_t n_lambda, int32_t N) {
+    const int Lc = n_lambda < kMaxLambdaChunk ? n_lambda : kMaxLambdaChunk;
+    return (size_t)Lc * (size_t)n_ch * (size_t)(N + 1) * sizeof(uint32_t);
+}
+}
+}
+
 extern "C" size_t vbq_quantize_workspace_bytes(int32_t n_ch, int32_t n_lambda, int32_t N) {
     if (n_ch <= 0 || n_lambda <= 0 || N < 0) return 0;
-    const int Lc = n_lambda < vbq::kMaxLambdaChunk ? n_lambda : vbq::kMaxLambdaChunk;
-    return (size_t)Lc * (size_t)n_ch * (size_t)(N + 1) * sizeof(double) + 256;
+    return vbq::penalty_table_bytes(n_ch, n_lambda, N) +
+           (size_t)vbq::level_counts_hull_resident_grid(n_ch) * vbq::partial_table_bytes(n_ch, n_lambda, N);
 }
 
 namespace vbq {
@@ -532,6 +545,86 @@
                           reinterpret_cast<unsigned long long *>(d_level_counts), 0, reserved_workgroups, stream);
 }
 
+namespace vbq {
+namespace {
+int partials_entry(const char *who, const float *d_mu, const float *d_sigma, int64_t n_rows, int32_t n_ch, int32_t layout,
+                   const float *d_table_lm, const double *h_lambdas, int32_t n_lambda, int32_t N, void *d_workspace,
+                   size_t workspace_bytes, uint32_t **partials, int64_t *cap) {
+    VBQ_REQUIRE(n_rows >= 1 && n_ch >= 1 && n_ch <= 65535 && n_lambda >= 1 && N >= 0, VBQ_ERR_INVALID_ARGUMENT,
+                "%s: bad sizes n_rows=%lld n_ch=%d n_lambda=%d N=%d", who, (long long)n_rows, n_ch, n_lambda, N);
+    VBQ_REQUIRE(d_mu && d_sigma && d_table_lm && h_lambdas, VBQ_ERR_INVALID_ARGUMENT, "%s: null pointer argument", who);
+    VBQ_REQUIRE(layout == VBQ_LAYOUT_CB || n_ch == 1, VBQ_ERR_UNSUPPORTED, "%s: channel-major planes (VBQ_LAYOUT_CB) or n_ch = 1 only", who);
+    const size_t need = vbq_quantize_workspace_bytes(n_ch, n_lambda, N);
+    VBQ_REQUIRE(d_workspace && workspace_bytes >= need, VBQ_ERR_WORKSPACE, "%s: workspace of %zu bytes given, %zu needed", who,
+                workspace_bytes, need);
+    VBQ_REQUIRE((reinterpret_cast<uintptr_t>(d_workspace) & 3) == 0, VBQ_ERR_INVALID_ARGUMENT, "%s: workspace must be 4-byte aligned", who);
+    const size_t off = penalty_table_bytes(n_ch, n_lambda, N);
+    *partials = reinterpret_cast<uint32_t *>(static_cast<char *>(d_workspace) + off);
+    *cap = (int64_t)((workspace_bytes - off) / partial_table_bytes(n_ch, n_lambda, N));
+    return VBQ_OK;
+}
+}
+}
+
+extern "C" int vbq_level_partials_f32(const float *d_mu, const float *d_sigma, int64_t n_rows, int32_t n_ch, int32_t layout,
+                                      const float *d_table_lm, const double *h_lambdas, int32_t n_lambda, int32_t N,
+                                      void *d_workspace, size_t workspace_bytes, int32_t reserved_workgroups,
+                                      int32_t *h_n_partials, void *stream) {
+    using namespace vbq;
+    VBQ_REQUIRE(h_n_partials, VBQ_ERR_INVALID_ARGUMENT, "vbq_level_partials_f32: null pointer argument");
+    *h_n_partials = 0;
+    uint32_t *partials = nullptr;
+    int64_t cap = 0;
+    if (const int r = partials_entry("vbq_level_partials_f32", d_mu, d_sigma, n_rows, n_ch, layout, d_table_lm, h_lambdas, n_lambda, N,
+                                     d_workspace, workspace_bytes, &partials, &cap); r != VBQ_OK) return r;
+    if (N != 10 || n_lambda > kMaxLambdaChunk) return VBQ_OK;
+    for (int i = 0; i < n_lambda; ++i)
+        if (!(h_lambdas[i] >= 1.9e-12 && h_lambdas[i] <= 1.8e19)) return VBQ_OK;
+    const int vec2_ok = ((reinterpret_cast<uintptr_t>(d_mu) | reinterpret_cast<uintptr_t>(d_sigma)) % 4 == 0) ? 1 : 0;
+    int32_t n = 0;
+    const int r = launch_level_counts_hull10(d_mu, d_sigma, n_rows, n_rows, n_ch, d_table_lm, h_lambdas, n_lambda, vec2_ok, nullptr,
+                                             partials, cap, &n, reserved_workgroups < 0 ? 0 : reserved_workgroups,
+                                             reinterpret_cast<hipStream_t>(stream));
+    if (r < 0) return r;
+    if (r == VBQ_OK) *h_n_partials = n;
+    return VBQ_OK;
+}
+
+extern "C" int vbq_quantize_from_partials_f32(const float *d_mu, const float *d_sigma, int64_t n_rows, int32_t n_ch, int32_t layout,
+                                              const float *d_table_lm, const double *h_lambdas, int32_t n_lambda, int32_t N,
+                                              int32_t n_partials, const float *d_lut_levels, int64_t n_lut_levels,
+                                              int64_t *d_level_counts, float *d_level_len, float *d_raw_models, uint16_t *d_out_idx,
+                                              void *d_workspace, size_t workspace_bytes, int32_t workgroups_per_cu,
+                                              int32_t reserved_workgroups, void *stream) {
+    using namespace vbq;
+    const char *who = "vbq_quantize_from_partials_f32";
+    uint32_t *partials = nullptr;
+    int64_t cap = 0;
+    if (const int r = partials_entry(who, d_mu, d_sigma, n_rows, n_ch, layout, d_table_lm, h_lambdas, n_lambda, N, d_workspace,
+                                     workspace_bytes, &partials, &cap); r != VBQ_OK) return r;
+    VBQ_REQUIRE(d_lut_levels && n_lut_levels >= 1 && d_level_counts && d_level_len && d_raw_models && d_out_idx, VBQ_ERR_INVALID_ARGUMENT,
+                "%s: null pointer argument or an empty table", who);
+    VBQ_REQUIRE(N == 10 && n_lambda <= kMaxLambdaChunk, VBQ_ERR_UNSUPPORTED, "%s: N = 10 and at most %d lambdas (what vbq_level_partials_f32 serves)",
+                who, kMaxLambdaChunk);
+    VBQ_REQUIRE(n_partials >= 1 && n_partials <= cap, VBQ_ERR_INVALID_ARGUMENT, "%s: n_partials=%d, the workspace holds %lld tables", who,
+                n_partials, (long long)cap);
+    VBQ_REQUIRE(workgroups_per_cu >= 0 && workgroups_per_cu <= 5, VBQ_ERR_INVALID_ARGUMENT, "%s: workgroups_per_cu=%d not in 0..5", who,
+                workgroups_per_cu);
+    Lambdas32 l32;
+    for (int i = 0; i < kMaxLambdaChunk; ++i) {
+        l32.lam[i] = i < n_lambda ? (float)h_lambdas[i] : 0.0f;
+        VBQ_REQUIRE(i >= n_lambda || (h_lambdas[i] >= 1.9e-12 && h_lambdas[i] <= 1.8e19), VBQ_ERR_UNSUPPORTED,
+                    "%s: lambda %g outside [1.9e-12, 1.8e19]", who, h_lambdas[i]);
+    }
+    const int vec2_ok = ((reinterpret_cast<uintptr_t>(d_mu) | reinterpret_cast<uintptr_t>(d_sigma)) % 4 == 0 &&
+                         reinterpret_cast<uintptr_t>(d_out_idx) % 2 == 0) ? 1 : 0;
+    const Pass1Partials p1 = {partials, n_partials, d_lut_levels, (long)n_lut_levels, reinterpret_cast<long long *>(d_level_counts),
+                              d_level_len, d_raw_models};
+    return launch_quant_fast_p1(d_mu, d_sigma, n_rows, n_rows, n_ch, d_table_lm, l32, n_lambda, d_out_idx, n_rows * (int64_t)n_ch, vec2_ok,
+                                p1, workgroups_per_cu, reserved_workgroups < 0 ? 0 : reserved_workgroups,
+                                reinterpret_cast<hipStream_t>(stream));
+}
+
 extern "C" int vbq_n_bit_intervals_f32(const float *d_z_cb, int64_t n_rows, int32_t n_ch, const float *d_table_lm, int32_t N,
                                        float *d_left, float *d_right, void *stream) {
     using namespace vbq;
diff --git a/vbq_amd/csrc/vbq_quantize_fast.hip b/vbq_amd/csrc/vbq_quantize_fast.hip
--- a/vbq_amd/csrc/vbq_quantize_fast.hip
+++ b/vbq_amd/csrc/vbq_quantize_fast.hip
@@ -108,13 +108,14 @@
     return (bestL <= bestR) ? rkL : rkR;
 }
 
-template <int N, int MODE>
+template <int N, int MODE, bool FROM_PARTIALS = false>
 __global__ void __launch_bounds__(kFastThreads, VBQ_FAST_WAVES)
 k_quant_fast(const float *__restrict__ mu, const float *__restrict__ sg, long n_per_ch, long ch_stride, int C,
              const float *__restrict__ table, Lambdas32 lam, const float *__restrict__ len,
              int L, uint16_t *__restrict__ out_idx, float *__restrict__ out_zhat,
              float *__restrict__ out_bits, long E, int vec_ok, int dbg,
-             unsigned long long *__restrict__ level_counts) {
+             unsigned long long *__restrict__ level_counts, Pass1Partials p1) {
+    static_assert(!FROM_PARTIALS || MODE == 0, "the partials feed the index solve only");
     constexpr int T = table_size(N);
     constexpr int N1 = N + 1;
     constexpr int NE = kFastNE;
@@ -129,13 +130,76 @@
     if (COUNT) {
         for (int i = threadIdx.x; i < N1 * NE * kFastThreads; i += blockDim.x) scratch[i] = 0;
     }
-    for (int i = threadIdx.x; i < T; i += blockDim.x) tb[i] = table[(long)c * T + i];
     int odd = 0;
-    for (int i = threadIdx.x; i < L * PS; i += blockDim.x) {
-        const int l = i / PS, n = i - l * PS;
-        const float p = n < N1 ? __fmul_rn(lam.lam[l], len ? len[((long)l * C + c) * N1 + n] : (float)n) : 0.0f;
-        penl[i] = p;
-        odd |= (len != nullptr && !(p == 0.0f || (p >= 1.8189894e-12f && p <= 1.1805916e21f))) ? 1 : 0;
+    if constexpr (FROM_PARTIALS) {
+        constexpr int R = (kMaxLambdaChunk * PS + kFastThreads - 1) / kFastThreads;
+        const long pstride = (long)L * C * N1;
+        bool on[R];
+        int ll[R], nn[R];
+        long at[R];
+        unsigned long long cnt[R];
+#pragma unroll
+        for (int r = 0; r < R; ++r) {
+            const int i = (int)threadIdx.x + r * kFastThreads;
+            nn[r] = i % PS;
+            on[r] = i < L * PS && nn[r] < N1;
+            ll[r] = on[r] ? i / PS : 0;
+            at[r] = on[r] ? ((long)ll[r] * C + c) * N1 + nn[r] : 0;
+            cnt[r] = 0;
+        }
+        auto load4 = [&](int j0, uint32_t (&v)[R][4]) {
+#pragma unroll
+            for (int r = 0; r < R; ++r)
+#pragma unroll
+                for (int k = 0; k < 4; ++k) {
+                    const int j = j0 + k < p1.n_partials ? j0 + k : p1.n_partials - 1;
+                    uint32_t keep = (on[r] && j0 + k < p1.n_partials) ? ~0u : 0u;
+                    asm volatile("" : "+v"(keep));
+                    v[r][k] = p1.partials[(long)j * pstride + at[r]] & keep;
+                }
+        };
+        auto add4 = [&](const uint32_t (&v)[R][4]) {
+#pragma unroll
+            for (int r = 0; r < R; ++r)
+#pragma unroll
+                for (int k = 0; k < 4; ++k) cnt[r] += v[r][k];
+        };
+        uint32_t first[R][4];
+        load4(0, first);
+        for (int i = threadIdx.x; i < T; i += blockDim.x) tb[i] = table[(long)c * T + i];
+        add4(first);
+        for (int j0 = 4; j0 < p1.n_partials; j0 += 4) {
+            uint32_t v[R][4];
+            load4(j0, v);
+            add4(v);
+        }
+        float m[R];
+#pragma unroll
+        for (int r = 0; r < R; ++r) {
+            const long k = (long)cnt[r] >= p1.lut_n ? p1.lut_n - 1 : (long)cnt[r];
+            m[r] = p1.lut[k];
+        }
+#pragma unroll
+        for (int r = 0; r < R; ++r) {
+            const int i = (int)threadIdx.x + r * kFastThreads;
+            const float ln = __fadd_rn((float)nn[r], m[r]);
+            const float p = on[r] ? __fmul_rn(lam.lam[ll[r]], ln) : 0.0f;
+            if (i < L * PS) penl[i] = p;
+            odd |= !(p == 0.0f || (p >= 1.8189894e-12f && p <= 1.1805916e21f)) ? 1 : 0;
+            if (on[r] && blockIdx.x == 0) {
+                p1.level_counts[at[r]] = (long long)cnt[r];
+                p1.level_len[at[r]] = ln;
+                p1.raw_models[at[r]] = m[r];
+            }
+        }
+    } else {
+        for (int i = threadIdx.x; i < T; i += blockDim.x) tb[i] = table[(long)c * T + i];
+        for (int i = threadIdx.x; i < L * PS; i += blockDim.x) {
+            const int l = i / PS, n = i - l * PS;
+            const float p = n < N1 ? __fmul_rn(lam.lam[l], len ? len[((long)l * C + c) * N1 + n] : (float)n) : 0.0f;
+            penl[i] = p;
+            odd |= (len != nullptr && !(p == 0.0f || (p >= 1.8189894e-12f && p <= 1.1805916e21f))) ? 1 : 0;
+        }
     }
     const bool force_slow = dbg == 1 || __syncthreads_or(odd) != 0;
 
@@ -483,7 +547,7 @@
 __global__ void __launch_bounds__(kHullThreads, (VBQ_HULL_WAVES * 256) / kHullThreads)
 k_level_counts_hull(const float *__restrict__ mu, const float *__restrict__ sg, long n_per_ch, long ch_stride, int C,
                     const float *__restrict__ table, Lambdas32 lam, HullSweep sw, int vec_ok,
-                    unsigned long long *__restrict__ level_counts, int dbg) {
+                    unsigned long long *__restrict__ level_counts, int dbg, uint32_t *__restrict__ partials) {
     constexpr int T = table_size(N);
     constexpr int N1 = N + 1;
     constexpr int NE = VBQ_HULL_NE;
@@ -635,7 +699,8 @@
         const long hi_cnt = n == 0 ? (long)n_valid : (long)hs[(n - 1) * LB + l + 1];
         const long lo_cnt = n == N ? 0 : (long)hs[n * LB + l + 1];
         const long v = hi_cnt - lo_cnt + corr[i];
-        if (v) atomicAdd(&level_counts[((long)sw.perm[l] * C + c) * N1 + n], (unsigned long long)v);
+        if (partials) partials[(((long)blockIdx.x * L + sw.perm[l]) * C + c) * N1 + n] = (uint32_t)v;
+        else if (v) atomicAdd(&level_counts[((long)sw.perm[l] * C + c) * N1 + n], (unsigned long long)v);
     }
 }
 
@@ -1180,14 +1245,28 @@
     const int dbg = fast_debug();
     if (level_counts)
         hipLaunchKernelGGL((k_quant_fast<N, 2>), grid, block, 0, st, mu, sg, (long)n_per_ch, (long)ch_stride, (int)n_ch, table,
-                           lam, len, (int)L, out_idx, out_zhat, out_bits, (long)E, vec_ok, dbg, level_counts);
+                           lam, len, (int)L, out_idx, out_zhat, out_bits, (long)E, vec_ok, dbg, level_counts, Pass1Partials{});
     else if (out_zhat || out_bits)
         hipLaunchKernelGGL((k_quant_fast<N, 1>), grid, block, 0, st, mu, sg, (long)n_per_ch, (long)ch_stride, (int)n_ch, table,
-                           lam, len, (int)L, out_idx, out_zhat, out_bits, (long)E, vec_ok, dbg, level_counts);
+                           lam, len, (int)L, out_idx, out_zhat, out_bits, (long)E, vec_ok, dbg, level_counts, Pass1Partials{});
     else
         hipLaunchKernelGGL((k_quant_fast<N, 0>), grid, block, 0, st, mu, sg, (long)n_per_ch, (long)ch_stride, (int)n_ch, table,
-                           lam, len, (int)L, out_idx, out_zhat, out_bits, (long)E, vec_ok, dbg, level_counts);
+                           lam, len, (int)L, out_idx, out_zhat, out_bits, (long)E, vec_ok, dbg, level_counts, Pass1Partials{});
     VBQ_CHECK_LAUNCH("quant_fast");
+    return VBQ_OK;
+}
+
+int launch_quant_fast_p1(const float *mu, const float *sg, int64_t n_per_ch, int64_t ch_stride, int32_t n_ch, const float *table,
+                         const Lambdas32 &lam, int32_t L, uint16_t *out_idx, int64_t E, int vec_ok, const Pass1Partials &p1,
+                         int wg_per_cu, int reserved, hipStream_t st) {
+    int64_t gx = 1;
+    bool resident = false;
+    quant_fast_grid(n_per_ch, n_ch, wg_per_cu, reserved, false, &gx, &resident);
+    if (resident) vec_ok |= 4;
+    hipLaunchKernelGGL((k_quant_fast<10, 0, true>), dim3((unsigned)gx, (unsigned)n_ch), dim3(kFastThreads), 0, st, mu, sg, (long)n_per_ch,
+                       (long)ch_stride, (int)n_ch, table, lam, (const float *)nullptr, (int)L, out_idx, (float *)nullptr, (float *)nullptr,
+                       (long)E, vec_ok, fast_debug(), (unsigned long long *)nullptr, p1);
+    VBQ_CHECK_LAUNCH("quant_fast_p1");
     return VBQ_OK;
 }
 
@@ -1243,18 +1322,28 @@
     return gx < 1 ? 1 : gx;
 }
 
+int64_t level_counts_hull_resident_grid(int32_t n_ch) {
+    const int64_t cap = resident_slots(VBQ_HULL_WAVES * 256 / kHullThreads, 0) / n_ch;
+    return cap < 1 ? 1 : cap;
+}
+
 int launch_level_counts_hull10(const float *mu, const float *sg, int64_t n_per_ch, int64_t ch_stride, int32_t n_ch,
                                const float *table, const double *lam, int32_t L, int vec_ok,
-                               unsigned long long *level_counts, int reserved, hipStream_t st) {
+                               unsigned long long *level_counts, uint32_t *partials, int64_t partials_cap, int32_t *n_partials,
+                               int reserved, hipStream_t st) {
     if (L < 1 || L > 32) return 1;
     HullSweep sw;
     if (!build_lambda_sweep(lam, L, sw)) return 1;
     const int64_t gx = level_counts_hull_grid(n_per_ch, n_ch, reserved);
+    if (partials) {
+        if (gx > partials_cap) return 1;
+        *n_partials = (int32_t)gx;
+    }
     const int dbg = fast_debug();
     Lambdas32 l32;
     for (int i = 0; i < kMaxLambdaChunk; ++i) l32.lam[i] = i < L ? (float)lam[i] : 0.0f;
     hipLaunchKernelGGL((k_level_counts_hull<10>), dim3((unsigned)gx, (unsigned)n_ch), dim3(kHullThreads), 0, st, mu, sg,
-                       (long)n_per_ch, (long)ch_stride, (int)n_ch, table, l32, sw, vec_ok, level_counts, dbg);
+                       (long)n_per_ch, (long)ch_stride, (int)n_ch, table, l32, sw, vec_ok, level_counts, dbg, partials);
     VBQ_CHECK_LAUNCH("level_counts_hull");
     return VBQ_OK;
 }
diff --git a/vbq_amd/ops.py b/vbq_amd/ops.py
--- a/vbq_amd/ops.py
+++ b/vbq_amd/ops.py
@@ -196,6 +196,43 @@
                                      -1 if reserved_workgroups is None else int(reserved_workgroups), _stream(mu)),
               "vbq_level_counts_f32")
     return out
+
+
+def level_partials(mu: torch.Tensor, sigma: torch.Tensor, table_lm: torch.Tensor, lambdas: Sequence[float], workspace: torch.Tensor, *,
+                   N: int = 10, layout="cb", reserved_workgroups: Optional[int] = None) -> int:
+    layout = _LAYOUTS[layout]
+    mu, sigma, rows, Cc, table_lm, L, _ = _solve_inputs(mu, sigma, table_lm, lambdas, N, None, layout)
+    h = _lib.lib()
+    wsb = h.vbq_quantize_workspace_bytes(Cc, L, N)
+    ws = _workspace(workspace, wsb, mu.device)
+    n = C.c_int32(0)
+    if mu.numel():
+        check(h.vbq_level_partials_f32(_ptr(mu), _ptr(sigma), rows, Cc, layout, _ptr(table_lm), _doubles(lambdas), L, N, _ptr(ws),
+                                       ws.numel() * ws.element_size(), -1 if reserved_workgroups is None else int(reserved_workgroups),
+                                       C.byref(n), _stream(mu)), "vbq_level_partials_f32")
+    return int(n.value)
+
+
+def quantize_from_partials(mu: torch.Tensor, sigma: torch.Tensor, table_lm: torch.Tensor, lambdas: Sequence[float], n_partials: int,
+                           lut: torch.Tensor, workspace: torch.Tensor, *, out_level_counts: torch.Tensor, out_level_len: torch.Tensor,
+                           out_raw_models: torch.Tensor, N: int = 10, layout="cb", out_idx: Optional[torch.Tensor] = None,
+                           workgroups_per_cu: int = 0, reserved_workgroups: Optional[int] = None):
+    layout = _LAYOUTS[layout]
+    mu, sigma, rows, Cc, table_lm, L, _ = _solve_inputs(mu, sigma, table_lm, lambdas, N, None, layout)
+    lut = _dev(lut, torch.float32, "lut")
+    _out(out_level_counts, (L, Cc, N + 1), torch.int64, mu.device, "out_level_counts")
+    _out(out_level_len, (L, Cc, N + 1), torch.float32, mu.device, "out_level_len")
+    _out(out_raw_models, (L, Cc, N + 1), torch.float32, mu.device, "out_raw_models")
+    idx = _out(out_idx, (L,) + tuple(mu.shape), torch.uint16, mu.device, "out_idx")
+    h = _lib.lib()
+    wsb = h.vbq_quantize_workspace_bytes(Cc, L, N)
+    ws = _workspace(workspace, wsb, mu.device)
+    check(h.vbq_quantize_from_partials_f32(_ptr(mu), _ptr(sigma), rows, Cc, layout, _ptr(table_lm), _doubles(lambdas), L, N,
+                                           int(n_partials), _ptr(lut), lut.numel(), _ptr(out_level_counts), _ptr(out_level_len),
+                                           _ptr(out_raw_models), _ptr(idx), _ptr(ws), ws.numel() * ws.element_size(),
+                                           int(workgroups_per_cu), -1 if reserved_workgroups is None else int(reserved_workgroups),
+                                           _stream(mu)), "vbq_quantize_from_partials_f32")
+    return idx
 
 
 def code_lengths_from_counts(counts: torch.Tensor, lut: torch.Tensor, *, level_period: int = 0, want_len: bool = True,
diff --git a/vbq_amd/pipeline.py b/vbq_amd/pipeline.py
--- a/vbq_amd/pipeline.py
+++ b/vbq_amd/pipeline.py
@@ -254,6 +254,7 @@
         self.k1_workgroups_per_cu = 3
         self.side = torch.cuda.Stream(device=self.dev) if len(self.chunks) > 1 else None
         self._events = [torch.cuda.Event() for _ in self.chunks] if self.side is not None else []
+        self._partials_ok = self.world == 1 and self.lut1 is not None and self.side is None
         self.reducers = [None, None]
         self.works = [None, None]
         self._models_pending = [False, False]
@@ -330,6 +331,14 @@
             self._len_stage.enqueue()
         return self.level_len, self.raw_models
 
+    def _histogram_one_gpu(self):
+        fused = self.lut2 is not None and self.models is not None
+        self._t("k2", 0)
+        ops.histogram_models(self.idx, self.C, self.counts, N=self.N, lut=self.lut2 if fused else None,
+                             models=self.models if fused else None)
+        self._t("k2", 1)
+        self._models_current = fused
+
     def pass2(self, mu_cb, sg_cb, level_len):
         if self.world > 1:
             self._slot ^= 1
@@ -338,16 +347,11 @@
         main = torch.cuda.current_stream(self.dev)
         self._models_current = False
         if self.side is None and self.world == 1:
-            fused = self.lut2 is not None and self.models is not None
             self._t("k1", 0)
             ops.quantize(mu_cb, sg_cb, self.table, self.lambdas, N=self.N, level_len=level_len, layout="cb",
                          out_idx=self.idx, workspace=self.ws, reserved_workgroups=self._reserved())
             self._t("k1", 1)
-            self._t("k2", 0)
-            ops.histogram_models(self.idx, self.C, self.counts, N=self.N, lut=self.lut2 if fused else None,
-                                 models=self.models if fused else None)
-            self._t("k2", 1)
-            self._models_current = fused
+            self._histogram_one_gpu()
             return self.idx, self.counts
         self.counts.zero_()
         if self.side is None:
@@ -452,10 +456,29 @@
             if r is not None:
                 r.check()
 
+    def pass1_into_pass2(self, mu_cb, sg_cb) -> bool:
+        if not self._partials_ok:
+            return False
+        self._t("k1h", 0)
+        n = ops.level_partials(mu_cb, sg_cb, self.table, self.lambdas, self.ws, N=self.N, reserved_workgroups=self._reserved())
+        if n == 0:
+            self._partials_ok = False
+            return False
+        self._t("k1h", 1)
+        self._models_current = False
+        self._t("k1", 0)
+        ops.quantize_from_partials(mu_cb, sg_cb, self.table, self.lambdas, n, self.lut1, self.ws, out_level_counts=self.level_counts,
+                                   out_level_len=self.level_len, out_raw_models=self.raw_models, N=self.N, out_idx=self.idx,
+                                   reserved_workgroups=self._reserved())
+        self._t("k1", 1)
+        self._histogram_one_gpu()
+        return True
+
     def run(self, mu_cb, sg_cb, level_len=None, models: bool = True):
-        self.pass1(mu_cb, sg_cb, level_len)
-        ll, _ = self.lengths()
-        self.pass2(mu_cb, sg_cb, ll)
+        if level_len is not None or not self.pass1_into_pass2(mu_cb, sg_cb):
+            self.pass1(mu_cb, sg_cb, level_len)
+            ll, _ = self.lengths()
+            self.pass2(mu_cb, sg_cb, ll)
         if models and self.models is not None:
             if self.world == 1:
                 self.finish_models()
```

Measured after the change: 507.6 billion latents/s (median of 3 runs). About the same (+0.2%).
